# nihofm/volren

Hardware: AMD Instinct MI355X
Metric: Msamples/s (pixels x spp / s), volume path tracing (higher is better)
Workload: dtype f32; 1 GPU; BASELINE configs[1] 'c2': smoke.brick, no transfer function, 1024x1024, 1024 spp, seed 42, fov 40; parallelism=1 GPU, 1 fused launch(es)/frame (sample pool budget 64 GiB)

## Files before the change

### volren_amd/csrc/capi.cpp

```cpp
#include "../../include/volren_amd.h"

#include <algorithm>
#include <cmath>
#include <cstring>
#include <filesystem>
#include <functional>
#include <iostream>
#include <stdexcept>
#include <memory>
#include <string>
#include <vector>

#include "imageio.h"
#include "renderer.h"
#include "sharded.h"
#include "vr_device.h"
#include "vr_math_probe.h"

struct vr_renderer {
    vr::RendererHIP impl;
    int device = 0;
};

struct vr_sharded {
// ... 107 lines not shown

int vr_load_envmap(vr_renderer* r, const char* path) {
    NEED(r);
    if (!path) return fail(VR_ERR_ARG, "null path");
    return guard([&] { use_device(r); r->impl.environment = std::make_shared<vr::Environment>(std::string(path)); r->impl.sample = 0; });
}

int vr_load_transferfunc(vr_renderer* r, const char* path) {
    NEED(r);
    if (!path) return fail(VR_ERR_ARG, "null path");
    return guard([&] {
        use_device(r);
        r->impl.transferfunc = std::make_shared<vr::TransferFunction>(std::string(path));
        r->impl.show_environment = false;
        r->impl.sample = 0;
    });
}

static void install_grid(vr_renderer* r, const char* name, const std::shared_ptr<vr::Grid>& grid, int unit_cube) {
    const std::string n = name ? name : "density";
    auto& R = r->impl;
    if (n == "density") {
        R.volume = std::make_shared<vr::Volume>(grid);
        if (unit_cube) { R.density_scale = 1.f; R.scale_and_move_to_unit_cube(); }
    } else {
        if (!R.volume || R.volume->grids.empty()) throw std::runtime_error("set the density grid before '" + n + "'");
        R.volume->update_grid_frame(R.volume->grid_frame_counter, grid, n);
    }
    R.sample = 0;
}

int vr_set_volume_dense(vr_renderer* r, const char* name, const float* voxels, int nx, int ny, int nz, const float* transform, int unit_cube) {
    NEED(r);
    if (!voxels || nx <= 0 || ny <= 0 || nz <= 0) return fail(VR_ERR_ARG, "bad dense grid arguments");
    return guard([&] {
        use_device(r);
        auto g = std::make_shared<vr::DenseGrid>((uint32_t)nx, (uint32_t)ny, (uint32_t)nz, voxels);
        if (transform) memcpy(g->transform.m, transform, 64);
        install_grid(r, name, g, unit_cube);
    });
}

int vr_volume_add_grid_frame_dense(vr_renderer* r, const char* name, const float* voxels, int nx, int ny, int nz, const float* transform) {
    NEED(r);
    if (!voxels || nx <= 0 || ny <= 0 || nz <= 0) return fail(VR_ERR_ARG, "bad dense grid arguments");
    return guard([&] {
        auto g = std::make_shared<vr::DenseGrid>((uint32_t)nx, (uint32_t)ny, (uint32_t)nz, voxels);
        if (transform) memcpy(g->transform.m, transform, 64);
        if (!r->impl.volume) r->impl.volume = std::make_shared<vr::Volume>();
        r->impl.volume->add_grid_frame(g, name ? name : "density");
        r->impl.sample = 0;
    });
}
int vr_volume_update_grid_frame_dense(vr_renderer* r, int frame, const char* name, const float* voxels, int nx, int ny, int nz, const float* transform) {
    NEED(r);
    if (!voxels || nx <= 0 || ny <= 0 || nz <= 0 || frame < 0) return fail(VR_ERR_ARG, "bad dense grid arguments");
    return guard([&] {
        if (!r->impl.volume || (size_t)frame >= r->impl.volume->n_grid_frames()) throw std::out_of_range("vr_volume_update_grid_frame_dense: no such frame");
        auto g = std::make_shared<vr::DenseGrid>((uint32_t)nx, (uint32_t)ny, (uint32_t)nz, voxels);
        if (transform) memcpy(g->transform.m, transform, 64);
        r->impl.volume->update_grid_frame((size_t)frame, g, name ? name : "density");
        r->impl.sample = 0;
    });
}
int vr_volume_n_grid_frames(vr_renderer* r, int* n) {
    NEED(r);
    if (!n) return fail(VR_ERR_ARG, "null output");
    *n = r->impl.volume ? (int)r->impl.volume->n_grid_frames() : 0;
    return VR_OK;
}

int vr_set_volume_dense_f16(vr_renderer* r, const char* name, const uint16_t* voxels, int nx, int ny, int nz, const float* transform, int unit_cube) {
    NEED(r);
    if (!voxels || nx <= 0 || ny <= 0 || nz <= 0) return fail(VR_ERR_ARG, "bad dense grid arguments");
    return guard([&] {
        use_device(r);
        auto g = std::make_shared<vr::DenseGridF16>((uint32_t)nx, (uint32_t)ny, (uint32_t)nz, voxels);
        if (transform) memcpy(g->transform.m, transform, 64);
        install_grid(r, name, g, unit_cube);
    });
}

int vr_set_volume_brick(vr_renderer* r, const char* name, const float* transform, const uint32_t nb[3], const float min_maj[2],
                        const uint32_t* indirection, const uint32_t* range, const uint32_t atlas_dim[3], const uint8_t* atlas,
                        int n_mips, const uint32_t* const* mips, const uint32_t (*mip_dims)[3], int unit_cube) {
    NEED(r);
    if (!nb || !min_maj || !indirection || !range || !atlas_dim || !atlas || n_mips < 0 || n_mips > 3) return fail(VR_ERR_ARG, "bad brick grid arguments");
    return guard([&] {
        use_device(r);
        auto g = std::make_shared<vr::BrickGrid>();
        if (transform) memcpy(g->transform.m, transform, 64);
        g->n_bricks = { nb[0], nb[1], nb[2] };
        g->min_maj = { min_maj[0], min_maj[1] };
        const size_t n = (size_t)nb[0] * nb[1] * nb[2];
        g->indirection = vr::Buf3D<uint32_t>(nb[0], nb[1], nb[2]);
        g->range = vr::Buf3D<uint32_t>(nb[0], nb[1], nb[2]);
        memcpy(g->indirection.data.data(), indirection, n * 4);
        memcpy(g->range.data.data(), range, n * 4);
        if ((atlas_dim[0] % 8) || (atlas_dim[1] % 8) || (atlas_dim[2] % 8)) throw std::runtime_error("atlas dimensions must be multiples of 8");
        g->atlas = vr::Buf3D<uint8_t>(atlas_dim[0], atlas_dim[1], atlas_dim[2]);
        memcpy(g->atlas.data.data(), atlas, g->atlas.data.size());
        uint64_t cnt = 0;
        for (size_t i = 0; i < n; ++i) cnt += (vr::half2float(range[i] & 0xFFFFu) != vr::half2float(range[i] >> 16));
        g->brick_counter = cnt;
        for (int m = 0; m < n_mips; ++m) {
            vr::Buf3D<uint32_t> b(mip_dims[m][0], mip_dims[m][1], mip_dims[m][2]);
            memcpy(b.data.data(), mips[m], b.data.size() * 4);
            g->range_mipmaps.push_back(std::move(b));
        }
        install_grid(r, name, g, unit_cube);
    });
}

int vr_set_envmap(vr_renderer* r, const float* rgb, int w, int h) {
    NEED(r);
    if (!rgb || w <= 0 || h <= 0) return fail(VR_ERR_ARG, "bad envmap arguments");
    return guard([&] { use_device(r); r->impl.environment = std::make_shared<vr::Environment>(rgb, w, h); r->impl.sample = 0; });
}

int vr_set_transferfunc(vr_renderer* r, const float* rgba, int n) {
    NEED(r);
    return guard([&] {
        use_device(r);
        if (n <= 0 || !rgba) { r->impl.transferfunc.reset(); r->impl.sample = 0; return; }
        std::vector<vr::vec4> lut;
        for (int i = 0; i < n; ++i) lut.emplace_back(rgba[4 * i], rgba[4 * i + 1], rgba[4 * i + 2], rgba[4 * i + 3]);
        r->impl.transferfunc = std::make_shared<vr::TransferFunction>(lut);
        r->impl.sample = 0;
    });
}

int vr_set_int(vr_renderer* r, const char* name, int v) {
    NEED(r);
    if (!name) return fail(VR_ERR_ARG, "null name");
    return guard([&] {
        auto& R = r->impl;
        const std::string n = name;
        if (n == "sample") { R.sample = v; R.drop_tile_samples(); }
        else if (n == "sppx") R.sppx = v;
        else if (n == "seed") R.seed = v;
        else if (n == "bounces") R.bounces = v;
        else if (n == "show_environment") R.show_environment = v != 0;
        else if (n == "tonemapping") R.tonemapping = v != 0;
        else if (n == "integrator") R.integrator = v;
        else if (n == "fast_math") R.fast_math = v != 0;
        else if (n == "variance") { if (v < 0 || v > 1) throw std::runtime_error("variance: 0 (off) or 1 (keep the per-pixel second moments)"); R.variance = v; }
        else if (n == "denoise_iterations") {
            if (v < 0 || v > vr::kDenoiseMaxIterations) throw std::runtime_error("denoise_iterations must be in [0, 10]");
            R.denoise_iterations = v;
        }
        else if (n == "coalesce_trace") { R.flush_pending(); R.coalesce_trace = v != 0; }
        else if (n == "majorant_layout") { if (v < -1 || v > 1) throw std::runtime_error("majorant_layout: -1 (per grid, chosen at commit), 0 (linear), 1 (4x4x4-cell blocks)"); R.majorant_layout = v; }
        else if (n == "tf_float_atlas") R.tf_float_atlas = v != 0;
        else if (n == "wide_addressing") { if (v < 0 || v > 1) throw std::runtime_error("wide_addressing: 0 (by the tables' sizes), 1 (always the kernels with 64-bit gather addresses)"); R.tuning.wide_addressing = v; }
        else if (n == "gpu_encoder") R.gpu_encoder = v != 0;
        else if (n == "sample_pool_mb") { if (v < 16 || v > 65536) throw std::runtime_error("sample_pool_mb must be in [16, 65536] (item indices of a sub-launch are 32-bit: < 2^32 RGBA32F items)"); R.sample_pool_bytes = (size_t)v << 20; }
        else if (n == "launch_target_ms") { if (v < 0) throw std::runtime_error("launch_target_ms must be >= 0 (0 = no sizing by time)"); R.launch_target_ms = v; }
        else if (n == "order_tiles") { if (v < 0 || v > 2) throw std::runtime_error("order_tiles: 0 (never), 1 (tile subsets), 2 (always)"); R.order_tiles = v; }
        else if (n == "grid_frame_counter") {
            if (!R.volume || v < 0 || (size_t)v >= R.volume->n_grid_frames()) throw std::runtime_error("grid_frame_counter out of range");
            R.volume->grid_frame_counter = (size_t)v;
        } else throw std::runtime_error("unknown int parameter: " + n);
    });
}

int vr_get_int(vr_renderer* r, const char* name, int* v) {
    NEED(r);
    if (!name || !v) return fail(VR_ERR_ARG, "null argument");
    return guard([&] {
        auto& R = r->impl;
        const std::string n = name;
        if (n == "sample") *v = R.sample;
        else if (n == "sppx") *v = R.sppx;
        else if (n == "seed") *v = R.seed;
        else if (n == "bounces") *v = R.bounces;
        else if (n == "show_environment") *v = R.show_environment ? 1 : 0;
        else if (n == "tonemapping") *v = R.tonemapping ? 1 : 0;
        else if (n == "integrator") *v = R.integrator;
        else if (n == "fast_math") *v = R.fast_math ? 1 : 0;
        else if (n == "variance") *v = R.variance;
        else if (n == "denoise_iterations") *v = R.denoise_iterations;
        else if (n == "coalesce_trace") *v = R.coalesce_trace ? 1 : 0;
        else if (n == "majorant_layout") *v = R.majorant_layout;
        else if (n == "majorant_blocked") {
            vr::SceneParams P; R.fill_params(P); *v = P.density.maj_blocked;
        }
        else if (n == "kernel_variant" || n == "kernel_variant_reason") {
            vr::SceneParams P; R.fill_params(P);
            int why = 0; const int variant = vr::pathtrace_variant_of(P, &why);
            *v = n == "kernel_variant" ? variant : why;
        }
        else if (n == "wide_addressing") *v = R.tuning.wide_addressing;
        else if (n == "kernel_wide") {
            vr::SceneParams P; R.fill_params(P);
            *v = (vr::pathtrace_wide_of(R.tuning, P) || vr::pathtrace_variant_of(P, nullptr) >= 2) ? 1 : 0;
        }
        else if (n == "env_div_safe") *v = R.environment && R.environment->cdf_div_safe ? 1 : 0;
        else if (n == "env_compact") *v = R.environment && R.environment->envmap_rgbe ? 1 : 0;
        else if (n == "pending_samples") *v = R.pending_samples();
        else if (n == "tf_float_atlas") *v = R.tf_float_atlas ? 1 : 0;
        else if (n == "gpu_encoder") *v = R.gpu_encoder ? 1 : 0;
        else if (n == "sample_pool_mb") *v = (int)(R.sample_pool_bytes >> 20);
        else if (n == "launch_target_ms") *v = R.launch_target_ms;
        else if (n == "order_tiles") *v = R.order_tiles;
        else if (n == "grid_frame_counter") *v = R.volume ? (int)R.volume->grid_frame_counter : 0;
        else if (n == "n_grid_frames") *v = R.volume ? (int)R.volume->n_grid_frames() : 0;
        else if (n == "last_launches") *v = R.last_launches;
        else if (n == "adaptive_rounds") *v = R.adaptive_rounds;
        else if (n == "width") *v = R.resolution.x;
        else if (n == "height") *v = R.resolution.y;
        else throw std::runtime_error("unknown int parameter: " + n);
    });
}

namespace {
struct FloatField { float* ptr; int count; };
FloatField float_field(vr::RendererHIP& R, const std::string& n) {
    if (n == "tonemap_exposure") return { &R.tonemap_exposure, 1 };
    if (n == "tonemap_gamma") return { &R.tonemap_gamma, 1 };
    if (n == "albedo") return { &R.albedo.x, 3 };
    if (n == "phase") return { &R.phase, 1 };
    if (n == "density_scale") return { &R.density_scale, 1 };
    if (n == "emission_scale") return { &R.emission_scale, 1 };
    if (n == "vol_clip_min") return { &R.vol_clip_min.x, 3 };
    if (n == "vol_clip_max") return { &R.vol_clip_max.x, 3 };
    if (n == "cam_pos") return { &R.camera.pos.x, 3 };
    if (n == "cam_dir") return { &R.camera.dir.x, 3 };
    if (n == "cam_up") return { &R.camera.up.x, 3 };
    if (n == "cam_fov") return { &R.camera.fov_degree, 1 };
    if (n == "env_strength") { if (!R.environment) throw std::runtime_error("no environment"); return { &R.environment->strength, 1 }; }
    if (n == "env_transform") { if (!R.environment) throw std::runtime_error("no environment"); return { R.environment->transform.m, 9 }; }
    if (n == "tf_window_left") { if (!R.transferfunc) throw std::runtime_error("no transfer function"); return { &R.transferfunc->window_left, 1 }; }
    if (n == "tf_window_width") { if (!R.transferfunc) throw std::runtime_error("no transfer function"); return { &R.transferfunc->window_width, 1 }; }
    if (n == "volume_transform") { if (!R.volume) throw std::runtime_error("no volume"); return { R.volume->transform.m, 16 }; }
    if (n == "denoise_sigma") return { R.denoise_sigma, 5 };
    if (n == "denoise_alpha") return { &R.denoise_alpha, 1 };
    throw std::runtime_error("unknown float parameter: " + n);
}
}

int vr_set_float(vr_renderer* r, const char* name, const float* values, int count) {
    NEED(r);
    if (!name || !values) return fail(VR_ERR_ARG, "null argument");
    return guard([&] {
        auto& R = r->impl;
        const std::string n = name;
        if (n == "env_rot") {
            if (count != 1) throw std::runtime_error("env_rot takes 1 value");
            if (!R.environment) throw std::runtime_error("no environment");
            R.environment->transform = vr::rotation_axis(values[0], 1);
            return;
        }
        if (n == "albedo" && count == 1) { R.albedo = vr::vec3(values[0]); return; }
        if (n == "denoise_sigma") {
            if (count != 5) throw std::runtime_error("denoise_sigma takes 5 values (colour, normal, depth, coverage, albedo)");
            for (int i = 0; i < 5; ++i)
                if (!(values[i] >= vr::kDenoiseSigmaMin && values[i] <= vr::kDenoiseSigmaMax))
                    throw std::runtime_error("denoise_sigma: every value must be in [2^-60, 2^60]");
        }
        if (n == "denoise_alpha" && count == 1 && !(values[0] >= vr::kTemporalAlphaMin && values[0] <= vr::kTemporalAlphaMax))
            throw std::runtime_error("denoise_alpha must be in [2^-20, 1]");
        const FloatField f = float_field(R, n);
        if (count != f.count) throw std::runtime_error("wrong value count for " + n);
        memcpy(f.ptr, values, sizeof(float) * (size_t)count);
    });
}

int vr_get_float(vr_renderer* r, const char* name, float* values, int count) {
    NEED(r);
    if (!name || !values) return fail(VR_ERR_ARG, "null argument");
    return guard([&] {
        const FloatField f = float_field(r->impl, name);
        if (count != f.count) throw std::runtime_error(std::string("wrong value count for ") + name);
        memcpy(values, f.ptr, sizeof(float) * (size_t)count);
    });
}

int vr_commit(vr_renderer* r) { NEED(r); return guard([&] { use_device(r); r->impl.commit(); }); }
int vr_reset(vr_renderer* r) { NEED(r); return guard([&] { r->impl.reset(); }); }
int vr_scale_and_move_to_unit_cube(vr_renderer* r) { NEED(r); return guard([&] { r->impl.scale_and_move_to_unit_cube(); }); }

int vr_trace(vr_renderer* r) { NEED(r); return guard([&] { use_device(r); r->impl.trace(); }); }
int vr_flush(vr_renderer* r) { NEED(r); return guard([&] { use_device(r); r->impl.flush_pending(); }); }
int vr_render(vr_renderer* r, int spp) { NEED(r); return guard([&] { use_device(r); r->impl.render(spp); }); }

int vr_synchronize(vr_renderer* r) {
    NEED(r);
    return guard([&] {
        use_device(r);
        r->impl.synchronize();
        r->impl.check_watchdog();
    });
}

int vr_last_kernel_ms(vr_renderer* r, double* ms) {
    NEED(r);
    if (!ms) return fail(VR_ERR_ARG, "null argument");
    return guard([&] { use_device(r); *ms = r->impl.last_kernel_ms(); });
}

int vr_last_pathtrace_ms(vr_renderer* r, double* ms) {
    NEED(r);
    if (!ms) return fail(VR_ERR_ARG, "null output");
    return guard([&] { use_device(r); *ms = r->impl.last_pathtrace_ms(); });
}

int vr_framebuffer(vr_renderer* r, float* out) {
    NEED(r);
    if (!out) return fail(VR_ERR_ARG, "null argument");
    return guard([&] { use_device(r); r->impl.download(out); });
}
int vr_render_features(vr_renderer* r, int spp) {
    NEED(r);
    if (vr_device_count() <= 0) return fail(VR_ERR_NO_DEVICE, "no HIP device available (libvolren_amd has no CPU path)");
    return guard([&] { use_device(r); r->impl.render_features(spp); });
}
int vr_features(vr_renderer* r, float* out) {
    NEED(r);
    if (!out) return fail(VR_ERR_ARG, "null argument");
    if (vr_device_count() <= 0) return fail(VR_ERR_NO_DEVICE, "no HIP device available (libvolren_amd has no CPU path)");
    return guard([&] { use_device(r); r->impl.download_features(out); });
}
int vr_variance(vr_renderer* r, float* out) {
    NEED(r);
    if (!out) return fail(VR_ERR_ARG, "null argument");
    if (vr_device_count() <= 0) return fail(VR_ERR_NO_DEVICE, "no HIP device available (libvolren_amd has no CPU path)");
    return guard([&] { use_device(r); r->impl.download_variance(out); });
}
int vr_denoise(vr_renderer* r) {
    NEED(r);
    if (vr_device_count() <= 0) return fail(VR_ERR_NO_DEVICE, "no HIP device available (libvolren_amd has no CPU path)");
    return guard([&] { use_device(r); r->impl.denoise(); });
}
int vr_denoise_temporal(vr_renderer* r) {
    NEED(r);
    if (vr_device_count() <= 0) return fail(VR_ERR_NO_DEVICE, "no HIP device available (libvolren_amd has no CPU path)");
    return guard([&] { use_device(r); r->impl.denoise_temporal(); });
}
int vr_denoise_history_reset(vr_renderer* r) {
    NEED(r);
    if (vr_device_count() <= 0) return fail(VR_ERR_NO_DEVICE, "no HIP device available (libvolren_amd has no CPU path)");
    return guard([&] { use_device(r); r->impl.flush_pending(); r->impl.drop_history(); });
}
int vr_denoise_history(vr_renderer* r, float* rgba_out, float* var_out, float* length_out) {
    NEED(r);
    if (vr_device_count() <= 0) return fail(VR_ERR_NO_DEVICE, "no HIP device available (libvolren_amd has no CPU path)");
    return guard([&] { use_device(r); r->impl.download_history(rgba_out, var_out, length_out); });
}
int vr_denoised(vr_renderer* r, float* out) {
    NEED(r);
    if (!out) return fail(VR_ERR_ARG, "null argument");
    if (vr_device_count() <= 0) return fail(VR_ERR_NO_DEVICE, "no HIP device available (libvolren_amd has no CPU path)");
    return guard([&] { use_device(r); r->impl.download_denoised(out); });
// ... 272 lines not shown
```

### volren_amd/csrc/renderer.cpp

```cpp
#include "renderer.h"

#include <algorithm>
#include <cfloat>
#include <cmath>
#include <cstdlib>
#include <cstring>
#include <iostream>

#include "vr_adaptive.h"
#include "vr_device.h"
#include "vr_math.h"
#include "vr_probe.h"

namespace vr {

mat3 Camera::view_inverse() const {
    const vec3 f = normalize(dir);
    const vec3 s = normalize(cross(f, up));
    const vec3 u = cross(s, f);
    mat3 r(0.0f);
    r.m[0] = s.x; r.m[1] = s.y; r.m[2] = s.z;
    r.m[3] = u.x; r.m[4] = u.y; r.m[5] = u.z;
    r.m[6] = -f.x; r.m[7] = -f.y; r.m[8] = -f.z;
    return r;
// ... 192 lines not shown
}

BrickGridHIP RendererHIP::dense_grid_to_device(const std::shared_ptr<DenseGridF16>& g) {
    BrickGridHIP out;
    const uvec3 nb = g->range.stride;
    out.nb[0] = (int)nb.x; out.nb[1] = (int)nb.y; out.nb[2] = (int)nb.z;
    out.dim[0] = (int)g->dim.x; out.dim[1] = (int)g->dim.y; out.dim[2] = (int)g->dim.z;
    if (g->dim.x > 65535u || g->dim.y > 65535u || g->dim.z > 65535u) throw std::runtime_error("dense_grid_to_device: more than 65535 voxels along an axis");
    out.transform = g->transform;
    const uint32_t bx = (g->dim.x + 3u) / 4u, by = (g->dim.y + 3u) / 4u, bz = (g->dim.z + 3u) / 4u;
    if ((uint64_t)bx * by * bz > (1ull << 31)) throw std::runtime_error("dense_grid_to_device: more than 2^31 blocks");
    out.dblk[0] = (int)bx; out.dblk[1] = (int)by;
    std::vector<uint16_t> blocked((size_t)bx * by * bz * 64u, 0);
    for (uint32_t z = 0; z < g->dim.z; ++z)
        for (uint32_t y = 0; y < g->dim.y; ++y) {
            const uint16_t* row = &g->voxels[((size_t)z * g->dim.y + y) * g->dim.x];
            for (uint32_t x = 0; x < g->dim.x; ++x) blocked[dense_blocked_index(x, y, z, bx, by)] = row[x];
        }
    out.dense = make_device_buffer(blocked.size() * sizeof(uint16_t));
    out.dense->upload(blocked.data(), blocked.size() * sizeof(uint16_t));
    upload_range_words(out, nb, g->range, g->range_mipmaps);
    return out;
}

BrickGridHIP RendererHIP::brick_grid_to_device(const std::shared_ptr<BrickGrid>& g) {
    BrickGridHIP out;
    const uvec3 nb = g->n_bricks;
    const size_t n_bricks = (size_t)nb.x * nb.y * nb.z;
    if (n_bricks == 0) throw std::runtime_error("brick_grid_to_device: empty grid");
    out.nb[0] = (int)nb.x; out.nb[1] = (int)nb.y; out.nb[2] = (int)nb.z;
    out.transform = g->transform;
    const uvec3 ad = g->atlas.stride;
    const uint32_t sx = ad.x / 8, sy = ad.y / 8, sz = ad.z / 8;
    upload_range_words(out, nb, g->range, g->range_mipmaps);
    check_grid_bytes(brick_records(out) * (kBrickBlockBytes + sizeof(BrickRec) + 8), "the brick-linear atlas", out.nb);
    std::vector<BrickRec> recs(brick_records(out), BrickRec{ 0u, 0.f, 0.f, 0u });
    std::vector<uint8_t> atlas(recs.size() * (size_t)kBrickBlockBytes, 0);
    for (size_t i = 0; i < n_bricks; ++i) {
        const uint32_t ind = g->indirection.data[i], rg = g->range.data[i];
        const uint32_t px = ind >> 22, py = (ind >> 12) & 1023u, pz = (ind >> 2) & 1023u;
        const float lo = half2float(rg & 0xFFFFu), hi = half2float(rg >> 16);
        const size_t idx = i;
        BrickRec r;
        r.slot = (uint32_t)idx;
        r.rmin = lo;
        r.rdiff = hi - lo;
        r.range = rg;
        recs[idx] = r;
        uint8_t* dst = &atlas[idx * (size_t)kBrickBlockBytes];
        if (VR_BRICK_HEADERS)
            for (uint32_t l = 0; l < 5; ++l) { memcpy(dst + l * 128u, &r.rmin, 4); memcpy(dst + l * 128u + 4u, &r.rdiff, 4); }
        if (r.rdiff != 0.f && px < sx && py < sy && pz < sz) {
            ++out.n_active;
            for (uint32_t z = 0; z < 8; ++z)
                for (uint32_t y = 0; y < 8; ++y) {
                    const uint8_t* src = &g->atlas.data[g->atlas.index(px * 8, py * 8 + y, pz * 8 + z)];
                    for (uint32_t x = 0; x < 8; ++x) dst[brick_voxel_byte(z * 64 + y * 8 + x)] = src[x];
                }
        }
    }
    out.bricks = make_device_buffer(recs.size() * sizeof(BrickRec));
    out.bricks->upload(recs.data(), recs.size() * sizeof(BrickRec));
    std::vector<float> rng(recs.size() * 2);
    for (size_t i = 0; i < recs.size(); ++i) { rng[2 * i] = recs[i].rmin; rng[2 * i + 1] = recs[i].rdiff; }
    out.rng = make_device_buffer(rng.size() * sizeof(float));
    out.rng->upload(rng.data(), rng.size() * sizeof(float));
    out.atlas = make_device_buffer(atlas.size());
    out.atlas->upload(atlas.data(), atlas.size());
    return out;
}

void RendererHIP::scale_and_move_to_unit_cube() {
    vec3 bb_min(FLT_MAX), bb_max(FLT_MIN);
    for (const auto& frame : volume->grids) {
        const auto grid = frame.at("density");
        const uvec3 e = grid->index_extent();
        bb_min = vmin(bb_min, transform_point(grid->transform, vec3(0.f, 0.f, 0.f)));
        bb_max = vmax(bb_max, transform_point(grid->transform, vec3((float)e.x, (float)e.y, (float)e.z)));
    }
    const vec3 extent = bb_max - bb_min;
    const float size = std::fmax(extent.x, std::fmax(extent.y, extent.z));
    if (size != 1.f) {
        volume->transform = scale_then_translate(1.f / size, -bb_min - extent * 0.5f);
        density_scale *= size;
    }
}

static void copy3(float* dst, vec3 v) { dst[0] = v.x; dst[1] = v.y; dst[2] = v.z; }

static GridView make_view(const BrickGridHIP& g, bool paired = false, bool maj_blocked = false) {
    GridView v;
    memset(&v, 0, sizeof v);
    v.bricks = g.bricks ? g.bricks->as<BrickRec>() : nullptr;
    v.atlas = paired ? g.atlas_paired->as<uint8_t>() : (g.atlas ? g.atlas->as<uint8_t>() : nullptr);
    v.dense = g.dense ? g.dense->as<uint16_t>() : nullptr;
    for (int i = 0; i < 3; ++i) v.dim[i] = g.dim[i];
    for (int i = 0; i < 2; ++i) v.dblk[i] = g.dblk[i];
    v.majorant = g.majorant->as<float>();
    v.majorant16 = g.majorant16->as<uint16_t>();
    v.rng = g.rng ? g.rng->as<float>() : nullptr;
    v.atlas_f32 = g.atlas_f32 ? g.atlas_f32->as<float>() : nullptr;
    for (int i = 0; i < 3; ++i) v.nb[i] = g.nb[i];
    for (int i = 0; i < 3; ++i) { v.mshift[i] = g.mshift[i]; v.mlim[i] = (float)(8u << g.mshift[i]); }
    v.n_mips = g.n_mips;
    v.maj_blocked = maj_blocked ? 1 : 0;
    v.maj_outside = (int32_t)majorant_padded_cells((uint32_t)(g.mshift[0] + g.mshift[1] + g.mshift[2]));
    return v;
}

static float camera_z(float fov_degree) { return -0.5f / tan_(0.5f * kPi * fov_degree / 180.f); }

void RendererHIP::fill_params(SceneParams& P) {
    if (!volume || volume->grids.empty() || density_grids.empty())
        throw std::runtime_error("RendererHIP::trace: no volume committed");
    if (volume->grid_frame_counter >= density_grids.size())
        throw std::runtime_error("RendererHIP::trace: grid_frame_counter out of range (commit() after changing the volume)");
    memset(&P, 0, sizeof P);
    Uniforms& u = P.u;
    u.bounces = bounces;
    u.seed = seed;
    u.show_environment = show_environment ? 1 : 0;
    copy3(u.cam_pos, camera.pos);
    u.cam_fov = camera.fov_degree;
    const mat3 ct = camera.view_inverse();
    memcpy(u.cam_transform, ct.m, sizeof ct.m);
    P.cam_z = camera_z(camera.fov_degree);
    const auto [bb_min, bb_max] = volume->AABB();
    const auto [mn, maj] = volume->minorant_majorant();
    copy3(u.vol_bb_min, bb_min + vol_clip_min * (bb_max - bb_min));
    copy3(u.vol_bb_max, bb_min + vol_clip_max * (bb_max - bb_min));
    u.vol_minorant = mn * density_scale;
    u.vol_majorant = maj * density_scale;
    u.vol_inv_majorant = 1.f / (maj * density_scale);
    copy3(u.vol_albedo, albedo);
    u.vol_phase_g = phase;
    u.vol_density_scale = density_scale;
    u.vol_emission_scale = emission_scale;
    u.vol_emission_norm = majorant_emission > 0.f ? 1.f / std::fmax(majorant_emission, 1e-4f) : 1.f;
    const BrickGridHIP& density = density_grids[volume->grid_frame_counter];
    const mat4 dt = volume->transform * density.transform;
    const mat4 dti = inverse(dt);
    memcpy(u.vol_density_transform, dt.m, sizeof dt.m);
    memcpy(u.vol_density_inv_transform, dti.m, sizeof dti.m);
    P.density = make_view(density);
    if (volume->grid_frame_counter < emission_grids.size()) {
        const BrickGridHIP& emission = emission_grids[volume->grid_frame_counter];
        const mat4 et = volume->transform * emission.transform;
        const mat4 eti = inverse(et);
        memcpy(u.vol_emission_transform, et.m, sizeof et.m);
        memcpy(u.vol_emission_inv_transform, eti.m, sizeof eti.m);
        const mat4 efd = eti * dt;
        memcpy(P.emission_from_density, efd.m, sizeof efd.m);
        const bool scale_ok = u.vol_density_scale >= 1.0f / 65536.0f && u.vol_density_scale <= 16777216.0f;
        P.paired = (integrator == 0 && environment->cdf_div_safe && scale_ok && density.atlas_paired && density.atlas_paired == emission.atlas_paired) ? 1 : 0;
        if (P.paired) P.density = make_view(density, true, majorant_layout < 0 ? density.maj_blocked : majorant_layout == 1);
        P.emission = make_view(emission, P.paired != 0);
        u.has_emission = 1;
    }
    if (transferfunc) {
        u.use_tf = 1;
        u.tf_size = transferfunc->size();
        u.tf_window_left = transferfunc->window_left;
        u.tf_window_width = transferfunc->window_width;
        P.tf_lut = transferfunc->lut_ssbo->as<float>();
    }
    const mat3 eit = inverse(environment->transform);
    memcpy(u.env_transform, environment->transform.m, sizeof eit.m);
    memcpy(u.env_inv_transform, eit.m, sizeof eit.m);
    u.env_strength = environment->strength;
    u.env_imp_inv_dim[0] = u.env_imp_inv_dim[1] = 1.f / (float)environment->dimension();
    u.env_imp_base_mip = (int)std::floor(std::log2((float)environment->dimension()));
    P.envmap = environment->envmap->as<float>();
    P.env_rgbe = environment->envmap_rgbe ? environment->envmap_rgbe->as<uint32_t>() : nullptr;
    P.env_w = environment->width; P.env_h = environment->height;
    P.env_avg_w = environment->avg_importance; P.env_avg_w_set = 1;
    P.impmap = environment->impmap->as<float>();
    P.imp_dim = (int)environment->dimension();
    P.env_cdf = environment->cdf->as<float>();
    P.env_div_safe = environment->cdf_div_safe ? 1 : 0;
    u.resolution[0] = resolution.x; u.resolution[1] = resolution.y;
    u.integrator = integrator;
}

void RendererHIP::update_majorants(const LaunchInputs& in, BrickGridHIP& g) {
    const MajKey& k = in.maj;
    if (k.density_scale == maj_key_.density_scale && k.tf_version == maj_key_.tf_version &&
        k.wl == maj_key_.wl && k.ww == maj_key_.ww && k.frame == maj_key_.frame && k.blocked == maj_key_.blocked)
        return;
    launch_majorants(in.P, g.range_words->as<uint32_t>(), g.nb, g.mip_off, g.n_mips, g.mshift, g.majorant->as<float>(), g.majorant16->as<uint16_t>(), in.stream);
    VR_HIP(hipGetLastError());
    maj_key_ = k;
}

void RendererHIP::set_tiles(const std::vector<int32_t>& tile_ids) {
    flush_pending();
    tiles_host_ = tile_ids;
    tiles_dev_.reset();
    if (tile_ids.empty()) return;
    if (resolution.x > 0) {
        const int n_all = tile_count(resolution.x, resolution.y);
        for (int32_t t : tile_ids)
            if (t < 0 || t >= n_all) throw std::runtime_error("set_tiles: tile id out of range");
    }
    tiles_dev_ = make_device_buffer(tile_ids.size() * sizeof(int32_t));
    tiles_dev_->upload(tile_ids.data(), tile_ids.size() * sizeof(int32_t));
}

std::vector<int32_t> RendererHIP::costliest_first(const SceneParams& P, const std::vector<int32_t>& tile_ids, int n_tiles) const {
    const Uniforms& u = P.u;
    const int W = u.resolution[0], H = u.resolution[1], tiles_x = vr::tiles_x(W);
    std::vector<int32_t> ids(tile_ids);
    if (ids.empty()) { ids.resize((size_t)n_tiles); for (int i = 0; i < n_tiles; ++i) ids[(size_t)i] = i; }
    auto chord = [&](float px, float py) {
        float d[3] = { (px - 0.5f * (float)W) / (float)H, (py - 0.5f * (float)H) / (float)H, P.cam_z };
        float w[3];
        for (int i = 0; i < 3; ++i) w[i] = u.cam_transform[i] * d[0] + u.cam_transform[3 + i] * d[1] + u.cam_transform[6 + i] * d[2];
        const float len = std::sqrt(w[0] * w[0] + w[1] * w[1] + w[2] * w[2]);
        float t0 = 0.f, t1 = FLT_MAX;
        for (int i = 0; i < 3; ++i) {
            const float inv = 1.f / (w[i] / len);
            const float a = (u.vol_bb_min[i] - u.cam_pos[i]) * inv, b = (u.vol_bb_max[i] - u.cam_pos[i]) * inv;
            t0 = std::fmax(t0, std::fmin(a, b)); t1 = std::fmin(t1, std::fmax(a, b));
        }
        return t1 > t0 ? t1 - t0 : 0.f;
    };
    std::vector<float> cost(ids.size());
    for (size_t k = 0; k < ids.size(); ++k) {
        const float x0 = (float)((ids[k] % tiles_x) * 16), y0 = (float)((ids[k] / tiles_x) * 16);
        const float x1 = std::fmin(x0 + 16.f, (float)W), y1 = std::fmin(y0 + 16.f, (float)H);
        cost[k] = std::fmax(std::fmax(std::fmax(chord(x0, y0), chord(x1, y0)), std::fmax(chord(x0, y1), chord(x1, y1))), chord(0.5f * (x0 + x1), 0.5f * (y0 + y1)));
    }
    std::vector<int32_t> perm(ids.size());
    for (size_t k = 0; k < perm.size(); ++k) perm[k] = (int32_t)k;
    const size_t seg = (ids.size() + 7) / 8;
    for (size_t b = 0; b < ids.size(); b += seg)
        std::stable_sort(perm.begin() + (ptrdiff_t)b, perm.begin() + (ptrdiff_t)std::min(ids.size(), b + seg), [&](int32_t x, int32_t y) { return cost[(size_t)x] > cost[(size_t)y]; });
    std::vector<int32_t> ordered(ids.size());
    for (size_t k = 0; k < ids.size(); ++k) ordered[k] = ids[(size_t)perm[k]];
    return ordered;
}

const int32_t* RendererHIP::tile_order(const SceneParams& P, const std::vector<int32_t>& ids, int n_tiles) {
    const Uniforms& u = P.u;
    uint64_t key = 1469598103934665603ull;
    auto mix = [&key](const void* p, size_t nbytes) { const uint8_t* b = static_cast<const uint8_t*>(p); for (size_t i = 0; i < nbytes; ++i) { key ^= b[i]; key *= 1099511628211ull; } };
    mix(u.cam_pos, sizeof u.cam_pos); mix(u.cam_transform, sizeof u.cam_transform); mix(&P.cam_z, sizeof P.cam_z);
    mix(u.vol_bb_min, sizeof u.vol_bb_min); mix(u.vol_bb_max, sizeof u.vol_bb_max); mix(u.resolution, sizeof u.resolution); mix(&n_tiles, sizeof n_tiles);
    if (!ids.empty()) mix(ids.data(), ids.size() * sizeof(int32_t));
    key = key ? key : 1;
    if (order_dev_ && order_key_ == key && order_dev_->size_bytes() == (size_t)n_tiles * sizeof(int32_t)) return order_dev_->as<int32_t>();
    const std::vector<int32_t> ordered = costliest_first(P, ids, n_tiles);
    ensure_buffer(order_dev_, ordered.size() * sizeof(int32_t));
    order_dev_->upload(ordered.data(), ordered.size() * sizeof(int32_t), stream);
    order_key_ = key;
    return order_dev_->as<int32_t>();
}

bool RendererHIP::LaunchInputs::same_launch_as(const LaunchInputs& o) const {
    return memcmp(&P, &o.P, sizeof P) == 0 && frame == o.frame && maj.density_scale == o.maj.density_scale && maj.tf_version == o.maj.tf_version &&
           maj.wl == o.maj.wl && maj.ww == o.maj.ww && maj.blocked == o.maj.blocked && memcmp(tuning.thr, o.tuning.thr, sizeof tuning.thr) == 0 && tuning.stats == o.tuning.stats &&
           tuning.samples_per_unit == o.tuning.samples_per_unit && tuning.blocks_per_cu == o.tuning.blocks_per_cu && tuning.wide_addressing == o.tuning.wide_addressing && order_tiles == o.order_tiles &&
           launch_target_ms == o.launch_target_ms && fast_math == o.fast_math && variance == o.variance && sample_pool_bytes == o.sample_pool_bytes && stream == o.stream;
}

void RendererHIP::capture(LaunchInputs& in) {
    if (!color) throw std::runtime_error("RendererHIP::trace: no framebuffer (call resize first)");
    if (integrator == 2 && !transferfunc) throw std::runtime_error("RendererHIP::trace: integrator 2 (direct volume rendering) needs a transfer function");
    if (integrator < 0 || integrator > 3) throw std::runtime_error("RendererHIP::trace: unknown integrator");
    if (fast_math && transferfunc) throw std::runtime_error("RendererHIP::trace: fast_math is not available while a transfer function is bound (it misses the 1e-3 bound there); set fast_math 0");
    if (!volume || volume->grids.empty() || density_grids.empty()) throw std::runtime_error("RendererHIP::trace: no volume committed");
    if (volume->grid_frame_counter >= density_grids.size()) throw std::runtime_error("RendererHIP::trace: grid_frame_counter out of range (commit() after changing the volume)");
    {
        BrickGridHIP& g = density_grids[volume->grid_frame_counter];
        const bool build = transferfunc && tf_float_atlas && !g.dense && g.atlas && g.rng && !g.atlas_f32 && !g.atlas_f32_failed;
        const bool drop = (!transferfunc || !tf_float_atlas) && (g.atlas_f32 || g.atlas_f32_failed);
        if (build || drop) flush_pending();
        if (build) {
            try {
                const size_t n_blocks = g.atlas->size_bytes() / kBrickBlockBytes, want = n_blocks * 512u * sizeof(float);
                auto drop_others = [&] { for (BrickGridHIP& other : density_grids) if (&other != &g) other.atlas_f32.reset(); };
                size_t free_b = 0, total_b = 0;
                if (hipMemGetInfo(&free_b, &total_b) != hipSuccess) { (void)hipGetLastError(); free_b = ~(size_t)0; }
                if (want > free_b / 2) drop_others();
                try { g.atlas_f32 = make_device_buffer(want); }
                catch (const std::exception&) { (void)hipGetLastError(); drop_others(); g.atlas_f32 = make_device_buffer(want); }
                launch_decode_atlas(g.rng->as<float>(), g.atlas->as<uint8_t>(), g.atlas_f32->as<float>(), n_blocks, stream);
                VR_HIP(hipGetLastError());
            } catch (const std::exception& e) {
                (void)hipGetLastError();
                g.atlas_f32.reset();
                g.atlas_f32_failed = true;
                std::cerr << "volren_amd: no room for the decoded float atlas (" << (g.atlas->size_bytes() / kBrickBlockBytes * 2048u >> 20) << " MiB): transfer-function taps read the byte atlas (" << e.what() << ")" << std::endl;
            }
        }
        if (drop) { g.atlas_f32.reset(); g.atlas_f32_failed = false; }
    }
    fill_params(in.P);
    in.frame = volume->grid_frame_counter;
    in.maj = MajKey{};
    in.maj.density_scale = density_scale;
    in.maj.tf_version = transferfunc ? transferfunc->version : 0;
    in.maj.wl = transferfunc ? transferfunc->window_left : 0.f;
    in.maj.ww = transferfunc ? transferfunc->window_width : 0.f;
    in.maj.frame = in.frame;
    in.maj.blocked = in.P.density.maj_blocked;
    in.tuning = tuning;
    in.order_tiles = order_tiles; in.launch_target_ms = launch_target_ms; in.fast_math = fast_math ? 1 : 0; in.variance = variance != 0 ? 1 : 0;
    in.sample_pool_bytes = sample_pool_bytes;
    in.stream = stream;
    in.env = environment; in.tf = transferfunc;
    in.keep[0] = environment->envmap; in.keep[1] = environment->impmap; in.keep[2] = environment->cdf;
    in.keep[3] = transferfunc ? transferfunc->lut_ssbo : DeviceBufferPtr();
    in.keep[4] = environment->envmap_rgbe;
}

int RendererHIP::samples_per_launch(const LaunchInputs& in, int n_tiles) const {
    const size_t per_sample = pathtrace_pool_floats(in.tuning, n_tiles, 1) * sizeof(float);
    int per_launch = (int)std::max<size_t>(1, in.sample_pool_bytes / per_sample);
    const size_t lim = (size_t)0xFFFFFFFFu / ((size_t)n_tiles * 256u);
    per_launch = (int)std::min<size_t>((size_t)per_launch, lim > 8 ? lim - 8 : 1);
    if (per_launch > 32) per_launch -= per_launch % 32;
    return per_launch;
}

void RendererHIP::submit_tile_set(const LaunchInputs& in, int first, int n) {
    if (n <= 0) return;
    const int n_tiles = tiles_dev_ ? (int)tiles_host_.size() : tile_count(in.P.u.resolution[0], in.P.u.resolution[1]);
    const bool ordered = in.order_tiles >= 2 || (in.order_tiles == 1 && tiles_dev_);
// ... 518 lines not shown
```

### volren_amd/csrc/renderer.h

```cpp
#pragma once

#include <memory>
#include <vector>

#include "devmem.h"
#include "environment.h"
#include "grids.h"
#include "transferfunc.h"
#include "vr_device.h"
#include "vr_scene.h"

namespace vr {

struct Camera {
    vec3 pos{ 1.f, 0.f, 1.f };
    vec3 dir = normalize(-pos);
    vec3 up{ 0.f, 1.f, 0.f };
    float fov_degree = 70.f;
    mat3 view_inverse() const;
};

struct BrickGridHIP {
    DeviceBufferPtr bricks;
    DeviceBufferPtr atlas;
    DeviceBufferPtr range_words;
    DeviceBufferPtr majorant;
    DeviceBufferPtr majorant16;
    DeviceBufferPtr rng;
    DeviceBufferPtr atlas_f32;
    bool atlas_f32_failed = false;
    DeviceBufferPtr atlas_paired;
    DeviceBufferPtr dense;
    int32_t dim[3] = { 0, 0, 0 };
    int32_t dblk[2] = { 0, 0 };
    int32_t nb[3] = { 0, 0, 0 };
    int32_t mip_off[4] = { 0, 0, 0, 0 };
    int32_t n_mips = 0;
    int32_t n_cells = 0;
    int32_t mshift[3] = { 3, 3, 3 };
    size_t n_active = 0;
    bool maj_blocked = false;
    mat4 transform;
};

struct RendererHIP {
    void init();
    void resize(uint32_t w, uint32_t h);
    void commit();
    void trace();
    void draw();
    void reset();

    void render(int n = 0);
    void render_adaptive(int min_spp, int max_spp, float threshold);
    std::vector<int32_t> tile_samples();
    std::vector<float> tile_error();
    bool ragged();
    void drop_tile_samples();
    void check_watchdog();

    BrickGridHIP brick_grid_to_device(const std::shared_ptr<BrickGrid>& grid);
    BrickGridHIP dense_grid_to_device(const std::shared_ptr<DenseGridF16>& grid);
    BrickGridHIP grid_to_device(const Volume::GridPtr& grid);
    BrickGridHIP dense_to_bricks_on_device(const std::shared_ptr<DenseGrid>& grid);
    bool gpu_encoder = true;
    void grid_checksums(const BrickGridHIP& g, uint64_t out[3]) const;
    void scale_and_move_to_unit_cube();

    int sample = 0;
    int sppx = 1024;
    int seed = 42;
    int bounces = 100;
    float tonemap_exposure = 5.f;
    float tonemap_gamma = 2.2f;
    bool tonemapping = true;
    bool show_environment = true;

    vec3 albedo = vec3(0.9f);
    float phase = 0.f;
    float density_scale = 1.f;
    float emission_scale = 100.f;

    DeviceBufferPtr color;
    DeviceBufferPtr display;
    std::vector<BrickGridHIP> density_grids;
    std::vector<BrickGridHIP> emission_grids;
    float majorant_emission = 0.f;

    std::shared_ptr<Volume> volume;

    vec3 vol_clip_min = vec3(0.f);
    vec3 vol_clip_max = vec3(1.f);

    std::shared_ptr<Environment> environment;
    std::shared_ptr<TransferFunction> transferfunc;

    Camera camera;
    ivec2 resolution{ 0, 0 };
    hipStream_t stream = nullptr;
    int integrator = 0;
    bool tf_float_atlas = true;
    int order_tiles = 1;
    int majorant_layout = -1;
    int variance = 0;
    int denoise_iterations = kDenoiseDefaultIterations;
    float denoise_sigma[5] = { kDenoiseDefaultSigma[0], kDenoiseDefaultSigma[1], kDenoiseDefaultSigma[2], kDenoiseDefaultSigma[3], kDenoiseDefaultSigma[4] };
    float denoise_alpha = kTemporalDefaultAlpha;
    bool fast_math = false;
    PathtraceTuning tuning = default_tuning();
    int last_launches = 0;
    int adaptive_rounds = 0;
    int launch_target_ms = 2000;
    size_t sample_pool_bytes = (size_t)64 << 30;

    void set_tiles(const std::vector<int32_t>& tile_ids);
    void fill_params(SceneParams& P);
    void download(float* rgba);
    void render_features(int spp);
    void probe(int what, int form, const uint32_t* in, float* out, size_t n);
    void download_features(float* out);
    void download_variance(float* rgba);
    void denoise();
    void denoise_temporal();
    void drop_history();
    void download_history(float* rgba, float* var, float* length);
    void download_denoised(float* rgba);
    const DeviceBuffer* denoised() const { return denoised_.get(); }
    void draw_from(const DeviceBuffer& src);
    void download_display(float* rgba) const;
    void synchronize();
    void flush_pending();
    int pending_samples() const { return pending_n_; }
    bool coalesce_trace = true;
    double last_kernel_ms();
    double last_pathtrace_ms();
    void sched_stats(bool enable, unsigned long long out[32]);
    void wave_timeline(unsigned long long* out, size_t n_words);
    uint32_t watchdog_status();
    ~RendererHIP();

private:
    struct MajKey { float density_scale = -1.f; uint64_t tf_version = ~0ull; float wl = 0, ww = 0; size_t frame = ~(size_t)0; int blocked = -1; };
    struct LaunchInputs {
        SceneParams P;
        MajKey maj;
        size_t frame = 0;
        PathtraceTuning tuning;
        int order_tiles = 0, launch_target_ms = 0, fast_math = 0, variance = 0;
        size_t sample_pool_bytes = 0;
        hipStream_t stream = nullptr;
        std::shared_ptr<Environment> env;
        std::shared_ptr<TransferFunction> tf;
        DeviceBufferPtr keep[5];
        bool same_launch_as(const LaunchInputs& o) const;
    };
    void capture(LaunchInputs& in);
    void submit(const LaunchInputs& in, int first, int n, const int32_t* tiles, int n_tiles);
    void submit_tile_set(const LaunchInputs& in, int first, int n);
    int samples_per_launch(const LaunchInputs& in, int n_tiles) const;
    LaunchInputs pending_;
    int pending_n_ = 0, pending_first_ = 0, pending_cap_ = 0;
    void update_majorants(const LaunchInputs& in, BrickGridHIP& g);
    std::vector<int32_t> tiles_host_;
    DeviceBufferPtr tiles_dev_;
    DeviceBufferPtr order_dev_;
    uint64_t order_key_ = 0;
    std::vector<int32_t> costliest_first(const SceneParams& P, const std::vector<int32_t>& ids, int n_tiles) const;
    const int32_t* tile_order(const SceneParams& P, const std::vector<int32_t>& ids, int n_tiles);
    std::vector<int32_t> tile_n_;
    int tile_n_sample_ = -1;
    DeviceBufferPtr tile_n_dev_, adaptive_lists_, adaptive_err_;
    bool keep_timing_ = false;
    DeviceBufferPtr status_;
    DeviceBufferPtr pool_;
    DeviceBufferPtr workspace_;
    DeviceBufferPtr stats_;
    DeviceBufferPtr features_;
    DeviceBufferPtr moments_;
    int moments_n_ = -1;
    void check_moments(const char* who);
    DeviceBufferPtr dn_guide_, dn_var_[2], dn_color_[2];
    DeviceBufferPtr denoised_;
    void run_denoise(const char* who, bool temporal);
    DeviceBufferPtr hist_color_[2], hist_record_[2];
    int hist_cur_ = -1;
    TemporalCamera hist_cam_{};
    hipEvent_t ev0_ = nullptr, ev1_ = nullptr;
    std::vector<hipEvent_t> pt_events_;
    size_t pt_events_used_ = 0;
    double last_ms_ = 0.0, last_pathtrace_ms_ = 0.0;
    bool timing_pending_ = false;
    double rate_samples_per_ms_ = 0.0;
    uint64_t rate_key_ = 0, rate_pending_key_ = 0;
    double rate_pending_samples_ = 0.0;
    void harvest_rate(bool wait);
    MajKey maj_key_;
};

using Renderer = RendererHIP;

}
```

### volren_amd/csrc/vr_device.h

```cpp
#pragma once

#include <hip/hip_runtime.h>
#include <stdint.h>

#include "vr_denoise.h"
#include "vr_scene.h"
#include "vr_temporal.h"
#include "vr_tiles.h"

namespace vr {

struct PathtraceTuning {
    int32_t thr[8] = { 64, 0, 56, 0, 60, 60, 64, 0 };
    unsigned long long* stats = nullptr;
    int32_t samples_per_unit = 0;
    int32_t blocks_per_cu = 0;
    int32_t wide_addressing = 0;
};
PathtraceTuning default_tuning();
size_t pathtrace_pool_floats(const PathtraceTuning& T, int32_t n_tiles, int32_t n_samples);
size_t pathtrace_workspace_floats();
void launch_pathtrace(const PathtraceTuning& T, const SceneParams& P, float* fb, float* sample_pool, float* workspace, uint32_t* unit_counter, const int32_t* tiles, int32_t n_tiles,
                      int32_t first_sample, int32_t n_samples, uint32_t* status, hipStream_t stream, bool fast_math = false,
                      hipEvent_t ev_kernel_begin = nullptr, hipEvent_t ev_kernel_end = nullptr,
                      float* moments = nullptr);
constexpr uint32_t kFeatureLostStatus = 4u;
void launch_features(const SceneParams& P, const int32_t* tiles, int32_t n_tiles, int32_t spp, float* out, uint32_t* status, hipStream_t stream);
enum PathtraceVariantReason : int {
    VR_VARIANT_INTEGRATOR = 1,
    VR_VARIANT_ENV_DIVISION = 2,
    VR_VARIANT_DENSITY_SCALE = 4,
    VR_VARIANT_GRID_FORMS = 8
};
int pathtrace_variant_of(const SceneParams& P, int* why);
bool pathtrace_wide_of(const PathtraceTuning& T, const SceneParams& P);
void launch_denoise_prepare(const float* moments, const float* features, int32_t W, int32_t H, int32_t n, float vscale, const int32_t* counts, float* v, float* guide,
                            hipStream_t stream);
void launch_denoise_atrous(const float* cin, const float* vin, const float* guide, int32_t W, int32_t H, int32_t step, const DenoiseSigma& sg,
                           float* cout, float* vout, hipStream_t stream);
void launch_denoise_temporal(const float* color, float* v, const float* guide, const float* hist_color, const float* hist_record, bool same_cam,
                             const TemporalCamera& cur, const TemporalCamera& prev, int32_t W, int32_t H, float alpha, float* out_color, float* out_record,
                             hipStream_t stream);
void launch_adaptive_error(const float* fb, const float* moments, const int32_t* tiles, const int32_t* counts, int32_t n_tiles, int32_t W, int32_t H, float* out,
                           hipStream_t stream);

void launch_tonemap(float* fb, int32_t w, int32_t h, float exposure, float gamma, hipStream_t stream);

void launch_pack_tiles(const float* fb, int32_t w, int32_t h, const int32_t* tiles, int32_t n_tiles, float* packed, hipStream_t stream);
void launch_unpack_tiles(const float* packed, const int32_t* tiles, int32_t n_tiles, float* fb, int32_t w, int32_t h, hipStream_t stream);
void launch_build_impmap(const float* envmap_rgba, int32_t env_w, int32_t env_h, int32_t dim, float* pyramid, hipStream_t stream);

void launch_build_env_cdf(const float* pyramid, int32_t dim, float* table, uint32_t* unsafe_flag, hipStream_t stream);

void launch_majorants(const SceneParams& P, const uint32_t* range_words_all_mips, const int32_t nb[3], const int32_t mip_off[4], int32_t n_mips,
                      const int32_t mshift[3], float* out_padded, uint16_t* out16_padded, hipStream_t stream);

void launch_encode_ranges(const float* dense, const int32_t dim[3], const int32_t nb[3], uint32_t* range, uint32_t* flag, hipStream_t stream);
void launch_encode_bricks(const float* dense, const int32_t dim[3], const int32_t nb[3], const uint32_t* range, const uint32_t* flag,
                          BrickRec* recs, float* rng, uint8_t* atlas, hipStream_t stream);
void launch_range_mip(const uint32_t* src, const int32_t sdim[3], uint32_t* dst, const int32_t ddim[3], hipStream_t stream);

void launch_pair_atlas(const uint8_t* atlas_density, const uint8_t* atlas_emission, uint8_t* out, size_t n_records, hipStream_t stream);

void launch_decode_atlas(const float* rng, const uint8_t* atlas, float* out, size_t n_records, hipStream_t stream);
void launch_math_probe(int32_t fn, const float* a, const float* b, float* out, int32_t n, hipStream_t stream);
void launch_math_sweep(int32_t fn, uint32_t first, float b, float* out, int32_t n, hipStream_t stream);
void launch_fast_math_sweep(int32_t fn, uint32_t first, float* out, int32_t n, hipStream_t stream);
void launch_probe(const SceneParams& P, int32_t what, int32_t form, const uint32_t* in, float* out, uint32_t n, hipStream_t stream);

}
```

### volren_amd/csrc/vr_launch.hip

```cpp
#include <hip/hip_runtime.h>

#include <algorithm>
#include <cstdlib>
#include <map>
#include <mutex>
#include <stdexcept>
#include <string>

#include "vr_device.h"
#include "vr_pathtrace.h"

namespace vr {

template <int INTEGRATOR>
__global__ void __launch_bounds__(256)
item_kernel(const SceneParams P, float* __restrict__ sbuf, const LaunchDesc D) {
    const uint32_t per_unit = (uint32_t)(D.spu * 64);
    const uint32_t g = blockIdx.x * 256u + threadIdx.x;
    const uint32_t u = g / per_unit, item = g - u * per_unit;
    if (u >= D.n_units) return;
    const WorkUnit wu = make_unit(D, P.u.resolution[0], u, sbuf);
    if ((int32_t)item >= wu.n_items) return;
    const int32_t px = wu.px0 + (int32_t)(item & 7u), py = wu.py0 + (int32_t)((item >> 3) & 7u);
    if (px >= P.u.resolution[0] || py >= P.u.resolution[1]) return;
    float L[4];
    if (INTEGRATOR == 2) dvr_sample(P, px, py, wu.first_sample + (int32_t)(item >> 6), L);
    else raymarch_path_sample(P, px, py, wu.first_sample + (int32_t)(item >> 6), L);
    reinterpret_cast<float4*>(sbuf)[wu.base + item] = pack4(L);
}

template <bool MOMENTS>
__global__ void __launch_bounds__(256)
accumulate_kernel(const float* __restrict__ sbuf, float* __restrict__ fb, float* __restrict__ moments, const int32_t* __restrict__ tiles, int32_t n_tiles,
                  int32_t W, int32_t H, int32_t first_sample, int32_t n_samples, int32_t spu) {
    const TilePixel q = wave_tiled_pixel(tiles ? tiles[blockIdx.x] : (int32_t)blockIdx.x, threadIdx.x, W);
    if (q.px >= W || q.py >= H) return;
    float4* texel = reinterpret_cast<float4*>(fb) + (size_t)q.py * W + q.px;
    float4* mtexel = MOMENTS ? reinterpret_cast<float4*>(moments) + (size_t)q.py * W + q.px : nullptr;
    float acc[4] = { 0.0f, 0.0f, 0.0f, 0.0f }, S[4] = { 0.0f, 0.0f, 0.0f, 0.0f };
    if (first_sample > 1) {
        unpack4(*texel, acc);
        if (MOMENTS) unpack4(*mtexel, S);
    }
    const float4* sb = reinterpret_cast<const float4*>(sbuf);
    for (int32_t k = 0; k < n_samples; ++k) {
        const int32_t chunk = k / spu, sl = k - chunk * spu;
        float L[4];
        unpack4(sb[pool_slot<size_t>((size_t)chunk, n_tiles, (size_t)blockIdx.x, (uint32_t)q.sub, spu, (size_t)sl, (uint32_t)q.lane)], L);
        const float a = 1.0f / (float)(first_sample + k);
        for (int32_t c = 0; c < 4; ++c) {
            const float x = sanitize(L[c]);
            const float mu = acc[c], mu1 = mix_(mu, x, a);
            if (MOMENTS) S[c] = mix_(S[c], (x - mu) * (x - mu1), a);
            acc[c] = mu1;
        }
    }
    *texel = pack4(acc);
    if (MOMENTS) *mtexel = pack4(S);
}

template <bool TF>
__global__ void __launch_bounds__(256)
features_kernel(const SceneParams P, const int32_t* __restrict__ tiles, int32_t spp, float* __restrict__ out, uint32_t* __restrict__ status) {
    const int32_t W = P.u.resolution[0], H = P.u.resolution[1];
    const TilePixel q = wave_tiled_pixel(tiles ? tiles[blockIdx.x] : (int32_t)blockIdx.x, threadIdx.x, W);
    if (q.px >= W || q.py >= H) return;
    float f[8];
    if (!feature_pixel<TF>(P, q.px, q.py, spp, f)) atomicOr(status, kFeatureLostStatus);
    float4* o = reinterpret_cast<float4*>(out) + 2u * ((size_t)q.py * W + q.px);
    o[0] = pack4(f);
    o[1] = pack4(f + 4);
}
void launch_features(const SceneParams& P, const int32_t* tiles, int32_t n_tiles, int32_t spp, float* out, uint32_t* status, hipStream_t stream) {
    if (n_tiles <= 0 || spp <= 0) return;
    if (P.u.use_tf) hipLaunchKernelGGL(features_kernel<true>, dim3((unsigned)n_tiles), dim3(256), 0, stream, P, tiles, spp, out, status);
    else hipLaunchKernelGGL(features_kernel<false>, dim3((unsigned)n_tiles), dim3(256), 0, stream, P, tiles, spp, out, status);
}

constexpr int32_t kMaxSamplesPerUnit = 8;
static int32_t samples_per_unit(const PathtraceTuning& T, int variant) { return T.samples_per_unit > 0 ? T.samples_per_unit : ((variant == 1 || variant == 2 || variant == 4) ? 4 : kMaxSamplesPerUnit); }
constexpr int kPtVariants = 5;

PathtraceTuning default_tuning() {
    static std::once_flag once;
    static int32_t env_spu = 0, env_blocks = 0;
    std::call_once(once, [] {
        if (const char* e = getenv("VR_SPU")) env_spu = std::max(1, atoi(e));
        if (const char* e = getenv("VR_BLOCKS_PER_CU")) env_blocks = std::max(0, atoi(e));
    });
    PathtraceTuning T;
    T.samples_per_unit = env_spu;
    T.blocks_per_cu = env_blocks;
    return T;
}

size_t pathtrace_pool_floats(const PathtraceTuning& T, int32_t n_tiles, int32_t n_samples) {
    size_t padded = 0;
    for (int variant = 0; variant < kPtVariants; ++variant) {
        const int32_t spu = std::min(n_samples, samples_per_unit(T, variant));
        padded = std::max(padded, (size_t)((n_samples + spu - 1) / spu) * (size_t)spu);
    }
    return padded * (size_t)n_tiles * 4u * 64u * 4u;
}

extern "C" {
#define VR_PT_DECL(N) \
    int vr_pt_occupancy_##N(int tf, int stats); \
    void vr_pt_launch_##N(int tf, int stats, unsigned grid, hipStream_t stream, const void* P, float* sbuf, float* cold_ws, const void* D, const void* S, uint32_t* status, unsigned long long* stats_buf);
VR_PT_DECL(0) VR_PT_DECL(1) VR_PT_DECL(2) VR_PT_DECL(3) VR_PT_DECL(4) VR_PT_DECL(0_fast) VR_PT_DECL(1_fast) VR_PT_DECL(2_fast) VR_PT_DECL(3_fast) VR_PT_DECL(4_fast)
VR_PT_DECL(0w) VR_PT_DECL(1w) VR_PT_DECL(0w_fast) VR_PT_DECL(1w_fast)
#undef VR_PT_DECL
}
typedef int (*PtOccupancy)(int, int);
typedef void (*PtLaunch)(int, int, unsigned, hipStream_t, const void*, float*, float*, const void*, const void*, uint32_t*, unsigned long long*);
static const PtOccupancy kPtOccupancy[2][2][kPtVariants] = { { { vr_pt_occupancy_0, vr_pt_occupancy_1, vr_pt_occupancy_2, vr_pt_occupancy_3, vr_pt_occupancy_4 },
                                                               { vr_pt_occupancy_0w, vr_pt_occupancy_1w, vr_pt_occupancy_2, vr_pt_occupancy_3, vr_pt_occupancy_4 } },
                                                             { { vr_pt_occupancy_0_fast, vr_pt_occupancy_1_fast, vr_pt_occupancy_2_fast, vr_pt_occupancy_3_fast, vr_pt_occupancy_4_fast },
                                                               { vr_pt_occupancy_0w_fast, vr_pt_occupancy_1w_fast, vr_pt_occupancy_2_fast, vr_pt_occupancy_3_fast, vr_pt_occupancy_4_fast } } };
static const PtLaunch kPtLaunch[2][2][kPtVariants] = { { { vr_pt_launch_0, vr_pt_launch_1, vr_pt_launch_2, vr_pt_launch_3, vr_pt_launch_4 },
                                                         { vr_pt_launch_0w, vr_pt_launch_1w, vr_pt_launch_2, vr_pt_launch_3, vr_pt_launch_4 } },
                                                       { { vr_pt_launch_0_fast, vr_pt_launch_1_fast, vr_pt_launch_2_fast, vr_pt_launch_3_fast, vr_pt_launch_4_fast },
                                                         { vr_pt_launch_0w_fast, vr_pt_launch_1w_fast, vr_pt_launch_2_fast, vr_pt_launch_3_fast, vr_pt_launch_4_fast } } };

int pathtrace_variant_of(const SceneParams& P, int* why) {
    const bool scale_ok = P.u.vol_density_scale >= 1.0f / 65536.0f && P.u.vol_density_scale <= 16777216.0f;
    int reason = 0;
    if (P.u.integrator != 0) reason |= VR_VARIANT_INTEGRATOR;
    if (!P.env_div_safe) reason |= VR_VARIANT_ENV_DIVISION;
    if (!scale_ok) reason |= VR_VARIANT_DENSITY_SCALE;
    int variant;
    if (reason) variant = 3;
    else if (P.u.has_emission) {
        const bool mixed = P.density.dense || P.emission.dense || (VR_PAIRED_ATLAS && !P.paired);
        if (mixed) reason |= VR_VARIANT_GRID_FORMS;
        variant = mixed ? 3 : (P.density.maj_blocked ? 4 : 2);
    } else variant = P.density.dense ? 1 : 0;
    if (why) *why = reason;
    return variant;
}
bool pathtrace_wide_of(const PathtraceTuning& T, const SceneParams& P) {
    if (T.wide_addressing) return true;
    uint64_t m = grid_largest_table_bytes(P.density, P.paired != 0, P.u.use_tf != 0);
    if (P.u.has_emission) m = std::max(m, grid_largest_table_bytes(P.emission, P.paired != 0, false));
    return m >= (1ull << 32);
}
static int pathtrace_variant(const SceneParams& P) {
    int why = 0;
    const int variant = pathtrace_variant_of(P, &why);
    if (why & (VR_VARIANT_ENV_DIVISION | VR_VARIANT_DENSITY_SCALE)) {
        static std::once_flag once;
        std::call_once(once, [&] {
            fprintf(stderr, "volren_amd: note: this scene is rendered by the run-time kernel variant (slower; results unchanged):%s%s\n",
                    (why & VR_VARIANT_ENV_DIVISION) ? " the environment's warp table has thresholds below 2^-76 (vr_get_int env_div_safe = 0);" : "",
                    (why & VR_VARIANT_DENSITY_SCALE) ? " the density scale lies outside [2^-16, 2^24];" : "");
        });
    }
    return variant;
}

static int resident_blocks(const PathtraceTuning& T, int mode, int wide, int variant, bool tf, bool stats) {
    int dev = 0, cus = 0;
    if (hipGetDevice(&dev) != hipSuccess) return 1024;
    static std::mutex mu;
    static std::map<uint32_t, std::pair<int, int>> cache;
    const uint32_t key = ((uint32_t)dev << 8) | ((uint32_t)wide << 6) | ((uint32_t)mode << 5) | ((uint32_t)variant << 2) | (tf ? 2u : 0u) | (stats ? 1u : 0u);
    std::pair<int, int> v;
    {
        std::lock_guard<std::mutex> lock(mu);
        auto it = cache.find(key);
        if (it == cache.end()) {
            if (hipDeviceGetAttribute(&cus, hipDeviceAttributeMultiprocessorCount, dev) != hipSuccess || cus <= 0) cus = 256;
            it = cache.emplace(key, std::make_pair(cus, kPtOccupancy[mode][wide][variant](tf, stats))).first;
        }
        v = it->second;
    }
    const int per_cu = T.blocks_per_cu > 0 ? T.blocks_per_cu : v.second;
    return std::min(v.first * per_cu, kMaxWorkgroups * 4 / kWgWaves);
}

size_t pathtrace_workspace_floats() { return kColdMainFloats + (size_t)kMaxWorkgroups * 4u * (size_t)kColdSideWaveFloats; }

void launch_pathtrace(const PathtraceTuning& T, const SceneParams& P, float* fb, float* sample_pool, float* workspace, uint32_t* unit_counter, const int32_t* tiles, int32_t n_tiles,
                      int32_t first_sample, int32_t n_samples, uint32_t* status, hipStream_t stream, bool fast_math, hipEvent_t ev_kernel_begin, hipEvent_t ev_kernel_end,
                      float* moments) {
    if (n_tiles <= 0 || n_samples <= 0) return;
    SchedParams S;
    for (int i = 0; i < ST_COUNT; ++i) S.thr[i] = T.thr[i];
    LaunchDesc D;
    D.tiles = tiles; D.n_tiles = n_tiles; D.first_sample = first_sample; D.n_samples = n_samples;
    const int variant = pathtrace_variant(P);
    D.spu = std::min(n_samples, samples_per_unit(T, variant));
    const int32_t chunks = (n_samples + D.spu - 1) / D.spu;
    if ((uint64_t)chunks * (uint64_t)n_tiles * 4u * (uint64_t)(D.spu * 64) > 0xFFFFFFFFull)
        throw std::runtime_error("launch_pathtrace: " + std::to_string(n_tiles) + " tiles x " + std::to_string(n_samples) + " samples do not fit the 32-bit item index of one launch");
    D.n_units = (uint32_t)chunks * (uint32_t)n_tiles * 4u;
    D.chunks = (uint32_t)chunks;
    D.seg_len = (D.n_units + kQueueSegments - 1u) / kQueueSegments;
    D.unit_counter = unit_counter;
    S.max_iters = kMaxIdleIters;
    if (S.thr[ST_COLLIDE] <= 0) S.thr[ST_COLLIDE] = (P.u.use_tf || P.u.has_emission) ? 32 : 24;
    const bool tf = P.u.use_tf != 0, stats = T.stats != nullptr;
    const int mode = fast_math ? 1 : 0, wide = pathtrace_wide_of(T, P) ? 1 : 0;
    const int blocks = resident_blocks(T, mode, wide, variant, tf, stats);
    const uint32_t groups_needed = (D.n_units + (uint32_t)kWgWaves - 1u) / (uint32_t)kWgWaves;
    const dim3 grid((unsigned)std::min<uint32_t>((uint32_t)blocks, groups_needed > 0 ? groups_needed : 1u)), block(256);
    if (P.u.integrator == 3 || (P.u.integrator == 2 && P.u.use_tf)) {
        const uint64_t items = (uint64_t)D.n_units * (uint64_t)(D.spu * 64);
        const auto integrate = P.u.integrator == 2 ? item_kernel<2> : item_kernel<3>;
        hipLaunchKernelGGL(integrate, dim3((unsigned)((items + 255) / 256)), block, 0, stream, P, sample_pool, D);
    } else {
        (void)hipMemsetAsync(unit_counter, 0, kQueueSegments * sizeof(uint32_t), stream);
        if (ev_kernel_begin) (void)hipEventRecord(ev_kernel_begin, stream);
        kPtLaunch[mode][wide][variant](tf, stats, grid.x, stream, &P, sample_pool, workspace, &D, &S, status, T.stats);
        if (ev_kernel_end) (void)hipEventRecord(ev_kernel_end, stream);
    }
    const auto accumulate = moments ? accumulate_kernel<true> : accumulate_kernel<false>;
    hipLaunchKernelGGL(accumulate, dim3((unsigned)n_tiles), block, 0, stream, sample_pool, fb, moments, tiles, n_tiles, P.u.resolution[0], P.u.resolution[1],
                       first_sample, n_samples, D.spu);
}

}
```

### volren_amd/csrc/vr_pathtrace.h

```cpp
#pragma once

#include <hip/hip_runtime.h>

#include <type_traits>

#include "vr_tiles.h"
#include "vr_trace.h"

namespace vr {

struct SchedParams {
    int32_t thr[ST_COUNT];
    uint32_t max_iters;
};

constexpr uint32_t kQueueSegments = 8u;
constexpr uint32_t kMaxIdleIters = 1u << 26;
constexpr uint64_t kMaxIdleTicks = 7200000000ull;
struct LaunchDesc {
    const int32_t* tiles;
    int32_t n_tiles, first_sample, n_samples, spu;
    uint32_t n_units, chunks, seg_len;
    uint32_t* unit_counter;
};

__device__ __forceinline__ WorkUnit make_unit(const LaunchDesc& D, int32_t W, uint32_t j, float* sbuf) {
    const uint32_t rem = j / D.chunks, chunk = j - rem * D.chunks;
    const uint32_t slot = rem >> 2, sub = rem & 3u;
    const TilePixel q = wave_tiled_pixel(D.tiles ? D.tiles[slot] : (int32_t)slot, sub * 64u, W);
    WorkUnit wu;
    wu.px0 = q.px;
    wu.py0 = q.py;
    wu.first_sample = D.first_sample + (int32_t)chunk * D.spu;
    wu.n_items = min(D.spu, D.n_samples - (int32_t)chunk * D.spu) * 64;
    wu.base = pool_slot<uint32_t>(chunk, D.n_tiles, slot, sub, D.spu, 0u, 0u);
    wu.out = sbuf;
    return wu;
}

#ifndef VR_WAVES_PER_SIMD
#define VR_WAVES_PER_SIMD 4
#endif
#ifndef VR_MARCH_SPECULATIVE
#define VR_MARCH_SPECULATIVE 1
#endif
#ifndef VR_MARCH_LOADS_PINNED
#define VR_MARCH_LOADS_PINNED (VR_MARCH_STEPS == 2)
#endif
#ifndef VR_DIAG_PAD_VALU
#define VR_DIAG_PAD_VALU 0
#endif
#ifndef VR_DIAG_PAD_SLEEP
#define VR_DIAG_PAD_SLEEP 0
#endif
#ifndef VR_BATCH_REGS
#define VR_BATCH_REGS 1
#endif
#ifndef VR_PRIO_HOT
#define VR_PRIO_HOT 1
#endif
#ifndef VR_PRIO_EVENTS
#define VR_PRIO_EVENTS 0
#endif
#ifndef VR_EMISSION_BY_POINTER
#define VR_EMISSION_BY_POINTER 1
#endif

#ifndef VR_HOT_RI
#define VR_HOT_RI 0
#endif
#ifndef VR_HOT_STRIDE
#define VR_HOT_STRIDE (VR_HOT_RI ? 15 : 12)
#endif
#ifndef VR_WG_WAVES
#define VR_WG_WAVES 4
#endif
#ifndef VR_MAJ_LDS
#define VR_MAJ_LDS 0
#endif
constexpr int32_t kWgWaves = VR_WG_WAVES;
constexpr int32_t kLdsPerWorkgroup = 163840 / 16 * kWgWaves;
constexpr int32_t kLutLdsEntries = 256;
template <class K> constexpr int32_t maj_lds_cells() { return !VR_MAJ_LDS ? 0 : (K::tf ? 2560 : ((K::dense == 0 && K::emission == 0) ? 10240 : 5120)); }
#ifndef VR_COLD_REGS
#define VR_COLD_REGS 0
#endif
template <class K> constexpr bool cold_in_regs() { return VR_COLD_REGS != 0 && !K::tf && K::dense == 1 && K::emission == 0; }
template <class K> constexpr int32_t waves_per_simd() { return cold_in_regs<K>() ? 3 : VR_WAVES_PER_SIMD; }

enum PoolStack : int32_t { Q_READY = 0, Q_NEE = 1, Q_POST = 2, Q_ESC = 3, Q_FREE = 4, Q_COUNT = 5 };

#ifndef VR_LAZY_EMISSION
#define VR_LAZY_EMISSION 1
#endif
template <class K> constexpr bool lazy_emission() { return VR_LAZY_EMISSION != 0 && !VR_HOT_RI && K::emission == 1; }
template <class K> constexpr int32_t hot_stride() { return lazy_emission<K>() ? 15 : VR_HOT_STRIDE; }
constexpr int32_t HOT_EL = 12;
template <class K> constexpr int32_t pool_slots() {
#ifdef VR_NSLOT
    return cold_in_regs<K>() ? 192 : VR_NSLOT;
#else
    if (cold_in_regs<K>()) return 192;
    const int32_t shared = maj_lds_cells<K>() * (K::tf ? 4 : 2) + (K::tf ? kLutLdsEntries * 16 + 16 : kWgWaves * 256);
    const int32_t n = (kLdsPerWorkgroup - shared) / kWgWaves / (hot_stride<K>() * 4 + Q_COUNT);
    return n > 192 ? 192 : n;
#endif
}
constexpr int32_t NSLOT = 192;
constexpr int32_t HOT_COL = VR_HOT_RI ? 12 : 4;
template <int32_t HOT_STRIDE, bool WORLD = false>
struct HotStoreT {
    static constexpr int32_t kStride = HOT_STRIDE;
    uint32_t* base;
    __device__ __forceinline__ void save_first_radiance(v3 eL, int32_t slot) const { uint32_t* p = base + slot * HOT_STRIDE + HOT_EL; p[0] = f2u(eL.x); p[1] = f2u(eL.y); p[2] = f2u(eL.z); }
    __device__ __forceinline__ v3 load_first_radiance(int32_t slot) const { const uint32_t* p = base + slot * HOT_STRIDE + HOT_EL; return v3{ u2f(p[0]), u2f(p[1]), u2f(p[2]) }; }
    float cam_ipos[3];
    __device__ __forceinline__ static uint32_t flags(const Hot& h) { return (uint32_t)h.state | ((uint32_t)h.shadow << 8) | ((uint32_t)h.first << 12) | ((uint32_t)h.mipq << 16); }
    __device__ __forceinline__ void save_new(const Hot& h, int32_t slot) const {
        uint32_t* p = base + slot * HOT_STRIDE;
        p[0] = h.seed;
        const v3 a = WORLD ? h.wpos : h.ipos, d = WORLD ? h.wdir : h.idir;
        p[1] = f2u(a.x); p[2] = f2u(a.y); p[3] = f2u(a.z);
        p[4] = f2u(d.x); p[5] = f2u(d.y); p[6] = f2u(d.z);
        p[7] = f2u(h.t); p[8] = f2u(h.far); p[9] = f2u(h.tau);
        p[10] = f2u(h.Tr);
        p[11] = flags(h);
        if (VR_HOT_RI) { p[12] = f2u(h.ri.x); p[13] = f2u(h.ri.y); p[14] = f2u(h.ri.z); }
    }
    __device__ __forceinline__ void save(const Hot& h, int32_t slot) const {
        uint32_t* p = base + slot * HOT_STRIDE;
        p[0] = h.seed;
        if (WORLD) {
            p[1] = f2u(h.wpos.x); p[2] = f2u(h.wpos.y); p[3] = f2u(h.wpos.z);
            p[4] = f2u(h.wdir.x); p[5] = f2u(h.wdir.y); p[6] = f2u(h.wdir.z);
            if (!h.first) p[10] = f2u(h.Tr);
        } else {
        if (!h.first) { p[1] = f2u(h.ipos.x); p[2] = f2u(h.ipos.y); p[3] = f2u(h.ipos.z); p[10] = f2u(h.Tr); }
        p[4] = f2u(h.idir.x); p[5] = f2u(h.idir.y); p[6] = f2u(h.idir.z);
        }
        p[7] = f2u(h.t); p[8] = f2u(h.far); p[9] = f2u(h.tau);
        p[11] = flags(h);
        if (VR_HOT_RI) { p[12] = f2u(h.ri.x); p[13] = f2u(h.ri.y); p[14] = f2u(h.ri.z); }
    }
    __device__ __forceinline__ void save_marched(const Hot& h, int32_t slot) const {
        uint32_t* p = base + slot * HOT_STRIDE;
        p[0] = h.seed;
        p[7] = f2u(h.t); p[9] = f2u(h.tau);
        if (!h.first) p[10] = f2u(h.Tr);
        p[11] = flags(h);
    }
    __device__ __forceinline__ void load(Hot& h, int32_t slot) const {
        const uint32_t* p = base + slot * HOT_STRIDE;
        h.seed = p[0];
        h.ipos = v3{ u2f(p[1]), u2f(p[2]), u2f(p[3]) };
        h.idir = v3{ u2f(p[4]), u2f(p[5]), u2f(p[6]) };
        if (WORLD) { h.wpos = h.ipos; h.wdir = h.idir; }
        h.ri = VR_HOT_RI ? v3{ u2f(p[12 % HOT_STRIDE]), u2f(p[13 % HOT_STRIDE]), u2f(p[14 % HOT_STRIDE]) } : v3{ 0.0f, 0.0f, 0.0f };
        h.t = u2f(p[7]); h.far = u2f(p[8]); h.tau = u2f(p[9]);
        h.Tr = u2f(p[10]);
        const uint32_t f = p[11];
        h.state = (int32_t)(f & 0xFFu); h.shadow = (int32_t)((f >> 8) & 0xFu); h.first = (int32_t)((f >> 12) & 0xFu);
        h.mipq = (int32_t)(f >> 16);
        h.majorant = 0.0f;
    }
    __device__ __forceinline__ void load_resume(Hot& h, int32_t slot, const float* inv_transform = nullptr) const {
        load(h, slot);
        const bool first = h.first != 0;
        if (WORLD) {
            h.ipos = mat4_point(inv_transform, h.wpos);
            h.idir = mat4_dir(inv_transform, h.wdir);
        } else
        h.ipos = v3{ first ? cam_ipos[0] : h.ipos.x, first ? cam_ipos[1] : h.ipos.y, first ? cam_ipos[2] : h.ipos.z };
        h.Tr = first ? 1.0f : h.Tr;
        if (!VR_HOT_RI) h.ri = rcp3_exact(h.idir);
    }
};
constexpr uint32_t kStatsWaveBase = 32u;
constexpr int32_t kMaxWorkgroups = 2048;
#ifndef VR_COLD_NT_STORES
#define VR_COLD_NT_STORES 0
#endif
template <bool SWAP = false>
struct ColdGlobalT {
    static __device__ __forceinline__ constexpr int32_t phys(int32_t f) {
        return !SWAP ? f : ((f >= C_THR && f < C_THR + 3) ? f + (C_DIR - C_THR) : ((f >= C_DIR && f < C_DIR + 3) ? f - (C_DIR - C_THR) : (f == C_SHPDF ? C_FPL : (f == C_FPL ? C_SHPDF : f))));
    }
    float* base;
    float* side;
    float* col;
    __device__ __forceinline__ float ld(int32_t f) const {
        return f >= C_COL ? col[f - C_COL]
             : f < C_SIDE ? static_cast<const float*>(__builtin_assume_aligned(base, C_STRIDE * 4))[phys(f)]
                          : static_cast<const float*>(__builtin_assume_aligned(side, C_SIDE_STRIDE * 4))[f - C_SIDE];
    }
    __device__ __forceinline__ void st(int32_t f, float v) {
        if (f >= C_COL) col[f - C_COL] = v;
#if VR_COLD_NT_STORES
        else if (f < C_SIDE) __builtin_nontemporal_store(v, static_cast<float*>(__builtin_assume_aligned(base, C_STRIDE * 4)) + phys(f));
#else
        else if (f < C_SIDE) static_cast<float*>(__builtin_assume_aligned(base, C_STRIDE * 4))[phys(f)] = v;
#endif
        else static_cast<float*>(__builtin_assume_aligned(side, C_SIDE_STRIDE * 4))[f - C_SIDE] = v;
    }
};
typedef ColdGlobalT<false> ColdGlobal;
template <bool SWAP>
__device__ __forceinline__ Quad ld4(const ColdGlobalT<SWAP>& c, int32_t f3, int32_t f1) {
    const int32_t p3 = ColdGlobalT<SWAP>::phys(f3), p1 = ColdGlobalT<SWAP>::phys(f1);
    if (f3 + 2 < C_SIDE && f1 < C_SIDE && (p3 & 3) == 0 && p1 == p3 + 3 && ColdGlobalT<SWAP>::phys(f3 + 2) == p3 + 2) {
        const float4 v = *reinterpret_cast<const float4*>(static_cast<const float*>(__builtin_assume_aligned(c.base, C_STRIDE * 4)) + p3);
        return Quad{ v3{ v.x, v.y, v.z }, v.w };
    }
    return Quad{ ld3(c, f3), c.ld(f1) };
}
constexpr int32_t kColdWaveFloats = C_STRIDE * NSLOT, kColdSideWaveFloats = C_SIDE_STRIDE * NSLOT;
constexpr size_t kColdMainFloats = (size_t)kMaxWorkgroups * 4u * (size_t)kColdWaveFloats;

__device__ __forceinline__ uint64_t wave_ballot(bool cond) { return __builtin_amdgcn_ballot_w64(cond); }
__device__ __forceinline__ int32_t popc(uint64_t mask) { return (int32_t)__popcll(mask); }
__device__ __forceinline__ int32_t popc_s(uint64_t mask) { int32_t r; asm("s_bcnt1_i32_b64 %0, %1" : "=s"(r) : "s"(mask) : "scc"); return r; }
__device__ __forceinline__ uint32_t lane_rank(uint64_t mask) {
    return __builtin_amdgcn_mbcnt_hi((uint32_t)(mask >> 32), __builtin_amdgcn_mbcnt_lo((uint32_t)mask, 0u));
}

struct ShleBanks { v3 b[3]; uint32_t item[3]; };
__device__ __forceinline__ uint32_t lane_pull_u(uint32_t src_lane, uint32_t v) { return (uint32_t)__builtin_amdgcn_ds_bpermute((int)(src_lane << 2), (int)v); }
__device__ __forceinline__ float lane_pull(uint32_t src_lane, float v) { return u2f(lane_pull_u(src_lane, f2u(v))); }
template <bool ITEMS>
__device__ __forceinline__ void shle_park(ShleBanks& B, uint32_t* stage, int32_t lane, bool valid, int32_t bs, v3 val, bool with_item, uint32_t item) {
    stage[lane] = 0u;
    __builtin_amdgcn_fence(__ATOMIC_SEQ_CST, "wavefront");
    if (valid) reinterpret_cast<uint8_t*>(stage)[((bs & 63) << 2) + (bs >> 6)] = (uint8_t)((lane + 1) | (ITEMS && with_item ? 0x80 : 0));
    __builtin_amdgcn_fence(__ATOMIC_SEQ_CST, "wavefront");
    const uint32_t w = stage[lane];
#pragma unroll
    for (int k = 0; k < 3; ++k) {
        const uint32_t byte = (w >> (8 * k)) & 0xFFu, src = byte & 0x7Fu;
        const uint32_t from = src ? src - 1u : (uint32_t)lane;
        const float x = lane_pull(from, val.x), y = lane_pull(from, val.y), z = lane_pull(from, val.z);
        B.b[k] = v3{ src ? x : B.b[k].x, src ? y : B.b[k].y, src ? z : B.b[k].z };
        if (ITEMS) { const uint32_t it = lane_pull_u(from, item); B.item[k] = (byte & 0x80u) ? it : B.item[k]; }
    }
}
__device__ __forceinline__ uint32_t bank_home(int32_t lane, int32_t bs) { return bs >= 0 ? (uint32_t)(bs & 63) : (uint32_t)lane; }
__device__ __forceinline__ v3 shle_fetch(const ShleBanks& B, int32_t lane, int32_t bs) {
    const uint32_t home = bank_home(lane, bs);
    const int32_t k = bs >> 6;
    v3 r[3];
#pragma unroll
    for (int j = 0; j < 3; ++j) r[j] = v3{ lane_pull(home, B.b[j].x), lane_pull(home, B.b[j].y), lane_pull(home, B.b[j].z) };
    return v3{ k == 0 ? r[0].x : (k == 1 ? r[1].x : r[2].x), k == 0 ? r[0].y : (k == 1 ? r[1].y : r[2].y), k == 0 ? r[0].z : (k == 1 ? r[1].z : r[2].z) };
}
__device__ __forceinline__ uint32_t item_fetch(const ShleBanks& B, int32_t lane, int32_t bs) {
    const uint32_t home = bank_home(lane, bs);
    const int32_t k = bs >> 6;
    const uint32_t r0 = lane_pull_u(home, B.item[0]), r1 = lane_pull_u(home, B.item[1]), r2 = lane_pull_u(home, B.item[2]);
    return k == 0 ? r0 : (k == 1 ? r1 : r2);
}

constexpr int32_t kBankFields = 20;
static_assert(C_SIDE == 16 && C_SHLE == 16 && C_ITEM == 19 && C_COL == kBankFields, "ColdLocal maps field f to v[f]");
struct ColdBanks { float v[3][kBankFields]; };
struct ColdLocal {
    float v[kBankFields];
    float* col;
    __device__ __forceinline__ float ld(int32_t f) const { return f >= C_COL ? col[f - C_COL] : v[f]; }
    __device__ __forceinline__ void st(int32_t f, float x) { if (f >= C_COL) col[f - C_COL] = x; else v[f] = x; }
};
constexpr uint32_t cold_bits(int32_t first, int32_t n) { return ((1u << n) - 1u) << first; }
constexpr uint32_t kColdNeeR = cold_bits(C_POS, 3) | cold_bits(C_THR, 3) | cold_bits(C_DIR, 3);
constexpr uint32_t kColdNeeW = cold_bits(C_POS, 8) | cold_bits(C_SHLE, 3);
constexpr uint32_t kColdNeeWFirst = cold_bits(C_L, 8) | cold_bits(C_ITEM, 1);
constexpr uint32_t kColdPostR = cold_bits(C_POS, 15) | cold_bits(C_SHLE, 4);
constexpr uint32_t kColdPostW = cold_bits(C_THR, 3) | cold_bits(C_L, 8);
constexpr uint32_t kColdEscR = cold_bits(C_THR, 3) | cold_bits(C_L, 8) | cold_bits(C_ITEM, 1);
__device__ __forceinline__ void cold_clear(ColdLocal& c) {
#pragma unroll
    for (int f = 0; f < kBankFields; ++f) c.v[f] = 0.0f;
    c.col = nullptr;
}
template <uint32_t MASK>
__device__ __forceinline__ void cold_fetch(ColdLocal& c, const ColdBanks& B, int32_t lane, int32_t bs) {
    const uint32_t home = bank_home(lane, bs);
    const int32_t k = bs >> 6;
#pragma unroll
    for (int f = 0; f < kBankFields; ++f)
        if ((MASK >> f) & 1u) {
            const float r0 = lane_pull(home, B.v[0][f]), r1 = lane_pull(home, B.v[1][f]), r2 = lane_pull(home, B.v[2][f]);
            c.v[f] = k == 0 ? r0 : (k == 1 ? r1 : r2);
        }
}
__device__ __forceinline__ uint32_t cold_stage(uint32_t* stage, int32_t lane, int32_t bs, bool flag) {
    stage[lane] = 0u;
    __builtin_amdgcn_fence(__ATOMIC_SEQ_CST, "wavefront");
    if (bs >= 0) reinterpret_cast<uint8_t*>(stage)[((bs & 63) << 2) + (bs >> 6)] = (uint8_t)((lane + 1) | (flag ? 0x80 : 0));
    __builtin_amdgcn_fence(__ATOMIC_SEQ_CST, "wavefront");
    return stage[lane];
}
template <uint32_t MASK, bool FLAGGED>
__device__ __forceinline__ void cold_store(ColdBanks& B, uint32_t w, int32_t lane, const ColdLocal& c) {
#pragma unroll
    for (int k = 0; k < 3; ++k) {
        const uint32_t byte = (w >> (8 * k)) & 0xFFu, src = byte & 0x7Fu;
        const uint32_t from = src ? src - 1u : (uint32_t)lane;
        const bool take = FLAGGED ? byte > 0x80u : src != 0u;
#pragma unroll
        for (int f = 0; f < kBankFields; ++f)
            if ((MASK >> f) & 1u) {
                const float x = lane_pull(from, c.v[f]);
                B.v[k][f] = take ? x : B.v[k][f];
            }
    }
}

struct KernelArgs {
    SceneParams P;
    LaunchDesc D;
    SchedParams S;
    float* sbuf;
    float* cold_ws;
    uint32_t* status;
    unsigned long long* stats;
};
typedef const __attribute__((address_space(4))) KernelArgs* KernargPtr;
__device__ __forceinline__ const KernelArgs& event_args() {
    KernargPtr p = (KernargPtr)__builtin_amdgcn_kernarg_segment_ptr();
    asm volatile("" : "+s"(p));
    return *(const KernelArgs*)p;
}

template <class K, bool STATS>
__global__ void __launch_bounds__(64 * kWgWaves, waves_per_simd<K>())
pathtrace_kernel(const KernelArgs A) {
#ifndef VR_PIN_TAP_POINTERS
#define VR_PIN_TAP_POINTERS 0
#endif
#if VR_PIN_TAP_POINTERS
    SceneParams Ppin = A.P;
    asm volatile("" : "+s"(Ppin.density.atlas), "+s"(Ppin.density.dense));
    const SceneParams& P = Ppin;
#else
    const SceneParams& P = A.P;
#endif
    const int32_t wave = __builtin_amdgcn_readfirstlane(threadIdx.x >> 6), lane = threadIdx.x & 63;
    constexpr int32_t NS = pool_slots<K>() - (STATS ? 3 : 0);

    static_assert(!cold_in_regs<K>() || kWgWaves == 4, "the cold-state-in-registers experiment runs 3 workgroups of 4 wavefronts per CU");
    __shared__ uint8_t lds_q[kWgWaves * Q_COUNT * NS];
    uint8_t* const q = lds_q + wave * (Q_COUNT * NS);
    const uint32_t wave_index = blockIdx.x * (uint32_t)kWgWaves + (uint32_t)wave;
    float* const cold_base = A.cold_ws + (size_t)wave_index * (size_t)kColdWaveFloats;
    float* const side_base = A.cold_ws + kColdMainFloats + (size_t)wave_index * (size_t)kColdSideWaveFloats;
    typedef ColdGlobalT<world_slot<K>()> ColdT;
#define VR_COLD(SLOT) ColdT{ cold_base + (SLOT) * C_STRIDE, side_base + (SLOT) * C_SIDE_STRIDE, reinterpret_cast<float*>(hs.base + (SLOT) * HS + HOT_COL) }
    constexpr bool kColdRegs = cold_in_regs<K>();
    constexpr bool kShleInRegs = !K::tf && !kColdRegs;
    constexpr bool kItemInRegs = kShleInRegs && K::dense == 1;
    static_assert(!kItemInRegs || K::emission == 0, "with an emission grid do_new writes the sample-buffer slot to the side array (no stash to park it from)");
    static_assert(NS <= 192, "ShleBanks holds 3 x 64 slots");
    static_assert(!kColdRegs || (K::emission == 0 && !K::tf), "ColdBanks: no marching-path access to the cold state (EmissionCache), C_COL not wired");
    __shared__ uint32_t lds_stage[kShleInRegs || kColdRegs ? kWgWaves * 64 : 4];
    uint32_t* const stage = lds_stage + (kShleInRegs || kColdRegs ? wave * 64 : 0);
    ShleBanks banks;
    banks.b[0] = banks.b[1] = banks.b[2] = v3{ 0, 0, 0 };
    banks.item[0] = banks.item[1] = banks.item[2] = 0u;
    ColdBanks cb;
    if (kColdRegs) {
#pragma unroll
        for (int k = 0; k < 3; ++k)
#pragma unroll
            for (int f = 0; f < kBankFields; ++f) cb.v[k][f] = 0.0f;
    }
    constexpr int32_t HS = hot_stride<K>();
    constexpr bool kLazyEm = lazy_emission<K>();
    static_assert(VR_BATCH_REGS || !kLazyEm, "the VR_BATCH_REGS=0 swap path moves a marching path's radiance through its cold line: a `first` path of a lazy-emission kernel has none");
    __shared__ uint32_t lds_hot[kWgWaves * HS * NS];
    constexpr bool kWorld = world_slot<K>();
    HotStoreT<HS, kWorld> hs;
    hs.base = lds_hot + wave * (HS * NS);
    {
        const v3 ci = mat4_point(P.u.vol_density_inv_transform, v3{ P.u.cam_pos[0], P.u.cam_pos[1], P.u.cam_pos[2] });
        hs.cam_ipos[0] = u2f(__builtin_amdgcn_readfirstlane(f2u(ci.x)));
        hs.cam_ipos[1] = u2f(__builtin_amdgcn_readfirstlane(f2u(ci.y)));
        hs.cam_ipos[2] = u2f(__builtin_amdgcn_readfirstlane(f2u(ci.z)));
    }
    __shared__ float lds_lut[K::tf ? 4 * kLutLdsEntries : 4];
    const bool lut_in_lds = K::tf && P.u.tf_size <= (uint32_t)kLutLdsEntries;
    const bool emission_on = K::emission == 2 ? P.u.has_emission != 0 : K::emission == 1;
    constexpr int32_t kMajCells = maj_lds_cells<K>();
    typedef typename std::conditional<K::tf, float, uint16_t>::type MajT;
    __shared__ MajT lds_maj[kMajCells > 0 ? kMajCells : 1];
    int32_t maj_first = 0x7FFFFFFF;
    if (kMajCells > 0) {
        const uint32_t k = (uint32_t)(P.density.mshift[0] + P.density.mshift[1] + P.density.mshift[2]);
        const int32_t maj_end = (int32_t)majorant_table_cells(k);
        maj_first = maj_end;
#pragma unroll
        for (int mip = 3; mip >= 0; --mip) {
            const int32_t off = (int32_t)majorant_level_offset(k, (uint32_t)mip);
            if (maj_end - off <= kMajCells) maj_first = off;
        }
        maj_first = __builtin_amdgcn_readfirstlane(maj_first);
        for (int32_t i = (int32_t)threadIdx.x; i < maj_end - maj_first; i += 64 * kWgWaves)
            lds_maj[i] = K::tf ? (MajT)P.density.majorant[maj_first + i] : (MajT)P.density.majorant16[maj_first + i];
    }
    if (K::tf && lut_in_lds)
        for (uint32_t i = threadIdx.x; i < 4u * P.u.tf_size; i += 64u * (uint32_t)kWgWaves) lds_lut[i] = P.tf_lut[i];
    if (K::tf || kMajCells > 0) __syncthreads();

    const int32_t pool = (A.S.thr[ST_BEGIN] > 0 && A.S.thr[ST_BEGIN] < NS) ? A.S.thr[ST_BEGIN] : NS;
    const uint32_t thr_a = (uint32_t)(A.S.thr[ST_NEW] & 255) | ((uint32_t)(A.S.thr[ST_NEE] & 255) << 8) | ((uint32_t)(A.S.thr[ST_POSTNEE] & 255) << 16) | ((uint32_t)(A.S.thr[ST_ESCAPE] & 255) << 24);
    const uint32_t thr_b = (uint32_t)(A.S.thr[ST_MARCH] & 255) | ((uint32_t)pool << 8) | ((uint32_t)(A.S.thr[ST_COLLIDE] & 255) << 16);
#define VR_THR_NEW ((int32_t)(thr_a & 255u))
#define VR_THR_NEE ((int32_t)((thr_a >> 8) & 255u))
#define VR_THR_POST ((int32_t)((thr_a >> 16) & 255u))
#define VR_THR_ESC ((int32_t)(thr_a >> 24))
#define VR_THR_HUNGRY ((int32_t)(thr_b & 255u))
#define VR_POOL ((int32_t)((thr_b >> 8) & 255u))
#define VR_THR_COLLIDE ((int32_t)(thr_b >> 16))
    int32_t cnt_ready = 0, cnt_nee = 0, cnt_post = 0, cnt_esc = 0, cnt_free = pool;
#if VR_READY_FIFO
    int32_t rdy_head = 0;
#endif
    for (int32_t i = lane; i < pool; i += 64) q[Q_FREE * NS + i] = (uint8_t)i;
    __builtin_amdgcn_wave_barrier();

    WorkUnit wu;
    wu.px0 = wu.py0 = 0; wu.first_sample = 1; wu.n_items = 0; wu.base = 0u; wu.out = nullptr;
    uint32_t cursor = 0u;
    bool exhausted = false;
    uint32_t seg_tries = 0u;

    Hot l;
    hot_init(l);
    int32_t slot = -1;

#ifndef VR_STATS_LEVEL
#define VR_STATS_LEVEL 2
#endif
    constexpr bool STATS_T = STATS && VR_STATS_LEVEL >= 2;
    const unsigned long long t_begin_rt = STATS_T ? __builtin_amdgcn_s_memrealtime() : 0ull;
    uint32_t iters = 0u, idle_iters = 0u;
    if (VR_PRIO_EVENTS != VR_PRIO_HOT) __builtin_amdgcn_s_setprio(VR_PRIO_HOT);
    uint32_t t_last = (uint32_t)__builtin_readcyclecounter(), t_elapsed = 0u;
    __shared__ uint32_t lds_stat[STATS ? kWgWaves * 32 : 1];
    if (STATS) { if (lane < 32) lds_stat[wave * 32 + lane] = 0u; __builtin_amdgcn_wave_barrier(); }
    auto stat_add = [&](int i, uint32_t n) __attribute__((always_inline)) { if (lane == 0) lds_stat[wave * 32 + i] += n; };
    uint32_t t_blk = 0u;
    const unsigned long long t_start = STATS_T ? __builtin_readcyclecounter() : 0ull;
#ifndef VR_STAT_SCHED
#define VR_STAT_SCHED 0
#endif
#if VR_STAT_SCHED
    uint32_t t_tail = 0u;
    bool have_tail = false;
#endif
    unsigned long long t_exhausted = 0ull;
#define VR_STAT(ST, N) do { if (STATS) { stat_add(2 * (ST), 1u); stat_add(2 * (ST) + 1, (uint32_t)(N)); if (STATS_T) t_blk = (uint32_t)__builtin_readcyclecounter(); } } while (0)
#define VR_STAT_END(ST) do { if (STATS_T) { stat_add(18 + (ST), (uint32_t)__builtin_readcyclecounter() - t_blk); } } while (0)
#define VR_PUSH(QI, CNT, COND, SLOTV) do { \
        const uint64_t m_ = wave_ballot(COND); \
        if (m_) { if (COND) q[(QI) * NS + (CNT) + (int32_t)lane_rank(m_)] = (uint8_t)(SLOTV); (CNT) += popc(m_); } \
    } while (0)

#ifndef VR_READY_FIFO
#define VR_READY_FIFO 0
#endif
#if VR_READY_FIFO
#define VR_PUSH_READY(COND, SLOTV) do { \
        const uint64_t m_ = wave_ballot(COND); \
        if (m_) { if (COND) { int32_t p_ = rdy_head + cnt_ready + (int32_t)lane_rank(m_); p_ = p_ >= NS ? p_ - NS : p_; q[Q_READY * NS + p_] = (uint8_t)(SLOTV); } cnt_ready += popc(m_); } \
    } while (0)
#else
#define VR_PUSH_READY(COND, SLOTV) VR_PUSH(Q_READY, cnt_ready, COND, SLOTV)
#endif
#define VR_ROUTE_ST(BS, STV) do { \
         \
        const int32_t s_ = (BS) >= 0 ? (STV) : -1; \
        VR_PUSH_READY((uint32_t)(s_ - ST_MARCH) < 2u, BS);                         \
        VR_PUSH(Q_NEE, cnt_nee, s_ == ST_NEE, BS); \
        VR_PUSH(Q_POST, cnt_post, s_ == ST_POSTNEE, BS); \
        VR_PUSH(Q_ESC, cnt_esc, s_ == ST_ESCAPE, BS); \
        const bool lost_ = s_ == ST_BEGIN || s_ > ST_ESCAPE || s_ < -1; \
        if (wave_ballot(lost_)) { if (lost_) atomicOr(event_args().status, 2u); } \
        const int32_t free0_ = cnt_free; \
        VR_PUSH(Q_FREE, cnt_free, s_ == ST_NEW || lost_, BS); \
        if (cnt_free != free0_) { idle_iters = 0u; t_elapsed = 0u; }           \
    } while (0)
#define VR_ROUTE(BS) VR_ROUTE_ST(BS, l.state)
#define VR_ROUTE_B(BS) VR_ROUTE_ST(BS, b.state)

    for (;;) {
        ++iters;
        bool give_up = ++idle_iters > kMaxIdleIters;
        if ((iters & 1023u) == 0u) {
            const uint32_t now = (uint32_t)__builtin_readcyclecounter(), d = now - t_last;
            t_last = now;
            if (d < (1u << 31)) t_elapsed += d >> 10;
            give_up = give_up || t_elapsed > (uint32_t)(kMaxIdleTicks >> 10);
        }
        if (give_up) {
            if (lane == 0) atomicOr(event_args().status, 1u);
            break;
        }
#if VR_STAT_SCHED
        uint32_t t_sec = STATS_T ? (uint32_t)__builtin_readcyclecounter() : 0u;
        if (STATS_T && have_tail) stat_add(26 + 4, t_sec - t_tail);
#define VR_SECTION(K) do { if (STATS_T) { const uint32_t n_ = (uint32_t)__builtin_readcyclecounter(); stat_add(26 + (K), n_ - t_sec); t_sec = n_; } } while (0)
#else
#define VR_SECTION(K) do { } while (0)
#endif
        {
            const uint64_t idle = wave_ballot(slot < 0);
            const int32_t take = min(popc(idle), cnt_ready);
            if (take > 0) {
                if (STATS) stat_add(14, 1u);
                if (slot < 0) {
                    const int32_t r = (int32_t)lane_rank(idle);
                    if (r < take) {
#if VR_READY_FIFO
                        int32_t p_ = rdy_head + r; p_ = p_ >= NS ? p_ - NS : p_;
                        slot = q[Q_READY * NS + p_]; hs.load_resume(l, slot, kWorld ? event_args().P.u.vol_density_inv_transform : nullptr);
#else
                        slot = q[Q_READY * NS + cnt_ready - 1 - r]; hs.load_resume(l, slot, kWorld ? event_args().P.u.vol_density_inv_transform : nullptr);
#endif
                        if (emission_on && !l.shadow) {
                            if (kLazyEm && l.first) { l.ethr = v3{ 1.0f, 1.0f, 1.0f }; l.eL = hs.load_first_radiance(slot); }
                            else { const ColdT c = VR_COLD(slot); l.ethr = ld3(c, C_THR); l.eL = ld3(c, C_L); }
                        }
                    }
                }
                cnt_ready -= take;
#if VR_READY_FIFO
                rdy_head += take; rdy_head = rdy_head >= NS ? rdy_head - NS : rdy_head;
#endif
            }
        }
        VR_SECTION(0);
#if !VR_STAT_SCHED
        if (STATS_T) { stat_add(26, (uint32_t)popc(wave_ballot(slot >= 0))); stat_add(27, (uint32_t)cnt_ready); stat_add(28, (uint32_t)cnt_nee); stat_add(29, (uint32_t)cnt_post); stat_add(30, (uint32_t)cnt_esc); stat_add(31, (uint32_t)cnt_free); }
#endif
#ifndef VR_HOT_PAIRS
#define VR_HOT_PAIRS 4
#endif
#ifndef VR_HOT_PAIRS_TF_EMISSION
#define VR_HOT_PAIRS_TF_EMISSION 4
#endif
        constexpr int kHotPairs = (K::tf && K::emission == 1) ? (VR_HOT_PAIRS_TF_EMISSION < VR_HOT_PAIRS ? VR_HOT_PAIRS_TF_EMISSION : VR_HOT_PAIRS) : VR_HOT_PAIRS;

#ifndef VR_HOT_PAIR_MIN
#define VR_HOT_PAIR_MIN 44
#endif
#ifndef VR_DRAIN
#define VR_DRAIN 0
#endif
#ifndef VR_BALLOT_VALID
#define VR_BALLOT_VALID 1
#endif
        const uint64_t holds_path = wave_ballot(slot >= 0);
#ifndef VR_CLEAN_FORMS
#define VR_CLEAN_FORMS VR_CLEAN_FLAG
#endif
#ifndef VR_CLEAN_FORMS_TF_EMISSION
#define VR_CLEAN_FORMS_TF_EMISSION 1
#endif
        constexpr bool kCleanForms = VR_CLEAN_FORMS && ((K::tf && K::emission == 1) ? VR_CLEAN_FORMS_TF_EMISSION != 0 : true);
        const bool all_clean = kCleanForms && (holds_path & wave_ballot((int32_t)f2u(l.far) < 0)) == 0ull;
#ifndef VR_EARLY_MARCH
#define VR_EARLY_MARCH 0
#endif
        constexpr bool kEarlyMarch = VR_EARLY_MARCH != 0 && VR_MARCH_SPECULATIVE && VR_MARCH_STEPS == 2 && K::global == 0 && !K::tf && K::emission == 0 && !K::maj_reuse && maj_lds_cells<K>() == 0;
        MarchIO pre;
        march_idle(pre); pre.maj1 = pre.maj2 = 0u;
        auto hot_pair = [&](auto clean_tag, const int hot_rep_, const int n_copies_) __attribute__((always_inline)) -> bool {
            constexpr bool CLEAN = decltype(clean_tag)::value;
#if VR_BALLOT_VALID
            if (hot_rep_ > 0 && popc_s(holds_path & wave_ballot((uint32_t)(l.state - ST_MARCH) < 2u)) < (VR_DRAIN && exhausted ? 1 : VR_HOT_PAIR_MIN)) return false;
#else
            if (hot_rep_ > 0 && popc(wave_ballot(slot >= 0 && (uint32_t)(l.state - ST_MARCH) < 2u)) < VR_HOT_PAIR_MIN) return false;
#endif
            if (STATS_T) t_blk = (uint32_t)__builtin_readcyclecounter();
            const bool is_m = slot >= 0 && l.state == ST_MARCH;
#if VR_MARCH_SPECULATIVE
            MarchIO mio;
            if (kEarlyMarch && hot_rep_ > 0) mio = pre;
            else {
            march_idle(mio);
            if (is_m) march_prep<K::dense, K::majb, CLEAN>(l, P, mio);
            if constexpr (kMajCells > 0) march_load_lds<K::tf, MajT, K::a32>(P, mio, lds_maj, maj_first);
            else if constexpr (K::maj_reuse) march_load_reuse<K::tf, K::a32>(P, mio, l);
            else march_load<K::tf, K::a32>(P, mio);
#if VR_MARCH_LOADS_PINNED
            asm volatile("" : "+v"(mio.maj1), "+v"(mio.maj2));
#endif
            }
            if (is_m) march_finish<K::tf, K::maj_reuse, CLEAN>(l, P, mio);
#else
            for (int32_t k = 0; k < 2; ++k)
                if (slot >= 0 && l.state == ST_MARCH) do_march<K::tf, K::dense, K::majb>(l, P);
#endif
            if (STATS) { const int32_t nm = popc(wave_ballot(is_m)); if (nm) { stat_add(2 * ST_MARCH, 1u); stat_add(2 * ST_MARCH + 1, (uint32_t)nm); } }
            if (STATS_T) { const uint32_t t_now = (uint32_t)__builtin_readcyclecounter(); stat_add(18 + ST_MARCH, t_now - t_blk); t_blk = t_now; }
#if VR_DIAG_PAD_VALU > 0
            {
                float pad_ = l.t;
#pragma unroll
                for (int k_ = 0; k_ < VR_DIAG_PAD_VALU; ++k_) asm volatile("v_add_f32 %0, 1.0, %0" : "+v"(pad_));
                asm volatile("" :: "v"(pad_));
            }
#endif
#if VR_DIAG_PAD_SLEEP > 0
            __builtin_amdgcn_s_sleep(VR_DIAG_PAD_SLEEP);
#endif
            const bool is_c = slot >= 0 && l.state == ST_COLLIDE;
#if VR_BALLOT_VALID
            const int32_t n_c = popc(holds_path & wave_ballot(l.state == ST_COLLIDE));
            const int32_t n_m = popc(holds_path & wave_ballot(l.state == ST_MARCH));
#else
            const int32_t n_c = popc(wave_ballot(is_c));
            const int32_t n_m = popc(wave_ballot(slot >= 0 && l.state == ST_MARCH));
#endif
            const bool run_c = n_c > 0 && n_c >= min(VR_THR_COLLIDE, (n_c + n_m + 1) >> 1);
            if (kEarlyMarch) {
                CollideIO<K> cio;
                collide_idle<K>(cio);
                if (run_c) {
                    if (is_c) collide_prep<K, CLEAN>(l, P, P, cio);
                    collide_load<K>(P, P, cio);
                }
                const bool early = hot_rep_ + 1 < n_copies_;
                if (early) {
                    const bool spec = run_c && is_c;
                    Hot ls = l;
                    ls.mipq = spec ? (l.mipq > 8 ? l.mipq - 8 : 0) : l.mipq;
                    march_idle(pre);
                    if (slot >= 0 && (l.state == ST_MARCH || spec)) march_prep<K::dense, K::majb, CLEAN>(ls, P, pre);
                    march_load<K::tf, K::a32>(P, pre);
                    if (VR_EARLY_MARCH == 1) asm volatile("" : "+v"(cio.d.raw), "+v"(cio.d.rmin), "+v"(cio.d.rdiff));
                }
                if (run_c) {
                    if (is_c) { ColdT c = VR_COLD(slot); collide_finish<K, ColdT, true>(l, c, P, P, cio, P.tf_lut); }
                    if (STATS) { stat_add(2 * ST_COLLIDE, 1u); stat_add(2 * ST_COLLIDE + 1, (uint32_t)n_c); }
                }
                if (early) asm volatile("" : "+v"(pre.maj1), "+v"(pre.maj2));
            } else
            if (run_c) {
                CollideIO<K> cio;
                collide_idle<K>(cio);
                const SceneParams& PE = VR_EMISSION_BY_POINTER && K::emission != 0 ? event_args().P : P;
#ifndef VR_COLLIDE_BY_POINTER
#define VR_COLLIDE_BY_POINTER 1
#endif
                const SceneParams& PF = (VR_COLLIDE_BY_POINTER && K::tf && (K::global == 2 || K::emission == 1)) ? event_args().P : P;
                if (is_c) collide_prep<K, CLEAN>(l, PF, PE, cio);
                collide_load<K>(PF, PE, cio);
                if (is_c) {
                    ColdT c = VR_COLD(slot);
                    if (lut_in_lds) collide_finish<K, ColdT, true>(l, c, PF, PE, cio, lds_lut);
                    else collide_finish<K, ColdT, true>(l, c, PF, PE, cio, PF.tf_lut);
                }
                if (STATS) { stat_add(2 * ST_COLLIDE, 1u); stat_add(2 * ST_COLLIDE + 1, (uint32_t)n_c); }
            }
            __builtin_amdgcn_s_waitcnt(0x0F70);
            if (STATS_T) stat_add(18 + ST_COLLIDE, (uint32_t)__builtin_readcyclecounter() - t_blk);
            return true;
        };
        if constexpr (kCleanForms) {
            if (all_clean) {
#pragma unroll
                for (int hot_rep_ = 0; hot_rep_ < kHotPairs; ++hot_rep_) if (!hot_pair(std::true_type{}, hot_rep_, kHotPairs)) break;
            } else hot_pair(std::false_type{}, 0, 1);
        } else {
#pragma unroll
            for (int hot_rep_ = 0; hot_rep_ < kHotPairs; ++hot_rep_) if (!hot_pair(std::false_type{}, hot_rep_, kHotPairs)) break;
        }
        VR_SECTION(1);
        {
            const int32_t ps = (slot >= 0 && l.state != ST_MARCH && l.state != ST_COLLIDE) ? l.state : -1;
            if (wave_ballot(ps >= 0)) {
                if (STATS) stat_add(15, 1u);
                if (ps >= 0) {
                    hs.save_marched(l, slot);
                    if (emission_on && !l.shadow) {
                        if (kLazyEm && l.first) hs.save_first_radiance(l.eL, slot);
                        else { ColdT c = VR_COLD(slot); st3(c, C_L, l.eL); }
                    }
                }
                VR_PUSH(Q_NEE, cnt_nee, ps == ST_NEE, slot);
                VR_PUSH(Q_POST, cnt_post, ps == ST_POSTNEE, slot);
                VR_PUSH(Q_ESC, cnt_esc, ps == ST_ESCAPE, slot);
                if (ps >= 0) slot = -1;
            }
        }
        VR_SECTION(2);
        int32_t n;
        const int32_t n_live = popc(wave_ballot(slot >= 0)) + cnt_ready;
        const bool hungry = n_live < VR_THR_HUNGRY;
        const int32_t c_new = exhausted ? 0 : cnt_free;
        int32_t big = c_new;
        if (cnt_nee > big) big = cnt_nee;
        if (cnt_post > big) big = cnt_post;
        if (cnt_esc > big) big = cnt_esc;
        const bool drain_all = VR_DRAIN && exhausted;
        const bool want_new = c_new > 0 && (c_new >= VR_THR_NEW || (hungry && c_new == big));
        const bool want_nee = cnt_nee > 0 && (cnt_nee >= VR_THR_NEE || (hungry && (cnt_nee == big || drain_all)));
        const bool want_post = cnt_post > 0 && (cnt_post >= VR_THR_POST || (hungry && (cnt_post == big || drain_all)));
        const bool want_esc = cnt_esc > 0 && (cnt_esc >= VR_THR_ESC || (hungry && (cnt_esc == big || drain_all)));
        if (want_new || want_nee || want_post || want_esc) {
#if VR_BATCH_REGS
            Hot b;
#else
            const int32_t my_slot = slot;
            const float my_majorant = l.majorant;
            if (my_slot >= 0) { hs.save(l, my_slot); if (emission_on && !l.shadow) { ColdT c = VR_COLD(my_slot); st3(c, C_L, l.eL); } }
            __builtin_amdgcn_wave_barrier();
            Hot& b = l;
#endif
            if (VR_PRIO_EVENTS != VR_PRIO_HOT) __builtin_amdgcn_s_setprio(VR_PRIO_EVENTS);
            if (want_esc) {
                n = min(64, cnt_esc);
                VR_STAT(ST_ESCAPE, n);
                int32_t bs = -1;
                if (lane < n) { bs = q[Q_ESC * NS + cnt_esc - 1 - lane]; hs.load(b, bs); if (kLazyEm && b.first) b.eL = hs.load_first_radiance(bs); }
                if (kItemInRegs) b.item = item_fetch(banks, lane, bs);
                if constexpr (kColdRegs) {
                    ColdLocal c;
                    cold_clear(c);
                    cold_fetch<kColdEscR>(c, cb, lane, bs);
                    if (lane < n) {
                        const KernelArgs& E = event_args();
                        WorkUnit w; w.out = E.sbuf;
                        do_escape<ColdLocal, false>(b, c, E.P, w);
                    }
                } else
                if (lane < n) {
                    const ColdT c = VR_COLD(b.first ? 0 : bs);
                    const KernelArgs& E = event_args();
                    WorkUnit w; w.out = E.sbuf;
                    do_escape<ColdT, kItemInRegs, kLazyEm, kWorld>(b, c, E.P, w);
                }
                cnt_esc -= n;
                VR_ROUTE_B(bs);
                VR_STAT_END(ST_ESCAPE);
            }
            if (want_post) {
                n = min(64, cnt_post);
                VR_STAT(ST_POSTNEE, n);
                int32_t bs = -1;
                if (lane < n) { bs = q[Q_POST * NS + cnt_post - 1 - lane]; hs.load(b, bs); }
                if (kShleInRegs) b.shle = shle_fetch(banks, lane, bs);
                if (kItemInRegs) b.item = item_fetch(banks, lane, bs);
                if constexpr (kColdRegs) {
                    ColdLocal c;
                    cold_clear(c);
                    cold_fetch<kColdPostR>(c, cb, lane, bs);
                    if (lane < n) {
                        const KernelArgs& E = event_args();
                        WorkUnit w; w.out = E.sbuf;
                        do_postnee<K, ColdLocal, false, false>(b, c, E.P, w);
                        hs.save(b, bs);
                    }
                    cold_store<kColdPostW, false>(cb, cold_stage(stage, lane, bs, false), lane, c);
                } else
                if (lane < n) {
                    ColdT c = VR_COLD(bs);
                    const KernelArgs& E = event_args();
                    WorkUnit w; w.out = E.sbuf;
                    do_postnee<K, ColdT, kShleInRegs, kItemInRegs>(b, c, E.P, w);
                    hs.save(b, bs);
                }
                cnt_post -= n;
                VR_ROUTE_B(bs);
                VR_STAT_END(ST_POSTNEE);
            }
            if (want_new) {
                if (cursor == (uint32_t)wu.n_items) {
                    const KernelArgs& E = event_args();
                    uint32_t j = 0xFFFFFFFFu;
                    while (seg_tries < kQueueSegments) {
                        const uint32_t k = ((blockIdx.x & (kQueueSegments - 1u)) + seg_tries) & (kQueueSegments - 1u);
                        const uint32_t lo = k * E.D.seg_len, hi = min(lo + E.D.seg_len, E.D.n_units);
                        uint32_t v = 0xFFFFFFFFu;
                        if (lo < hi) { if (lane == 0) v = atomicAdd(E.D.unit_counter + k, 1u); v = __builtin_amdgcn_readfirstlane(v); }
                        if (lo < hi && v < hi - lo) { j = lo + v; break; }
                        ++seg_tries;
                    }
                    if (j == 0xFFFFFFFFu) { exhausted = true; if (STATS_T) t_exhausted = __builtin_amdgcn_s_memrealtime(); }
                    else { wu = make_unit(E.D, E.P.u.resolution[0], j, nullptr); cursor = 0u; idle_iters = 0u; t_elapsed = 0u; }
                }
                n = min(min(64, cnt_free), (int32_t)((uint32_t)wu.n_items - cursor));
                if (n > 0) {
                    VR_STAT(ST_NEW, n);
                    int32_t bs = -1;
                    if (lane < n) {
                        bs = q[Q_FREE * NS + cnt_free - 1 - lane];
                        hot_init(b);
                        ColdT c = VR_COLD(bs);
                        do_new<K, ColdT, kLazyEm>(b, c, event_args().P, wu, cursor + (uint32_t)lane);
                        hs.save_new(b, bs);
                        if (kLazyEm) hs.save_first_radiance(v3{ 0.0f, 0.0f, 0.0f }, bs);
                    }
                    cnt_free -= n;
                    cursor += (uint32_t)n;
                    VR_ROUTE_B(bs);
                    VR_STAT_END(ST_NEW);
                }
            }
            if (want_nee) {
                n = min(64, cnt_nee);
                VR_STAT(ST_NEE, n);
                int32_t bs = -1;
                bool was_first = false;
                uint32_t first_item = 0u;
                if (lane < n) { bs = q[Q_NEE * NS + cnt_nee - 1 - lane]; hs.load(b, bs); }
                if constexpr (kColdRegs) {
                    ColdLocal c;
                    cold_clear(c);
                    cold_fetch<kColdNeeR>(c, cb, lane, bs);
                    if (lane < n) {
                        was_first = b.first != 0;
                        do_nee<K, ColdLocal, false, false>(b, c, c, event_args().P);
                        hs.save(b, bs);
                    }
                    const uint32_t w = cold_stage(stage, lane, bs, was_first);
                    cold_store<kColdNeeW, false>(cb, w, lane, c);
                    if (wave_ballot(was_first)) cold_store<kColdNeeWFirst, true>(cb, w, lane, c);
                } else
                if (lane < n) {
                    was_first = b.first != 0; first_item = f2u(b.Tr);
                    if (kLazyEm && b.first) b.eL = hs.load_first_radiance(bs);
                    ColdT c = VR_COLD(bs);
                    const ColdT crd = VR_COLD(b.first ? 0 : bs);
                    do_nee<K, ColdT, kShleInRegs, kItemInRegs, kLazyEm>(b, c, crd, event_args().P);
                    hs.save(b, bs);
                }
                if (kShleInRegs) shle_park<kItemInRegs>(banks, stage, lane, bs >= 0, bs, b.shle, was_first, first_item);
                cnt_nee -= n;
                VR_ROUTE_B(bs);
                VR_STAT_END(ST_NEE);
            }
#if !VR_BATCH_REGS
            __builtin_amdgcn_wave_barrier();
            if (my_slot >= 0) { hs.load_resume(l, my_slot); l.majorant = my_majorant; if (emission_on && !l.shadow) { const ColdT c = VR_COLD(my_slot); l.ethr = ld3(c, C_THR); l.eL = ld3(c, C_L); } }
#endif
        }
        if (VR_PRIO_EVENTS != VR_PRIO_HOT) __builtin_amdgcn_s_setprio(VR_PRIO_HOT);
        VR_SECTION(3);
#if VR_STAT_SCHED
        t_tail = t_sec; have_tail = true;
#endif
        if (exhausted && cnt_free == VR_POOL) break;
    }
    unsigned long long* const stats = A.stats;
    if (STATS && stats) {
        stat_add(16, iters);
        stat_add(17, 1u);
        __builtin_amdgcn_wave_barrier();
        if (lane < 32 && lane != 25) atomicAdd(&stats[lane], (unsigned long long)lds_stat[wave * 32 + lane]);
        if (STATS_T && lane == 0) {
            atomicAdd(&stats[25], __builtin_readcyclecounter() - t_start);
            stats[kStatsWaveBase + 3u * wave_index] = t_begin_rt;
            stats[kStatsWaveBase + 3u * wave_index + 1u] = t_exhausted;
            stats[kStatsWaveBase + 3u * wave_index + 2u] = __builtin_amdgcn_s_memrealtime();
        }
    }
#undef VR_STAT
#undef VR_COLD
#undef VR_THR_NEW
#undef VR_THR_NEE
#undef VR_THR_POST
#undef VR_THR_ESC
#undef VR_THR_HUNGRY
#undef VR_POOL
#undef VR_THR_COLLIDE
#undef VR_STAT_END
#undef VR_SECTION
#undef VR_PUSH
#undef VR_PUSH_READY
#undef VR_ROUTE
#undef VR_ROUTE_B
#undef VR_ROUTE_ST
}

}
```

### volren_amd/csrc/vr_probe.h

```cpp
#pragma once

#include "vr_trace.h"

namespace vr {

enum ProbeWhat { PROBE_VOXEL = 0, PROBE_TRILINEAR, PROBE_MAJORANT, PROBE_IMPORTANCE, PROBE_TEXEL, PROBE_SKY, PROBE_LIGHT, PROBE_TF, PROBE_COUNT };
constexpr int32_t kProbeInWords = 4;
VR_HD int32_t probe_out_words(int32_t what) {
    return what == PROBE_LIGHT ? 7 : (what == PROBE_TF ? 4 : ((what == PROBE_TEXEL || what == PROBE_SKY) ? 3 : 1));
}

struct ProbeForm { int32_t dense, pair, majb, f32; bool tf, clean; };
inline ProbeForm probe_decode_form(int32_t what, int32_t form) {
    ProbeForm f{ 0, 0, 0, 0, false, false };
    if (what == PROBE_VOXEL) { f.dense = form % 3; f.pair = form / 3; }
    else if (what == PROBE_TRILINEAR) { f.dense = form % 3; f.pair = (form / 3) % 2; f.f32 = form / 6; }
    else if (what == PROBE_MAJORANT) { f.tf = (form & 1) != 0; f.dense = (form >> 1) % 3; f.majb = (form / 6) % 3; f.clean = form / 18 != 0; }
    return f;
}

inline const char* probe_form_error(const SceneParams& P, int32_t what, int32_t form) {
    if (what < 0 || what >= PROBE_COUNT) return "unknown probe";
    if (form < 0) return "negative form";
    const ProbeForm f = probe_decode_form(what, form);
    const bool dense_grid = P.density.dense != nullptr;
    switch (what) {
    case PROBE_VOXEL:
    case PROBE_TRILINEAR:
        if (what == PROBE_VOXEL ? form >= 9 : form >= 12) return "form out of range";
        if (f.pair != 0 && f.dense != 0) return "no kernel reads a paired atlas in a DENSE form other than 0";
        if (f.pair != 0 && !P.paired) return "PAIR form on a scene without a paired atlas";
        if (f.dense == 0 && dense_grid) return "DENSE = 0 form on a dense density grid";
        if (f.dense == 1 && !dense_grid) return "DENSE = 1 form on a brick density grid";
        if (f.f32 && (dense_grid || !P.density.atlas_f32)) return "no decoded float atlas (needs a brick grid, a LUT and tf_float_atlas)";
        return nullptr;
    case PROBE_MAJORANT:
        if (form >= 36) return "form out of range";
        if (!((f.dense == 0 && f.majb == 0) || (f.dense == 1 && f.majb == 0) || (f.dense == 0 && f.majb == 1) || (f.dense == 2 && f.majb == 2)))
            return "no kernel is compiled for this (DENSE, MAJB)";
        if (f.clean && f.dense == 2) return "the run-time variant has no CLEAN form";
        if (f.tf != (P.u.use_tf != 0)) return "TF form does not match the scene (a kernel's TF instance is chosen by use_tf)";
        if (f.dense == 0 && dense_grid) return "DENSE = 0 form on a dense density grid";
        if (f.dense == 1 && !dense_grid) return "DENSE = 1 form on a brick density grid";
        if (f.majb != 2 && (f.majb == 1) != (P.density.maj_blocked != 0)) return "MAJB form does not match the layout the table is built in";
        return nullptr;
    case PROBE_IMPORTANCE: return form > 2 ? "form out of range" : nullptr;
    case PROBE_TEXEL:
        if (form > 1) return "form out of range";
        return (form == 1 && !P.env_rgbe) ? "the environment map has no compact form" : nullptr;
    case PROBE_SKY: return form != 0 ? "form out of range" : nullptr;
    case PROBE_LIGHT:
        if (form > 1) return "form out of range";
        return (form == 0 && !P.env_div_safe) ? "the div_core sampler on a warp table that failed the division check (env_div_safe = 0)" : nullptr;
    case PROBE_TF:
        if (form != 0) return "form out of range";
        return P.u.use_tf ? nullptr : "no transfer function bound";
    }
    return "unknown probe";
}

inline const char* probe_items_error(const SceneParams& P, int32_t what, int32_t form, const uint32_t* in, size_t n) {
    const ProbeForm f = probe_decode_form(what, form);
    for (size_t i = 0; i < n; ++i) {
        const uint32_t* w = in + kProbeInWords * i;
        if (what == PROBE_VOXEL || what == PROBE_TRILINEAR) {
            if (w[0] > 1u) return "grid must be 0 (density) or 1 (emission)";
            if (w[0] == 1u && !P.u.has_emission) return "no emission grid";
            if (f.pair != 0 && w[0] != (what == PROBE_VOXEL ? (uint32_t)f.pair - 1u : 0u)) return "PAIR 1 reads the density grid, PAIR 2 the emission grid";
            if (w[0] == 1u && (f.f32 || f.dense == 1)) return "only the density grid has a decoded float atlas or a compiled-in dense form";
            if (w[0] == 1u && f.dense == 0 && P.emission.dense) return "DENSE = 0 form on a dense emission grid";
        } else if (what == PROBE_MAJORANT) {
            if (w[3] > 3u) return "mip must be 0..3 (the table has four levels)";
            if (f.clean)
                for (int k = 0; k < 3; ++k) { const float x = u2f(w[k]); if (!(abs_(x) < kCleanBound)) return "CLEAN form: positions must be finite and below 2^20"; }
        } else if (what == PROBE_IMPORTANCE && form == 0) {
            if ((int32_t)w[2] < 0 || (int32_t)w[2] > P.u.env_imp_base_mip) return "mip outside the pyramid";
        }
    }
    return nullptr;
}

template <int DENSE, int PAIR>
VR_HD float probe_voxel(const GridView& g, int32_t x, int32_t y, int32_t z) {
    const TapAddr a = tap_addr<DENSE>(g, x, y, z);
    return tap_value<DENSE>(g, tap_load<DENSE, PAIR>(g, a), a.in);
}
template <int DENSE, int PAIR>
VR_HD float probe_trilinear(const SceneParams& P, const GridView& g, v3 ipos) {
    TriIO io;
    trilinear_prep<DENSE>(g, ipos, io);
    trilinear_load<DENSE, PAIR>(g, io);
    return P.u.vol_density_scale * trilinear_value<DENSE>(g, io);
}
template <bool TF, int DENSE, int MAJB, bool CLEAN>
VR_HD float probe_majorant(const SceneParams& P, v3 ipos, int32_t mip) {
    if (!CLEAN) return majorant_at<TF, DENSE, MAJB>(P, ipos, mip);
    const int32_t idx = majorant_index<DENSE, MAJB, CLEAN>(P.density, ipos, mip);
    return majorant_of<TF>(P, idx, majorant_fetch<TF>(P.density, idx));
}

VR_HD void probe_item(const SceneParams& P, int32_t what, int32_t form, const uint32_t* w, float* out) {
    const float fx = u2f(w[0]), fy = u2f(w[1]), fz = u2f(w[2]);
    switch (what) {
    case PROBE_VOXEL: {
        const GridView& g = w[0] ? P.emission : P.density;
        const int32_t x = (int32_t)w[1], y = (int32_t)w[2], z = (int32_t)w[3];
        switch (form) {
        case 0: out[0] = probe_voxel<0, 0>(g, x, y, z); break;
        case 1: out[0] = probe_voxel<1, 0>(g, x, y, z); break;
        case 2: out[0] = probe_voxel<2, 0>(g, x, y, z); break;
        case 3: out[0] = probe_voxel<0, 1>(g, x, y, z); break;
        case 6: out[0] = probe_voxel<0, 2>(g, x, y, z); break;
        default: out[0] = nan_(); break;
        }
        break;
    }
    case PROBE_TRILINEAR: {
        GridView g = w[0] ? P.emission : P.density;
        if (form < 6) g.atlas_f32 = nullptr;
        const v3 p{ u2f(w[1]), u2f(w[2]), u2f(w[3]) };
        switch (form % 6) {
        case 0: out[0] = probe_trilinear<0, 0>(P, g, p); break;
        case 1: out[0] = probe_trilinear<1, 0>(P, g, p); break;
        case 2: out[0] = probe_trilinear<2, 0>(P, g, p); break;
        case 3: out[0] = probe_trilinear<0, 1>(P, g, p); break;
        default: out[0] = nan_(); break;
        }
        break;
    }
    case PROBE_MAJORANT: {
        const v3 p{ fx, fy, fz };
        const int32_t mip = (int32_t)w[3];
#define VR_PROBE_MAJ(TF, DENSE, MAJB, CLEAN) case ((TF ? 1 : 0) + 2 * DENSE + 6 * MAJB + (CLEAN ? 18 : 0)): out[0] = probe_majorant<TF, DENSE, MAJB, CLEAN>(P, p, mip); break;
        switch (form) {
        VR_PROBE_MAJ(false, 0, 0, false) VR_PROBE_MAJ(true, 0, 0, false) VR_PROBE_MAJ(false, 0, 0, true) VR_PROBE_MAJ(true, 0, 0, true)
        VR_PROBE_MAJ(false, 1, 0, false) VR_PROBE_MAJ(true, 1, 0, false) VR_PROBE_MAJ(false, 1, 0, true) VR_PROBE_MAJ(true, 1, 0, true)
        VR_PROBE_MAJ(false, 0, 1, false) VR_PROBE_MAJ(true, 0, 1, false) VR_PROBE_MAJ(false, 0, 1, true) VR_PROBE_MAJ(true, 0, 1, true)
        VR_PROBE_MAJ(false, 2, 2, false) VR_PROBE_MAJ(true, 2, 2, false)
        default: out[0] = nan_(); break;
        }
#undef VR_PROBE_MAJ
        break;
    }
    case PROBE_IMPORTANCE:
        if (form == 0) out[0] = imp_fetch(P, (int32_t)w[0], (int32_t)w[1], (int32_t)w[2]);
        else if (form == 1) out[0] = env_average_importance(P);
        else { SceneParams Q; Q.u.env_imp_base_mip = P.u.env_imp_base_mip; Q.impmap = P.impmap; Q.imp_dim = P.imp_dim; Q.env_avg_w_set = 0; Q.env_avg_w = 0.0f; out[0] = env_average_importance(Q); }
        break;
    case PROBE_TEXEL: {
        SceneParams Q;
        Q.envmap = P.envmap; Q.env_rgbe = form == 1 ? P.env_rgbe : nullptr; Q.env_w = P.env_w; Q.env_h = P.env_h;
        const v3 c = env_texture(Q, fx, fy);
        out[0] = c.x; out[1] = c.y; out[2] = c.z;
        break;
    }
    case PROBE_SKY: {
        const v3 c = lookup_environment(P, v3{ fx, fy, fz });
        out[0] = c.x; out[1] = c.y; out[2] = c.z;
        break;
    }
    case PROBE_LIGHT: {
        v3 wi, Le; float pdf;
        if (form == 0) sample_environment<true, true>(P, fx, fy, wi, Le, pdf);
        else sample_environment<false, false>(P, fx, fy, wi, Le, pdf);
        out[0] = wi.x; out[1] = wi.y; out[2] = wi.z; out[3] = Le.x; out[4] = Le.y; out[5] = Le.z; out[6] = pdf;
        break;
    }
    case PROBE_TF: tf_lookup(P, fx, out); break;
    default: break;
    }
}

}
```

### volren_amd/csrc/vr_trace.h

```cpp
#pragma once

#include "vr_math.h"
#include "vr_scene.h"

#if defined(VR_HOST_TRACE) && !defined(__HIP_DEVICE_COMPILE__)
namespace vr {
enum TraceClass : int32_t { TR_MAJORANT = 0, TR_TAP = 1, TR_ENV_WARP = 2, TR_ENV_TEXEL = 3 };
void host_trace(int32_t cls, const void* table, size_t a, size_t b);
}
#define VR_TRACE(CLS, TABLE, A, B) ::vr::host_trace((CLS), (TABLE), (size_t)(A), (size_t)(B))
#else
#define VR_TRACE(CLS, TABLE, A, B) do { } while (0)
#endif

namespace vr {

enum LaneState : int32_t {
    ST_NEW = 0,
    ST_BEGIN = 1,
    ST_MARCH = 2,
    ST_COLLIDE = 3,
    ST_NEE = 4,
    ST_POSTNEE = 5,
    ST_ESCAPE = 6,
// ... 471 lines not shown
#if VR_TAP_CHAIN
        uint32_t st_ = sh8;
#if defined(__HIP_DEVICE_COMPILE__)
#define VR_TAP_KEEP(X) asm("" : "+v"(X))
#else
#define VR_TAP_KEEP(X) do { } while (0)
#endif
#define VR_TAP(J, V, W, S, N) do { \
            st_ = st_ * 1664525u + (1013904223u << 8); \
            VR_TAP_KEEP(st_); \
            const float x_ = fma_((float)st_, S, -(W));      \
            J = x_ < -kTapBand ? V : J; \
            amin = __builtin_fminf(amin, __builtin_fabsf(x_)); \
        } while (0)
#else
#define VR_TAP(J, V, W, S, N) do { \
            constexpr LcgJump g_ = lcg_jump(N); \
            const float x_ = fma_((float)(sh8 * g_.A + (g_.C << 8)), S, -(W));      \
            J = x_ < -kTapBand ? V : J; \
            amin = __builtin_fminf(amin, __builtin_fabsf(x_)); \
        } while (0)
#endif
#else
        const uint32_t lo24 = seed & 0x00FFFFFFu;
        bool unsure = false;
#define VR_TAP(J, V, W, S, N) do { \
            constexpr LcgJump g_ = lcg_jump(N); \
            bool yes_, no_; \
            tricubic_fast_test((float)((mul24(lo24, g_.A & 0x00FFFFFFu) + g_.C) & 0x00FFFFFFu), W, S, yes_, no_); \
            J = yes_ ? V : J; \
            unsure = unsure | !(yes_ | no_); \
        } while (0)
#endif
        VR_TAP(jx, 1, fx.w2, fx.s2, 1); VR_TAP(jy, 1, fy.w2, fy.s2, 2); VR_TAP(jz, 1, fz.w2, fz.s2, 3);
        VR_TAP(jx, 2, fx.w3, fx.s3, 4); VR_TAP(jy, 2, fy.w3, fy.s3, 5); VR_TAP(jz, 2, fz.w3, fz.s3, 6);
        VR_TAP(jx, 3, fx.w4, 6.0f, 7); VR_TAP(jy, 3, fy.w4, 6.0f, 8); VR_TAP(jz, 3, fz.w4, 6.0f, 9);
#undef VR_TAP
#if VR_TAP_ABS_BAND && VR_TAP_PRESHIFT
        const bool unsure = !(amin > kTapBand);
#endif
        rng_skip9(seed);
        exact = unsure;
        if (unsure) { seed = seed0; jx = jy = jz = 0; }
    } else {
        flx = floor_(ipos.x - 0.5f); fly = floor_(ipos.y - 0.5f); flz = floor_(ipos.z - 0.5f);
    }
    if (exact) {
        const AxisWeights ax = tricubic_axis_weights(ipos.x - 0.5f);
        const AxisWeights ay = tricubic_axis_weights(ipos.y - 0.5f);
        const AxisWeights az = tricubic_axis_weights(ipos.z - 0.5f);
        float r;
        r = rng(seed); if (r < ax.w2 / ax.s2) jx = 1;
        r = rng(seed); if (r < ay.w2 / ay.s2) jy = 1;
        r = rng(seed); if (r < az.w2 / az.s2) jz = 1;
        r = rng(seed); if (r < ax.w3 / ax.s3) jx = 2;
        r = rng(seed); if (r < ay.w3 / ay.s3) jy = 2;
        r = rng(seed); if (r < az.w3 / az.s3) jz = 2;
        r = rng(seed); if (r < ax.w4 / ax.s4) jx = 3;
        r = rng(seed); if (r < ay.w4 / ay.s4) jy = 3;
        r = rng(seed); if (r < az.w4 / az.s4) jz = 3;
    }
#endif
    tx = voxel_index(flx, jx - 1); ty = voxel_index(fly, jy - 1); tz = voxel_index(flz, jz - 1);
    if (GUARD) tx = nan_guard(tx, flx, fly, flz);
}
template <bool GUARD = true>
VR_HD void tricubic_tap(v3 ipos, uint32_t& seed, int32_t& tx, int32_t& ty, int32_t& tz) { tricubic_tap_t<VR_TAP_FAST != 0, GUARD>(ipos, seed, tx, ty, tz); }

VR_HD void tf_lookup_at(const Uniforms& u, const float* lut, float d, float rgba[4]) {
    const float tc = clamp_((d - u.tf_window_left) / u.tf_window_width, 0.0f, 1.0f - 1e-6f);
    const float tcs = tc * (float)u.tf_size;
    int32_t idx = floor2i(tcs);
    const float f = tcs - floor_(tcs);
    const int32_t n = (int32_t)u.tf_size;
    if (idx == kIntMin) idx = 0;
    idx = idx < 0 ? 0 : (idx > n - 1 ? n - 1 : idx);
    const int32_t idx1 = idx + 1 < n - 1 ? idx + 1 : n - 1;
    const float* a = lut + 4 * idx;
    const float* b = lut + 4 * idx1;
#pragma unroll
    for (int k = 0; k < 4; ++k) rgba[k] = mix_(a[k], b[k], f);
}
VR_HD void tf_lookup(const SceneParams& P, float d, float rgba[4]) { tf_lookup_at(P.u, P.tf_lut, d, rgba); }

VR_HD int32_t wrap_repeat(int32_t i, int32_t n) {
    if ((uint32_t)(i + n) < 3u * (uint32_t)n) return i < 0 ? i + n : (i >= n ? i - n : i);
    const int32_t m = i % n;
    return m < 0 ? m + n : m;
}
VR_HD int32_t clampi(int32_t i, int32_t lo, int32_t hi) { return i < lo ? lo : (i > hi ? hi : i); }

VR_HD void ld_pair(const uint32_t* p, uint32_t& a, uint32_t& b) {
#if defined(__HIP_DEVICE_COMPILE__)
    typedef uint32_t Pair __attribute__((ext_vector_type(2), aligned(4)));
    const Pair v = *reinterpret_cast<const Pair*>(p);
    a = v.x; b = v.y;
#else
    a = p[0]; b = p[1];
#endif
}
VR_HD void ld_quad(const float* p, float out[4]) {
#if defined(__HIP_DEVICE_COMPILE__)
    typedef float Quad4 __attribute__((ext_vector_type(4), aligned(4)));
    const Quad4 v = *reinterpret_cast<const Quad4*>(p);
    out[0] = v.x; out[1] = v.y; out[2] = v.z; out[3] = v.w;
#else
    out[0] = p[0]; out[1] = p[1]; out[2] = p[2]; out[3] = p[3];
#endif
}
VR_HD float rgbe_scale(uint32_t q) { const uint32_t e = q >> 24; return e ? u2f((e - 9u) << 23) : 0.0f; }
VR_HD v3 env_texture(const SceneParams& P, float u, float v) {
    const int32_t w = P.env_w, h = P.env_h;
    const float x = u * (float)w - 0.5f, y = v * (float)h - 0.5f;
    float fx = x - floor_(x), fy = y - floor_(y);
    int32_t ix = floor2i(x), iy = floor2i(y);
    if (ix == kIntMin || iy == kIntMin || ix > (1 << 28) || ix < -(1 << 28)) { ix = 0; iy = 0; fx = 0.0f; fy = 0.0f; }
    const int32_t x0 = wrap_repeat(ix, w), x1 = wrap_repeat(ix + 1, w);
    const int32_t y0 = clampi(iy, 0, h - 1), y1 = clampi(iy + 1, 0, h - 1);
    if (P.env_rgbe) {
        uint32_t q00, q10, q01, q11;
        if (x1 == x0 + 1) {
            ld_pair(P.env_rgbe + ((size_t)y0 * w + x0), q00, q10);
            ld_pair(P.env_rgbe + ((size_t)y1 * w + x0), q01, q11);
        } else {
            q00 = P.env_rgbe[(size_t)y0 * w + x0]; q10 = P.env_rgbe[(size_t)y0 * w + x1]; q01 = P.env_rgbe[(size_t)y1 * w + x0]; q11 = P.env_rgbe[(size_t)y1 * w + x1];
        }
        VR_TRACE(3, P.env_rgbe, ((size_t)y0 * w + x0) * 4, 4); VR_TRACE(3, P.env_rgbe, ((size_t)y0 * w + x1) * 4, 4);
        VR_TRACE(3, P.env_rgbe, ((size_t)y1 * w + x0) * 4, 4); VR_TRACE(3, P.env_rgbe, ((size_t)y1 * w + x1) * 4, 4);
        const float s00 = rgbe_scale(q00), s10 = rgbe_scale(q10), s01 = rgbe_scale(q01), s11 = rgbe_scale(q11);
        v3 r;
        r.x = mix_(mix_((float)(q00 & 255u) * s00, (float)(q10 & 255u) * s10, fx), mix_((float)(q01 & 255u) * s01, (float)(q11 & 255u) * s11, fx), fy);
        r.y = mix_(mix_((float)((q00 >> 8) & 255u) * s00, (float)((q10 >> 8) & 255u) * s10, fx), mix_((float)((q01 >> 8) & 255u) * s01, (float)((q11 >> 8) & 255u) * s11, fx), fy);
        r.z = mix_(mix_((float)((q00 >> 16) & 255u) * s00, (float)((q10 >> 16) & 255u) * s10, fx), mix_((float)((q01 >> 16) & 255u) * s01, (float)((q11 >> 16) & 255u) * s11, fx), fy);
        return r;
    }
    const float* t00 = P.envmap + kEnvTexelFloats * ((size_t)y0 * w + x0);
    const float* t10 = P.envmap + kEnvTexelFloats * ((size_t)y0 * w + x1);
    const float* t01 = P.envmap + kEnvTexelFloats * ((size_t)y1 * w + x0);
    const float* t11 = P.envmap + kEnvTexelFloats * ((size_t)y1 * w + x1);
    VR_TRACE(3, P.envmap, (t00 - P.envmap) * 4, 16); VR_TRACE(3, P.envmap, (t10 - P.envmap) * 4, 16);
    VR_TRACE(3, P.envmap, (t01 - P.envmap) * 4, 16); VR_TRACE(3, P.envmap, (t11 - P.envmap) * 4, 16);
    v3 r;
    r.x = mix_(mix_(t00[0], t10[0], fx), mix_(t01[0], t11[0], fx), fy);
    r.y = mix_(mix_(t00[1], t10[1], fx), mix_(t01[1], t11[1], fx), fy);
    r.z = mix_(mix_(t00[2], t10[2], fx), mix_(t01[2], t11[2], fx), fy);
    return r;
}
VR_HD int32_t imp_level_offset(int32_t dim, int32_t mip) { const int32_t d = dim >> mip; return (4 * dim * dim - 4 * d * d) / 3; }
VR_HD float imp_fetch(const SceneParams& P, int32_t x, int32_t y, int32_t mip) {
    const int32_t d = P.imp_dim >> mip;
    if (x < 0 || y < 0 || x >= d || y >= d) return 0.0f;
    return P.impmap[imp_level_offset(P.imp_dim, mip) + y * d + x];
}
VR_HD float env_average_importance(const SceneParams& P) { return P.env_avg_w_set ? P.env_avg_w : imp_fetch(P, 0, 0, P.u.env_imp_base_mip); }
VR_HD v3 lookup_environment(const SceneParams& P, v3 dir) {
    const v3 idir = mat3_mul(P.u.env_inv_transform, dir);
    const float u = atan2_(idir.z, idir.x) / (2.0f * kPi) + 0.5f;
    const float v = 1.0f - acos_(idir.y) / kPi;
    const v3 c = env_texture(P, u, v);
    return v3{ P.u.env_strength * c.x, P.u.env_strength * c.y, P.u.env_strength * c.z };
}
template <bool SAFE = false>
VR_HD int32_t env_warp_level(const float* rec, float& px, float& py, int32_t& posx, int32_t& posy) {
    const float d = rec[0], e0 = rec[1], e1 = rec[2];
    const bool right = !(px < d);
    const float e = right ? e1 : e0;
    const float nx = right ? px - d : px, dx = right ? 1.0f - d : d;
    px = SAFE ? div_core(nx, dx) : nx / dx;
    const bool up = !(py < e);
    const float ny = up ? py - e : py, dy = up ? 1.0f - e : e;
    py = SAFE ? div_core(ny, dy) : ny / dy;
    posx = 2 * posx + (right ? 1 : 0);
    posy = 2 * posy + (up ? 1 : 0);
    return (up ? 2 : 0) + (right ? 1 : 0);
}
#if defined(__HIP_DEVICE_COMPILE__)
template <bool ENVDC>
__device__ __forceinline__ void env_warp_block(float4 q0, float4 q1, float4 q2, float4 q3, float& px, float& py, int32_t& posx, int32_t& posy) {
    const float parent[3] = { q0.x, q0.y, q0.z };
    const int32_t c = env_warp_level<ENVDC>(parent, px, py, posx, posy);
    const bool c_right = (c & 1) != 0, c_up = (c & 2) != 0;
    const float lo_d = c_right ? q1.z : q0.w, lo_e0 = c_right ? q1.w : q1.x, lo_e1 = c_right ? q2.x : q1.y;
    const float hi_d = c_right ? q3.x : q2.y, hi_e0 = c_right ? q3.y : q2.z, hi_e1 = c_right ? q3.z : q2.w;
    const float child[3] = { c_up ? hi_d : lo_d, c_up ? hi_e0 : lo_e0, c_up ? hi_e1 : lo_e1 };
    env_warp_level<ENVDC>(child, px, py, posx, posy);
}
#endif
#ifndef VR_ENV_BLOCK_LOADS
#define VR_ENV_BLOCK_LOADS 1
#endif
#ifndef VR_ENV_SCALAR_TOP
#define VR_ENV_SCALAR_TOP 0
#endif
#ifndef VR_ENV_BLOCK_BELOW
#define VR_ENV_BLOCK_BELOW 64
#endif
template <bool BLOCK = true, bool ENVDC = false>
VR_HD void sample_environment(const SceneParams& P, float r0, float r1, v3& w_i, v3& Le, float& pdf_out) {
    int32_t posx = 0, posy = 0;
    float px = r0, py = r1;
    const int32_t top = P.u.env_imp_base_mip - 1;
    const float* blk = P.env_cdf;
    float w_texel = 0.0f;
    int32_t k = 0;
    if ((top & 1) == 0) {
        VR_TRACE(2, P.env_cdf, 0, 12);
        const int32_t c = env_warp_level<ENVDC>(blk, px, py, posx, posy);
        if (top == 0) w_texel = blk[3 + c];
        blk += kEnvCdfBlockFloats; k = 1;
    }
#if VR_ENV_BLOCK_LOADS && VR_ENV_SCALAR_TOP && defined(__HIP_DEVICE_COMPILE__)
    if (BLOCK && k == 0 && 1 < top) {
        typedef const float4 __attribute__((address_space(4))) * ConstQ;
        uint64_t addr = reinterpret_cast<uint64_t>(blk);
        asm("" : "+s"(addr));
        ConstQ cb = (ConstQ)(addr);
        env_warp_block<ENVDC>(cb[0], cb[1], cb[2], cb[3], px, py, posx, posy);
        blk += kEnvCdfBlockFloats; k = 2;
    }
#endif
    for (; k + 1 < top; k += 2) {
        const float* b = blk + kEnvCdfBlockFloats * (size_t)((posy << k) + posx);
        VR_TRACE(2, P.env_cdf, (b - P.env_cdf) * 4, 64);
#if VR_ENV_BLOCK_LOADS && defined(__HIP_DEVICE_COMPILE__)
        if (BLOCK && k < VR_ENV_BLOCK_BELOW) {
        const float4 q0 = reinterpret_cast<const float4*>(b)[0], q1 = reinterpret_cast<const float4*>(b)[1], q2 = reinterpret_cast<const float4*>(b)[2], q3 = reinterpret_cast<const float4*>(b)[3];
        env_warp_block<ENVDC>(q0, q1, q2, q3, px, py, posx, posy);
        } else
#endif
        {
        const int32_t c = env_warp_level<ENVDC>(b, px, py, posx, posy);
        env_warp_level<ENVDC>(b + 3 + 3 * c, px, py, posx, posy);
        }
        blk += (size_t)kEnvCdfBlockFloats << (2 * k);
    }
    if (k < top) {
        const int32_t s = (top & 1) ? 0 : 1;
        const float* b = P.env_cdf + env_cdf_last_pair_floats(s, (top + 1 - s) / 2) + kEnvCdfLastBlockFloats * (size_t)((posy << k) + posx);
        VR_TRACE(2, P.env_cdf, (b - P.env_cdf) * 4, 128);
        const int32_t c = env_warp_level<ENVDC>(b, px, py, posx, posy);
        const float* child = b + kEnvCdfLastChild0 + kEnvCdfLastChildFloats * c;
        float w4[4];
        ld_quad(child + 3, w4);
        const int32_t c2 = env_warp_level<ENVDC>(child, px, py, posx, posy);
        w_texel = c2 == 0 ? w4[0] : (c2 == 1 ? w4[1] : (c2 == 2 ? w4[2] : w4[3]));
    }
    const float u = ((float)posx + px) * P.u.env_imp_inv_dim[0];
    const float v = ((float)posy + py) * P.u.env_imp_inv_dim[1];
    const float theta = saturate(1.0f - v) * kPi;
    const float phi = (saturate(u) * 2.0f - 1.0f) * kPi;
    float sin_t, cos_t, sin_p, cos_p;
    sincos_(theta, sin_t, cos_t);
    sincos_(phi, sin_p, cos_p);
    w_i = mat3_mul(P.u.env_transform, v3{ sin_t * cos_p, cos_t, sin_t * sin_p });
    const v3 c = env_texture(P, u, v);
    Le = v3{ P.u.env_strength * c.x, P.u.env_strength * c.y, P.u.env_strength * c.z };
    const float avg_w = env_average_importance(P);
    pdf_out = (w_texel / avg_w) * kInv4Pi;
}

VR_HD float phase_hg(float cos_t, float g) {
    const float denom = 1.0f + sqr(g) + 2.0f * g * cos_t;
    return kInv4Pi * (1.0f - sqr(g)) / (denom * sqrt_(denom));
}
VR_HD v3 align(v3 N, v3 v) {
    const bool xa = abs_(N.x) > abs_(N.y);
    const float a = xa ? N.x : N.y;
    const v3 T = (xa ? v3{ -N.z, 0.0f, N.x } : v3{ 0.0f, N.z, -N.y }) / sqrt_(a * a + N.z * N.z);
    const v3 B = cross(N, T);
    return normalize(v3{ v.x * T.x + v.y * B.x + v.z * N.x,
                         v.x * T.y + v.y * B.y + v.z * N.y,
                         v.x * T.z + v.y * B.z + v.z * N.z });
}
VR_HD v3 sample_phase_hg(v3 dir, float g, float r0, float r1) {
    const float cos_t = abs_(g) < 1e-4f ? 1.0f - 2.0f * r0 :
        (1.0f + sqr(g) - sqr((1.0f - sqr(g)) / (1.0f - g + 2.0f * g * r0))) / (2.0f * g);
    const float sin_t = sqrt_(max_(0.0f, 1.0f - sqr(cos_t)));
    const float phi = 2.0f * kPi * r1;
    float sp, cp;
    sincos_(phi, sp, cp);
    return align(dir, v3{ sin_t * cp, sin_t * sp, cos_t });
}
VR_HD float power_heuristic(float a, float b) { return sqr(a) / (sqr(a) + sqr(b)); }

VR_HD v3 rcp3_exact(v3 v) {
#if defined(__HIP_DEVICE_COMPILE__) && !VR_FAST_DEVICE
    v3 r = v3{ rcp_newton(v.x), rcp_newton(v.y), rcp_newton(v.z) };
    if (!((int)rcp_in_fast_range(v.x) & (int)rcp_in_fast_range(v.y) & (int)rcp_in_fast_range(v.z))) r = v3{ 1.0f / v.x, 1.0f / v.y, 1.0f / v.z };
    return r;
#else
    return v3{ 1.0f / v.x, 1.0f / v.y, 1.0f / v.z };
#endif
}

VR_HD bool intersect_box(v3 pos, v3 dir, const float* bmin, const float* bmax, float& tnear, float& tfar) {
    const v3 inv = rcp3_exact(dir);
    const v3 lo = (v3{ bmin[0], bmin[1], bmin[2] } - pos) * inv;
    const v3 hi = (v3{ bmax[0], bmax[1], bmax[2] } - pos) * inv;
    const v3 tmin = v3{ min_(lo.x, hi.x), min_(lo.y, hi.y), min_(lo.z, hi.z) };
    const v3 tmax = v3{ max_(lo.x, hi.x), max_(lo.y, hi.y), max_(lo.z, hi.z) };
    tnear = max_(0.0f, max_(tmin.x, max_(tmin.y, tmin.z)));
    tfar = min_(tmax.x, min_(tmax.y, tmax.z));
    return tnear <= tfar;
}

#ifndef VR_DDA_INT_DIM
#define VR_DDA_INT_DIM 1
#endif
template <bool CLEAN = false>
VR_HD float step_dda(v3 p, v3 ri, int32_t mip) {
#if VR_DDA_INT_DIM
    const float dim = u2f((uint32_t)(130 + mip) << 23);
#else
    const float dim = (float)(8 << mip);
#endif
    const float idim = u2f((uint32_t)(124 - mip) << 23);
    const float ox = ri.x >= 0.0f ? dim + 0.5f : -0.5f;
    const float oy = ri.y >= 0.0f ? dim + 0.5f : -0.5f;
    const float oz = ri.z >= 0.0f ? dim + 0.5f : -0.5f;
    const float tx = (floor_(p.x * idim) * dim + ox - p.x) * ri.x;
    const float ty = (floor_(p.y * idim) * dim + oy - p.y) * ri.y;
    const float tz = (floor_(p.z * idim) * dim + oz - p.z) * ri.z;
    if (CLEAN) return __builtin_fminf(tx, __builtin_fminf(ty, tz));
    return min_(tx, min_(ty, tz));
}


VR_HD void hot_init(Hot& h) {
    h.seed = 0u; h.item = 0u;
    h.ipos = h.idir = h.ri = h.ethr = h.eL = h.shle = h.wpos = h.wdir = v3{ 0, 0, 0 };
    h.t = h.far = h.tau = h.majorant = h.Tr = 0.0f;
    h.mipq = 0;
    h.shadow = 0;
    h.state = ST_NEW;
    h.first = 0;
    h.maj_idx = -2; h.maj_raw = 0u;
}

#ifndef VR_SAMPLE_NT
#define VR_SAMPLE_NT 1
#endif
VR_HD void write_sample(const WorkUnit& wu, uint32_t item, v3 L, uint32_t n_paths) {
    float* o = wu.out + 4u * (size_t)item;
#if defined(__HIP_DEVICE_COMPILE__) && VR_SAMPLE_NT
    typedef float vr_f4 __attribute__((ext_vector_type(4)));
    __builtin_nontemporal_store(vr_f4{ L.x, L.y, L.z, n_paths > 0u ? 1.0f : 0.0f }, reinterpret_cast<vr_f4*>(o));
#elif defined(__HIP_DEVICE_COMPILE__)
    *reinterpret_cast<float4*>(o) = make_float4(L.x, L.y, L.z, n_paths > 0u ? 1.0f : 0.0f);
#else
    o[0] = L.x; o[1] = L.y; o[2] = L.z; o[3] = n_paths > 0u ? 1.0f : 0.0f;
#endif
}

VR_HD void accumulate_sample(float acc[4], const float L[4], int32_t current_sample) {
    const float a = 1.0f / (float)current_sample;
    acc[0] = mix_(acc[0], sanitize(L[0]), a);
    acc[1] = mix_(acc[1], sanitize(L[1]), a);
    acc[2] = mix_(acc[2], sanitize(L[2]), a);
    acc[3] = mix_(acc[3], sanitize(L[3]), a);
}

template <class K>
VR_HD bool begin_segment(Hot& h, const SceneParams& P, v3 pos, v3 d, int32_t shadow) {
    h.wpos = pos; h.wdir = d;
    h.shadow = shadow;
    h.Tr = 1.0f;
    h.mipq = 12;
    float tnear, tfar;
    if (!intersect_box(pos, d, P.u.vol_bb_min, P.u.vol_bb_max, tnear, tfar)) {
        h.state = segment_end_state(shadow);
        return false;
    }
    h.ipos = mat4_point(P.u.vol_density_inv_transform, pos);
    h.idir = mat4_dir(P.u.vol_density_inv_transform, d);
    h.far = tfar;
    if (K::global == 2 ? P.u.integrator != 0 : K::global == 1) {
        h.ri = v3{ 0, 0, 0 };
        h.tau = 0.0f;
        if (VR_CLEAN_FLAG) h.far = -tfar;
        h.t = tnear + neg_log_1m(rng(h.seed)) * P.u.vol_inv_majorant;
        if (h.t < tfar) { h.majorant = P.u.vol_majorant; h.state = ST_COLLIDE; }
        else h.state = segment_end_state(shadow);
        return true;
    }
    h.ri = rcp3_exact(h.idir);
    h.t = tnear + 1e-6f;
    h.tau = neg_log_1m(rng(h.seed));
    h.state = ST_MARCH;
#if VR_CLEAN_FLAG
    {
        const float ax = abs_(h.idir.x), ay = abs_(h.idir.y), az = abs_(h.idir.z), amax = __builtin_fmaxf(ax, __builtin_fmaxf(ay, az));
        const bool clean = (int)(abs_(h.ipos.x) < kCleanBound) & (int)(abs_(h.ipos.y) < kCleanBound) & (int)(abs_(h.ipos.z) < kCleanBound) &
                           (int)(ax * tfar < kCleanBound) & (int)(ay * tfar < kCleanBound) & (int)(az * tfar < kCleanBound) &
                           (int)(amax < kCleanBound) & (int)(amax >= 1.0f / kCleanBound);
        h.far = clean ? tfar : -tfar;
    }
#endif
    return true;
}

template <class K, class Cold, bool LAZY_EM = false>
VR_HD void do_new(Hot& h, Cold& c, const SceneParams& P, const WorkUnit& wu, uint32_t item) {
    const int32_t W = P.u.resolution[0], H = P.u.resolution[1];
    const int32_t px = wu.px0 + (int32_t)(item & 7u), py = wu.py0 + (int32_t)((item >> 3) & 7u);
    const int32_t smp = wu.first_sample + (int32_t)(item >> 6);
    if (px >= W || py >= H) return;
    h.seed = tea32((uint32_t)P.u.seed * (uint32_t)(py * W + px), (uint32_t)smp);
    const float jx = rng(h.seed), jy = rng(h.seed);
    const float fx = (((float)px + jx) - (float)W * 0.5f) / (float)H;
    const float fy = (((float)py + jy) - (float)H * 0.5f) / (float)H;
// ... 146 lines not shown
    if (t >= seg_far(h)) { h.state = segment_end_state(h.shadow); return; }
    h.majorant = maj;
    h.state = ST_COLLIDE;
}
#endif
template <bool TF, int DENSE = 2, int MAJB = 2>
VR_HD void do_march(Hot& h, const SceneParams& P) {
    if (!(h.t < seg_far(h))) { h.state = segment_end_state(h.shadow); return; }
    const v3 curr = axpy(h.ipos, h.t, h.idir);
    const int32_t m = round_mip_q(h.mipq);
    const float majorant = majorant_at<TF, DENSE, MAJB>(P, curr, m);
    const float dt = step_dda(curr, h.ri, m);
    h.t += dt;
    h.tau -= majorant * dt;
    h.mipq = h.mipq < 12 ? h.mipq + 1 : 12;
    if (h.tau > 0.0f) return;
    h.t += h.tau / majorant;
    if (h.t >= seg_far(h)) { h.state = segment_end_state(h.shadow); return; }
    h.majorant = majorant;
    h.state = ST_COLLIDE;
}

template <class K> struct CollideIO {
    TapAddr a; TapData d;
    TriIO tri;
    TapAddr ea; TapData ed;
};
template <class K, bool CLEAN = false>
VR_HD void collide_prep(Hot& h, const SceneParams& P, const SceneParams& PE, CollideIO<K>& io) {
    const v3 ip = axpy(h.ipos, h.t, h.idir);
    if (K::tf) {
        trilinear_prep<K::dense, !CLEAN>(P.density, ip, io.tri);
    } else {
        int32_t tx, ty, tz;
        tricubic_tap<!CLEAN>(ip, h.seed, tx, ty, tz);
        io.a = tap_addr<K::dense>(P.density, tx, ty, tz);
    }
    io.ea.cell = io.ea.off = 0u; io.ea.in = false;
    if (!h.shadow) {
        if (K::emission == 2 ? P.u.has_emission != 0 : K::emission == 1) {
            const v3 ie = mat4_point(PE.emission_from_density, ip);
            int32_t ex, ey, ez;
            tricubic_tap(ie, h.seed, ex, ey, ez);
            io.ea = tap_addr<K::edense>(PE.emission, ex, ey, ez);
        } else {
            rng_skip9(h.seed);
        }
    }
}
template <class K>
VR_HD void collide_idle(CollideIO<K>& io) {
    io.a.cell = io.a.off = 0u; io.a.in = false;
    io.ea.cell = io.ea.off = 0u; io.ea.in = false;
    if (K::tf) trilinear_idle(io.tri);
}
template <class K, bool CLEAN = false>
VR_HD void collide_prep(Hot& h, const SceneParams& P, CollideIO<K>& io) { collide_prep<K, CLEAN>(h, P, P, io); }
template <class K>
VR_HD void collide_load(const SceneParams& P, const SceneParams& PE, CollideIO<K>& io) {
    if (K::tf) trilinear_load<K::dense, K::pair_d, K::a32>(P.density, io.tri);
    else io.d = tap_load<K::dense, K::pair_d, K::a32>(P.density, io.a);
    if (K::emission == 2 ? P.u.has_emission != 0 : K::emission == 1) io.ed = tap_load<K::edense, K::pair_e, K::a32>(PE.emission, io.ea);
}
template <class K>
VR_HD void collide_load(const SceneParams& P, CollideIO<K>& io) { collide_load<K>(P, P, io); }
#ifndef VR_SHADOW_BLOCKED_SHORTCUT
#define VR_SHADOW_BLOCKED_SHORTCUT (!VR_FAST_DEVICE)
#endif
template <class K, class Cold, bool CACHED = false>
VR_HD void collide_finish(Hot& h, Cold& c, const SceneParams& P, const SceneParams& PE, const CollideIO<K>& io, const float* tf_lut) {
    constexpr bool USE_TF = K::tf;
    const Uniforms& u = P.u;
    const bool global = K::global == 2 ? u.integrator != 0 : K::global == 1;
    float d;
    float rgba[4] = { 0, 0, 0, 0 };
    if (USE_TF) {
        tf_lookup_at(u, tf_lut, (u.vol_density_scale * trilinear_value<K::dense>(P.density, io.tri)) * u.vol_inv_majorant, rgba);
        d = u.vol_majorant * rgba[3];
    } else {
        d = u.vol_density_scale * tap_value<K::dense>(P.density, io.d, io.a.in);
    }
    if (!h.shadow) {
        const float P_real = d * u.vol_inv_majorant;
        if (K::emission == 2 ? u.has_emission != 0 : K::emission == 1) {
            const float tt = tap_value<K::edense>(PE.emission, io.ed, io.ea.in) * u.vol_emission_norm;
            const v3 e3 = v3{ tt, sqr(tt), sqr(sqr(tt)) };
            const v3 em = v3{ u.vol_emission_scale * sqr(e3.x), u.vol_emission_scale * sqr(e3.y), u.vol_emission_scale * sqr(e3.z) };
            const v3 oma = v3{ 1.0f - u.vol_albedo[0], 1.0f - u.vol_albedo[1], 1.0f - u.vol_albedo[2] };
            const v3 thr = CACHED ? h.ethr : ld3(c, C_THR);
            const v3 L0 = CACHED ? h.eL : ld3(c, C_L);
            const v3 L1 = global ? L0 + ((thr * oma) * em) * P_real : L0 + (((thr * oma) * em) * d) * u.vol_inv_majorant;
            if (CACHED) h.eL = L1; else st3(c, C_L, L1);
        }
        if (global ? rng(h.seed) < P_real : rng(h.seed) * h.majorant < d) {
            if (USE_TF) st3(c, C_COL, v3{ rgba[0], rgba[1], rgba[2] });
            h.state = ST_NEE;
            return;
        }
    } else if (global) {
        h.Tr *= 1.0f - d * u.vol_inv_majorant;
        if (h.Tr < 0.1f) {
            const float prob = 1.0f - h.Tr;
            if (rng(h.seed) < prob) { h.Tr = 0.0f; h.state = ST_POSTNEE; return; }
            h.Tr /= 1.0f - prob;
        }
    } else {
        if (rng(h.seed) * h.majorant < d) {
#if VR_SHADOW_BLOCKED_SHORTCUT
            if ((h.majorant > 0.0f) & (h.majorant <= u.vol_majorant) & (abs_(h.Tr) < inf_())) {
                (void)rng(h.seed);
                h.Tr = 0.0f;
                h.state = ST_POSTNEE;
                return;
            }
#endif
            const float ratio = (K::global == 0 && !K::tf) ? div_core(u.vol_majorant, h.majorant) : u.vol_majorant / h.majorant;
            h.Tr *= max_(0.0f, 1.0f - ratio);
            if (h.Tr < 0.1f) {
                const float prob = 1.0f - h.Tr;
                if (rng(h.seed) < prob) { h.Tr = 0.0f; h.state = ST_POSTNEE; return; }
                h.Tr /= 1.0f - prob;
            }
        }
    }
    if (global) {
        h.t = h.t + neg_log_1m(rng(h.seed)) * u.vol_inv_majorant;
        if (!(h.t < seg_far(h))) h.state = segment_end_state(h.shadow);
        return;
    }
    h.tau = neg_log_1m(rng(h.seed));
    h.mipq = h.mipq > 8 ? h.mipq - 8 : 0;
    h.state = ST_MARCH;
}
template <class K, class Cold, bool CACHED = false>
VR_HD void collide_finish(Hot& h, Cold& c, const SceneParams& P, const CollideIO<K>& io, const float* tf_lut) { collide_finish<K, Cold, CACHED>(h, c, P, P, io, tf_lut); }
template <class K, class Cold, bool CLEAN = false>
VR_HD void do_collide(Hot& h, Cold& c, const SceneParams& P) {
    CollideIO<K> io;
    collide_prep<K, CLEAN>(h, P, io);
    collide_load<K>(P, io);
    collide_finish<K>(h, c, P, io, P.tf_lut);
}

template <class K, class Cold, bool SHLE_IN_HOT = false, bool ITEM_IN_HOT = false, bool FIRST_L_IN_HOT = false>
VR_HD void do_nee(Hot& h, Cold& c, const Cold& crd, const SceneParams& P) {
    const bool first = h.first != 0;
    constexpr bool WS = world_slot<K>();
    if (!WS) {
        v3 dir = ld3(crd, C_DIR), pos0 = ld3(crd, C_POS), thr = ld3(crd, C_THR);
        h.first = 0;
        const float r0 = rng(h.seed), r1 = rng(h.seed);
        float pdf;
        v3 w_i, Le;
        sample_environment<K::global != 2, K::global != 2>(P, r0, r1, w_i, Le, pdf);
        dir = v3{ first ? h.ipos.x : dir.x, first ? h.ipos.y : dir.y, first ? h.ipos.z : dir.z };
        pos0 = v3{ first ? P.u.cam_pos[0] : pos0.x, first ? P.u.cam_pos[1] : pos0.y, first ? P.u.cam_pos[2] : pos0.z };
        thr = v3{ first ? 1.0f : thr.x, first ? 1.0f : thr.y, first ? 1.0f : thr.z };
        const v3 pos = axpy(pos0, h.t, dir);
        const v3 alb = v3{ P.u.vol_albedo[0], P.u.vol_albedo[1], P.u.vol_albedo[2] };
        if (K::global == 2 ? P.u.integrator != 0 : K::global == 1) thr = K::tf ? thr * (ld3(c, C_COL) * alb) : thr * alb;
        else { thr = thr * alb; if (K::tf) thr = thr * ld3(c, C_COL); }
        if (first) {
            st3(c, C_L, FIRST_L_IN_HOT ? h.eL : v3{ 0, 0, 0 }); stu(c, C_NPATHS, 0u);
            st3(c, C_DIR, dir);
            c.st(C_FP, 0.0f);
            if (!ITEM_IN_HOT) stu(c, C_ITEM, f2u(h.Tr));
        }
        const bool lit = pdf > 0.0f;
        const float f_p = phase_hg(dot(-dir, w_i), P.u.vol_phase_g);
        st3(c, C_POS, pos); c.st(C_SHPDF, lit ? pdf : 0.0f);
        st3(c, C_THR, thr); c.st(C_FPL, lit ? f_p : 0.0f);
        if (lit) {
            if (SHLE_IN_HOT) h.shle = Le; else st3(c, C_SHLE, Le);
            begin_segment<K>(h, P, pos, w_i, 1);
        } else {
            h.shadow = 0;
            h.state = ST_POSTNEE;
        }
        return;
    }
    v3 dir, pos0, thr;
    if (WS) {
        dir = h.wdir; pos0 = h.wpos; thr = v3{ 1.0f, 1.0f, 1.0f };
    } else {
        dir = ld3(crd, C_DIR); pos0 = ld3(crd, C_POS); thr = ld3(crd, C_THR);
        dir = v3{ first ? h.ipos.x : dir.x, first ? h.ipos.y : dir.y, first ? h.ipos.z : dir.z };
        pos0 = v3{ first ? P.u.cam_pos[0] : pos0.x, first ? P.u.cam_pos[1] : pos0.y, first ? P.u.cam_pos[2] : pos0.z };
        thr = v3{ first ? 1.0f : thr.x, first ? 1.0f : thr.y, first ? 1.0f : thr.z };
    }
    const v3 pos = axpy(pos0, h.t, dir);
    if (WS) {
        if (first) st3(c, C_THR, thr);
    } else
    {
        const v3 alb = v3{ P.u.vol_albedo[0], P.u.vol_albedo[1], P.u.vol_albedo[2] };
        if (K::global == 2 ? P.u.integrator != 0 : K::global == 1) thr = K::tf ? thr * (ld3(c, C_COL) * alb) : thr * alb;
        else { thr = thr * alb; if (K::tf) thr = thr * ld3(c, C_COL); }
    }
    if (first) {
        st3(c, C_L, FIRST_L_IN_HOT ? h.eL : v3{ 0, 0, 0 }); stu(c, C_NPATHS, 0u);
        if (!WS) st3(c, C_DIR, dir);
        c.st(C_FP, 0.0f);
        if (!ITEM_IN_HOT) stu(c, C_ITEM, f2u(h.Tr));
    }
    h.first = 0;
    const float r0 = rng(h.seed), r1 = rng(h.seed);
    float pdf;
    v3 w_i, Le;
    sample_environment<K::global != 2, K::global != 2>(P, r0, r1, w_i, Le, pdf);
    if (WS) {
        const bool lit = pdf > 0.0f;
        st3(c, C_DIR, dir); c.st(C_SHPDF, lit ? pdf : 0.0f);
        if (lit) {
            if (SHLE_IN_HOT) h.shle = Le; else st3(c, C_SHLE, Le);
            begin_segment<K>(h, P, pos, w_i, 1);
        } else {
            h.wpos = pos;
            h.shadow = 0;
            h.state = ST_POSTNEE;
        }
        return;
    }
    const bool lit = pdf > 0.0f;
    const float f_p = phase_hg(dot(-dir, w_i), P.u.vol_phase_g);
    st3(c, C_POS, pos); c.st(C_SHPDF, lit ? pdf : 0.0f);
    st3(c, C_THR, thr); c.st(C_FPL, lit ? f_p : 0.0f);
    if (lit) {
        if (SHLE_IN_HOT) h.shle = Le; else st3(c, C_SHLE, Le);
        begin_segment<K>(h, P, pos, w_i, 1);
    } else {
        h.shadow = 0;
        h.state = ST_POSTNEE;
    }
}

template <class K, class Cold, bool SHLE_IN_HOT = false, bool ITEM_IN_HOT = false>
VR_HD void do_postnee(Hot& h, Cold& c, const SceneParams& P, const WorkUnit& wu) {
    constexpr bool WS = world_slot<K>();
    const Quad q_l = ld4(c, C_L, C_NPATHS), q_p = WS ? Quad{ h.wpos, 0.0f } : ld4(c, C_POS, C_SHPDF);
    const Quad q_t = ld4(c, C_THR, WS ? C_FP : C_FPL), q_d = ld4(c, C_DIR, WS ? C_SHPDF : C_FP);
    v3 L = q_l.a;
    const float sh_pdf = WS ? q_d.b : q_p.b;
    v3 thr = q_t.a;
    if (WS) thr = thr * v3{ P.u.vol_albedo[0], P.u.vol_albedo[1], P.u.vol_albedo[2] };
    const float fpl_kept = WS ? 0.0f : q_t.b;
    if (sh_pdf > 0.0f) {
        const float f_p = WS ? phase_hg(dot(-q_d.a, h.wdir), P.u.vol_phase_g) : fpl_kept;
        const float mis = P.u.show_environment > 0 ? power_heuristic(sh_pdf, f_p) : 1.0f;
        L = L + ((((thr * mis) * f_p) * h.Tr) * (SHLE_IN_HOT ? h.shle : ld3(c, C_SHLE))) / sh_pdf;
    }
    const uint32_t n_paths = f2u(q_l.b) + 1u;
    if (n_paths >= (uint32_t)P.u.bounces) { write_sample(wu, ITEM_IN_HOT ? h.item : ldu(c, C_ITEM), L, n_paths); h.state = ST_NEW; return; }
    const float rr = luma(thr);
    if (rr < 0.1f) {
        const float prob = 1.0f - rr;
        if (rng(h.seed) < prob) { write_sample(wu, ITEM_IN_HOT ? h.item : ldu(c, C_ITEM), L, n_paths); h.state = ST_NEW; return; }
        thr = thr / (1.0f - prob);
        if (!WS) { st3(c, C_THR, thr); c.st(C_FPL, fpl_kept); }
    }
    const v3 dir = q_d.a;
    const float s0 = rng(h.seed), s1 = rng(h.seed);
    const v3 sd = sample_phase_hg(dir, P.u.vol_phase_g, s0, s1);
    const float f_p_next = phase_hg(dot(-dir, sd), P.u.vol_phase_g);
    if (WS) {
        st3(c, C_L, L); stu(c, C_NPATHS, n_paths);
        st3(c, C_THR, thr); c.st(C_FP, f_p_next);
    } else {
        st3(c, C_L, L); stu(c, C_NPATHS, n_paths);
        st3(c, C_DIR, sd); c.st(C_FP, f_p_next);
    }
    begin_segment<K>(h, P, q_p.a, sd, 0);
}

template <class Cold, bool ITEM_IN_HOT = false, bool FIRST_L_IN_HOT = false, bool WS = false>
VR_HD void do_escape(Hot& h, const Cold& c, const SceneParams& P, const WorkUnit& wu) {
    const bool first = h.first != 0;
    v3 L = ld3(c, C_L), thr = ld3(c, C_THR), dir = ld3(c, C_DIR);
    uint32_t n_paths = ldu(c, C_NPATHS), item = ITEM_IN_HOT ? h.item : ldu(c, C_ITEM);
    const float f_p = c.ld(C_FP);
    v3 Le_early = v3{ 0.0f, 0.0f, 0.0f };
    if (WS && P.u.show_environment > 0) Le_early = lookup_environment(P, h.wdir);
    const v3 L_first = FIRST_L_IN_HOT ? h.eL : v3{ 0.0f, 0.0f, 0.0f };
    L = v3{ first ? L_first.x : L.x, first ? L_first.y : L.y, first ? L_first.z : L.z };
    thr = v3{ first ? 1.0f : thr.x, first ? 1.0f : thr.y, first ? 1.0f : thr.z };
    if (WS) dir = h.wdir;
    else dir = v3{ first ? h.ipos.x : dir.x, first ? h.ipos.y : dir.y, first ? h.ipos.z : dir.z };
    n_paths = first ? 0u : n_paths;
    item = first ? f2u(h.Tr) : item;
    h.first = 0;
    if (P.u.show_environment > 0) {
        const v3 Le = WS ? Le_early : lookup_environment(P, dir);
        float mis = 1.0f;
        if (n_paths > 0u) {
            const float avg_w = env_average_importance(P);
            const float pdf_env = (luma(Le) / avg_w) * kInv4Pi;
            mis = power_heuristic(f_p, pdf_env);
        }
        L = L + (thr * mis) * Le;
    }
    write_sample(wu, item, L, n_paths);
    h.state = ST_NEW;
}

VR_HD void dvr_sample(const SceneParams& P, int32_t px, int32_t py, int32_t smp, float out[4]) {
    const Uniforms& u = P.u;
    const int32_t W = u.resolution[0], H = u.resolution[1];
    uint32_t seed = tea32((uint32_t)u.seed * (uint32_t)(py * W + px), (uint32_t)smp);
    const float jx = rng(seed), jy = rng(seed);
    const float fx = (((float)px + jx) - (float)W * 0.5f) / (float)H;
    const float fy = (((float)py + jy) - (float)H * 0.5f) / (float)H;
    const v3 dir = normalize(mat3_mul(u.cam_transform, normalize(v3{ fx, fy, P.cam_z })));
    const v3 pos = v3{ u.cam_pos[0], u.cam_pos[1], u.cam_pos[2] };
    v3 L = v3{ 0, 0, 0 };
    float tnear, tfar;
    if (!intersect_box(pos, dir, u.vol_bb_min, u.vol_bb_max, tnear, tfar)) {
        const v3 e = lookup_environment(P, dir);
        out[0] = e.x; out[1] = e.y; out[2] = e.z; out[3] = 0.0f;
        return;
    }
    const v3 ipos = mat4_point(u.vol_density_inv_transform, pos);
    const v3 idir = mat4_dir(u.vol_density_inv_transform, dir);
    const float dt = (tfar - tnear) / 64.0f;
    tnear += rng(seed) * dt;
    float Tr = 1.0f;
    for (int32_t i = 0; i < 64; ++i) {
        float rgba[4];
        const v3 ip = axpy(ipos, min_(tnear + (float)i * dt, tfar), idir);
        tf_lookup(P, (u.vol_density_scale * density_trilinear_raw(P.density, ip)) * u.vol_inv_majorant, rgba);
        const float dtau = rgba[3] * u.vol_majorant * dt;
        L = L + (v3{ rgba[0], rgba[1], rgba[2] } * dtau) * Tr;
        Tr *= exp_(-dtau);
        if (Tr <= 1e-6f) { out[0] = L.x; out[1] = L.y; out[2] = L.z; out[3] = 1.0f - Tr; return; }
    }
    const v3 e = lookup_environment(P, dir);
    L = L + e * Tr;
    out[0] = L.x; out[1] = L.y; out[2] = L.z; out[3] = 1.0f - Tr;
}

enum FeatureResult : int32_t { FEAT_MISS = 0, FEAT_HIT = 1, FEAT_LOST = 2 };
constexpr uint32_t kFeatureMaxSteps = 1u << 20;
struct FeatureCold {
    float v[C_COUNT];
    VR_HD float ld(int32_t f) const { return v[f]; }
    VR_HD void st(int32_t f, float x) { v[f] = x; }
};
template <bool TF>
VR_HD int32_t feature_sample(const SceneParams& P, int32_t px, int32_t py, int32_t smp, float& t, v3& albedo, v3& normal) {
    using K = TraceCfg<TF, 0, 2, 2, 2, false>;
    const Uniforms& u = P.u;
    const int32_t W = u.resolution[0], H = u.resolution[1];
    Hot h;
    hot_init(h);
    h.seed = tea32((uint32_t)u.seed * (uint32_t)(py * W + px), (uint32_t)smp);
    const float jx = rng(h.seed), jy = rng(h.seed);
    const float fx = (((float)px + jx) - (float)W * 0.5f) / (float)H;
    const float fy = (((float)py + jy) - (float)H * 0.5f) / (float)H;
    const v3 dir = normalize(mat3_mul(u.cam_transform, normalize(v3{ fx, fy, P.cam_z })));
    const v3 pos = v3{ u.cam_pos[0], u.cam_pos[1], u.cam_pos[2] };
    if (!begin_segment<K>(h, P, pos, dir, 0)) return FEAT_MISS;
    FeatureCold c;
    for (int32_t i = 0; i < C_COUNT; ++i) c.v[i] = 0.0f;
    for (uint32_t steps = 0u; h.state == ST_MARCH || h.state == ST_COLLIDE; ++steps) {
        if (steps >= kFeatureMaxSteps) return FEAT_LOST;
        if (h.state == ST_MARCH) {
            const float t0 = h.t, tau0 = h.tau;
            const int32_t mip0 = h.mipq;
            do_march<TF, 2, 2>(h, P);
            if (h.state == ST_MARCH && h.t == t0 && h.tau == tau0 && h.mipq == mip0) return FEAT_MISS;
        } else {
            do_collide<K, FeatureCold, false>(h, c, P);
        }
    }
    if (h.state != ST_NEE) return FEAT_MISS;
    t = h.t;
    albedo = v3{ u.vol_albedo[0], u.vol_albedo[1], u.vol_albedo[2] };
    if (TF) albedo = albedo * ld3(c, C_COL);
    const v3 ip = axpy(h.ipos, h.t, h.idir);
    const v3 g = v3{ density_trilinear_raw(P.density, v3{ ip.x + 1.0f, ip.y, ip.z }) - density_trilinear_raw(P.density, v3{ ip.x - 1.0f, ip.y, ip.z }),
                     density_trilinear_raw(P.density, v3{ ip.x, ip.y + 1.0f, ip.z }) - density_trilinear_raw(P.density, v3{ ip.x, ip.y - 1.0f, ip.z }),
                     density_trilinear_raw(P.density, v3{ ip.x, ip.y, ip.z + 1.0f }) - density_trilinear_raw(P.density, v3{ ip.x, ip.y, ip.z - 1.0f }) };
    const float* m = u.vol_density_inv_transform;
    const v3 n = v3{ (m[0] * g.x + m[1] * g.y) + m[2] * g.z, (m[4] * g.x + m[5] * g.y) + m[6] * g.z, (m[8] * g.x + m[9] * g.y) + m[10] * g.z };
    normal = (n.x == 0.0f && n.y == 0.0f && n.z == 0.0f) ? v3{ 0, 0, 0 } : -normalize(n);
    return FEAT_HIT;
}
template <bool TF>
VR_HD bool feature_pixel(const SceneParams& P, int32_t px, int32_t py, int32_t spp, float out[8]) {
    int32_t hits = 0;
    v3 sa = v3{ 0, 0, 0 }, sn = v3{ 0, 0, 0 };
    float sd = 0.0f;
    bool ok = true;
    for (int32_t s = 1; s <= spp; ++s) {
        float t = 0.0f;
        v3 a, n;
        const int32_t r = feature_sample<TF>(P, px, py, s, t, a, n);
        if (r == FEAT_LOST) { ok = false; break; }
        if (r != FEAT_HIT) continue;
        ++hits;
        sa = sa + a; sn = sn + n; sd += t;
    }
    for (int32_t i = 0; i < 8; ++i) out[i] = 0.0f;
    if (hits == 0) return ok;
    const float fh = (float)hits;
    out[0] = sa.x / fh; out[1] = sa.y / fh; out[2] = sa.z / fh; out[3] = fh / (float)spp;
    out[4] = sn.x / fh; out[5] = sn.y / fh; out[6] = sn.z / fh; out[7] = sd / fh;
    return ok;
}

VR_HD float raymarch_density(const SceneParams& P, v3 ip, uint32_t& seed) {
    int32_t tx, ty, tz;
    tricubic_tap(ip, seed, tx, ty, tz);
    return P.u.vol_density_scale * brick_value<2>(P.density, tx, ty, tz);
}
VR_HD float transmittance_raymarch(const SceneParams& P, v3 wpos, v3 wdir, uint32_t& seed) {
    const Uniforms& u = P.u;
    float tnear, tfar;
    if (!intersect_box(wpos, wdir, u.vol_bb_min, u.vol_bb_max, tnear, tfar)) return 1.0f;
    const v3 ipos = mat4_point(u.vol_density_inv_transform, wpos);
    const v3 idir = mat4_dir(u.vol_density_inv_transform, wdir);
    const float dt = (tfar - tnear) / 64.0f;
    tnear += rng(seed) * dt;
    float tau = 0.0f;
    for (int32_t i = 0; i < 64; ++i) {
        const float d = raymarch_density(P, axpy(ipos, min_(tnear + (float)i * dt, tfar), idir), seed);
        if (u.use_tf) {
            float rgba[4];
            tf_lookup(P, d * u.vol_inv_majorant, rgba);
            tau += rgba[3] * u.vol_majorant * dt;
        } else {
            tau += d * dt;
        }
    }
    return exp_(-tau);
}
VR_HD bool sample_volume_raymarch(const SceneParams& P, v3 wpos, v3 wdir, float& t, v3& throughput, uint32_t& seed) {
    const Uniforms& u = P.u;
    float tnear, tfar;
    if (!intersect_box(wpos, wdir, u.vol_bb_min, u.vol_bb_max, tnear, tfar)) return false;
    const v3 ipos = mat4_point(u.vol_density_inv_transform, wpos);
    const v3 idir = mat4_dir(u.vol_density_inv_transform, wdir);
    const float tau_target = neg_log_1m(rng(seed));
    const float dt = (tfar - tnear) / 64.0f;
    tnear += rng(seed) * dt;
    float tau = 0.0f;
    for (int32_t i = 0; i < 64; ++i) {
        t = min_(tnear + (float)i * dt, tfar);
        const float d = raymarch_density(P, axpy(ipos, t, idir), seed);
        float rgba[4] = { 0, 0, 0, 0 };
        if (u.use_tf) {
            tf_lookup(P, d * u.vol_inv_majorant, rgba);
            tau += rgba[3] * u.vol_majorant * dt;
        } else {
            tau += d * dt;
        }
        if (tau >= tau_target) {
            const v3 alb = u.use_tf ? v3{ rgba[0] * u.vol_albedo[0], rgba[1] * u.vol_albedo[1], rgba[2] * u.vol_albedo[2] }
                                    : v3{ u.vol_albedo[0], u.vol_albedo[1], u.vol_albedo[2] };
            throughput = throughput * alb;
            return true;
        }
    }
    return false;
}
VR_HD void raymarch_path_sample(const SceneParams& P, int32_t px, int32_t py, int32_t smp, float out[4]) {
    const Uniforms& u = P.u;
    const int32_t W = u.resolution[0], H = u.resolution[1];
    uint32_t seed = tea32((uint32_t)u.seed * (uint32_t)(py * W + px), (uint32_t)smp);
    const float jx = rng(seed), jy = rng(seed);
    const float fx = (((float)px + jx) - (float)W * 0.5f) / (float)H;
    const float fy = (((float)py + jy) - (float)H * 0.5f) / (float)H;
    v3 dir = normalize(mat3_mul(u.cam_transform, normalize(v3{ fx, fy, P.cam_z })));
    v3 pos = v3{ u.cam_pos[0], u.cam_pos[1], u.cam_pos[2] };
    v3 L = v3{ 0, 0, 0 }, thr = v3{ 1, 1, 1 };
    bool free_path = true;
    uint32_t n_paths = 0u;
    float t = 0.0f, f_p = 0.0f;
    while (sample_volume_raymarch(P, pos, dir, t, thr, seed)) {
        pos = axpy(pos, t, dir);
        const float r0 = rng(seed), r1 = rng(seed);
        float pdf;
        v3 w_i, Le;
        sample_environment(P, r0, r1, w_i, Le, pdf);
        if (pdf > 0.0f) {
            f_p = phase_hg(dot(-dir, w_i), u.vol_phase_g);
            const float mis = u.show_environment > 0 ? power_heuristic(pdf, f_p) : 1.0f;
            const float Tr = transmittance_raymarch(P, pos, w_i, seed);
            L = L + ((((thr * mis) * f_p) * Tr) * Le) / pdf;
        }
        if (++n_paths >= (uint32_t)u.bounces) { free_path = false; break; }
        const float rr = luma(thr);
        if (rr < 0.1f) {
            const float prob = 1.0f - rr;
            if (rng(seed) < prob) { free_path = false; break; }
            thr = thr / (1.0f - prob);
        }
        const float s0 = rng(seed), s1 = rng(seed);
        const v3 sd = sample_phase_hg(dir, u.vol_phase_g, s0, s1);
        f_p = phase_hg(dot(-dir, sd), u.vol_phase_g);
        dir = sd;
    }
    if (free_path && u.show_environment > 0) {
        const v3 Le = lookup_environment(P, dir);
        float mis = 1.0f;
        if (n_paths > 0u) {
            const float avg_w = env_average_importance(P);
            mis = power_heuristic(f_p, (luma(Le) / avg_w) * kInv4Pi);
        }
        L = L + (thr * mis) * Le;
    }
    out[0] = L.x; out[1] = L.y; out[2] = L.z; out[3] = n_paths > 0u ? 1.0f : 0.0f;
}

template <class K, class Cold>
VR_HD void lane_step(Hot& h, Cold& c, const SceneParams& P, const WorkUnit& wu, uint32_t& next_item, FirstStash& stash) {
    if (h.first && (h.state == ST_NEE || h.state == ST_ESCAPE)) { h.ipos = stash.dir; h.Tr = u2f(stash.item); }
    switch (h.state) {
    case ST_NEW:
        if (next_item >= (uint32_t)wu.n_items) { h.state = ST_DONE; break; }
        do_new<K>(h, c, P, wu, next_item++);
        if (h.first) { stash.dir = h.ipos; stash.item = f2u(h.Tr); first_resume(h, P); }
        break;
    case ST_MARCH: { MarchIO io; if (seg_clean(h)) march_prep<K::dense, K::majb, true>(h, P, io); else march_prep<K::dense, K::majb, false>(h, P, io); march_load<K::tf, K::a32>(P, io); if (seg_clean(h)) march_finish<K::tf, false, true>(h, P, io); else march_finish<K::tf, false, false>(h, P, io); break; }
    case ST_COLLIDE: if (seg_clean(h)) do_collide<K, Cold, true>(h, c, P); else do_collide<K, Cold, false>(h, c, P); break;
    case ST_NEE: do_nee<K>(h, c, c, P); break;
    case ST_POSTNEE: do_postnee<K>(h, c, P, wu); break;
    case ST_ESCAPE: do_escape<Cold, false, false, world_slot<K>()>(h, c, P, wu); break;
    default: break;
    }
}

}
```

### volren_amd/renderer.py

```python
import ctypes as C

import numpy as np

from . import _lib

_INT_FIELDS = ("sample", "sppx", "seed", "bounces", "show_environment", "tonemapping", "integrator", "grid_frame_counter",
               "sample_pool_mb", "gpu_encoder", "fast_math", "tf_float_atlas", "launch_target_ms", "order_tiles", "coalesce_trace", "majorant_layout",
               "variance", "denoise_iterations", "wide_addressing")
_FLOAT_FIELDS = {"tonemap_exposure": 1, "tonemap_gamma": 1, "albedo": 3, "phase": 1, "density_scale": 1,
                 "emission_scale": 1, "vol_clip_min": 3, "vol_clip_max": 3, "env_strength": 1, "env_transform": 9,
                 "tf_window_left": 1, "tf_window_width": 1, "cam_pos": 3, "cam_dir": 3, "cam_up": 3, "cam_fov": 1,
                 "volume_transform": 16, "denoise_sigma": 5, "denoise_alpha": 1}


def _f32(a):
    return np.ascontiguousarray(a, dtype=np.float32)


class Renderer:

    def __init__(self, width, height, device=0, _borrowed=None):
        object.__setattr__(self, "_h", None)
        L = _lib.load()
        object.__setattr__(self, "_owned", _borrowed is None)
        if _borrowed is None:
            h = C.c_void_p()
            _lib.check(L.vr_create(C.byref(h), int(device), int(width), int(height)))
        else:
            h = C.c_void_p(_borrowed)
        object.__setattr__(self, "_h", h)
        object.__setattr__(self, "_L", L)
        object.__setattr__(self, "width", int(width))
        object.__setattr__(self, "height", int(height))

    def close(self):
        if self._h is not None:
            if self._owned:
                self._L.vr_destroy(self._h)
            object.__setattr__(self, "_h", None)

    def __del__(self):
        try:
            self.close()
        except Exception:
            pass

    def get_int(self, name):
        v = C.c_int()
        _lib.check(self._L.vr_get_int(self._h, name.encode(), C.byref(v)))
        return v.value

    def __getattr__(self, name):
        if name in _INT_FIELDS or name in ("n_grid_frames", "last_launches", "pending_samples", "majorant_blocked", "env_div_safe", "env_compact", "kernel_variant", "kernel_variant_reason", "kernel_wide",
                                              "adaptive_rounds"):
            v = C.c_int()
            _lib.check(self._L.vr_get_int(self._h, name.encode(), C.byref(v)))
            return bool(v.value) if name in ("show_environment", "tonemapping") else v.value
        if name in _FLOAT_FIELDS:
            n = _FLOAT_FIELDS[name]
            buf = (C.c_float * n)()
            _lib.check(self._L.vr_get_float(self._h, name.encode(), buf, n))
            return buf[0] if n == 1 else np.array(buf[:], np.float32)
        raise AttributeError(name)

    def __setattr__(self, name, value):
        if name in _INT_FIELDS:
            _lib.check(self._L.vr_set_int(self._h, name.encode(), int(value)))
        elif name in _FLOAT_FIELDS or name == "env_rot":
            v = _f32(np.atleast_1d(value)).reshape(-1)
            _lib.check(self._L.vr_set_float(self._h, name.encode(), v.ctypes.data_as(C.POINTER(C.c_float)), v.size))
        else:
            object.__setattr__(self, name, value)

    def has_fast_math(self):
        return True

    def load_volume(self, path):
        _lib.check(self._L.vr_load_volume(self._h, str(path).encode()))

    def set_volume_path(self, path):
        _lib.check(self._L.vr_set_volume_path(self._h, str(path).encode()))

    def volume_aabb(self, name="density"):
        out = (C.c_float * 6)()
        _lib.check(self._L.vr_volume_aabb(self._h, name.encode(), out))
        return np.array(out[:3], np.float32), np.array(out[3:], np.float32)

    def volume_minorant_majorant(self, name="density"):
        out = (C.c_float * 2)()
        _lib.check(self._L.vr_volume_minorant_majorant(self._h, name.encode(), out))
        return float(out[0]), float(out[1])

    def load_envmap(self, path):
        _lib.check(self._L.vr_load_envmap(self._h, str(path).encode()))

    def load_transferfunc(self, path):
        _lib.check(self._L.vr_load_transferfunc(self._h, str(path).encode()))

    def set_volume_dense(self, voxels_zyx, transform=None, name="density", unit_cube=True, commit=True):
        v = _f32(voxels_zyx)
        nz, ny, nx = v.shape
        t = _f32(transform).reshape(16) if transform is not None else None
        _lib.check(self._L.vr_set_volume_dense(self._h, name.encode(), v.ctypes.data, nx, ny, nz,
                                               t.ctypes.data if t is not None else None, 1 if unit_cube else 0))
        if commit:
            self.commit()

    def volume_add_grid_frame(self, voxels_zyx, name="density", transform=None):
        v = _f32(voxels_zyx)
        nz, ny, nx = v.shape
        t = _f32(transform).reshape(16) if transform is not None else None
        _lib.check(self._L.vr_volume_add_grid_frame_dense(self._h, name.encode(), v.ctypes.data, nx, ny, nz, t.ctypes.data if t is not None else None))

    def volume_update_grid_frame(self, frame, voxels_zyx, name="density", transform=None):
        v = _f32(voxels_zyx)
        nz, ny, nx = v.shape
        t = _f32(transform).reshape(16) if transform is not None else None
        _lib.check(self._L.vr_volume_update_grid_frame_dense(self._h, int(frame), name.encode(), v.ctypes.data, nx, ny, nz, t.ctypes.data if t is not None else None))

    def volume_n_grid_frames(self):
        n = C.c_int()
        _lib.check(self._L.vr_volume_n_grid_frames(self._h, C.byref(n)))
        return n.value

    def set_volume_dense_f16(self, voxels_zyx, transform=None, name="density", unit_cube=True, commit=True):
        v = np.ascontiguousarray(voxels_zyx, dtype=np.float16)
        nz, ny, nx = v.shape
        t = _f32(transform).reshape(16) if transform is not None else None
        _lib.check(self._L.vr_set_volume_dense_f16(self._h, name.encode(), v.ctypes.data, nx, ny, nz,
                                                   t.ctypes.data if t is not None else None, 1 if unit_cube else 0))
        if commit:
            self.commit()

    def set_volume_brick(self, transform, n_bricks, min_maj, indirection, rng, atlas_dim, atlas, mips=(), name="density",
                         unit_cube=True, commit=True):
        t = _f32(transform).reshape(16)
        nb = np.asarray(n_bricks, np.uint32)
        mm = _f32(min_maj)
        ind = np.ascontiguousarray(indirection, np.uint32)
        rg = np.ascontiguousarray(rng, np.uint32)
        ad = np.asarray(atlas_dim, np.uint32)
        at = np.ascontiguousarray(atlas, np.uint8)
        mip_arrays = [np.ascontiguousarray(a, np.uint32) for _, a in mips]
        mip_ptrs = (C.c_void_p * max(1, len(mips)))(*[a.ctypes.data for a in mip_arrays])
        mip_dims = np.asarray([d for d, _ in mips], np.uint32).reshape(-1, 3) if mips else np.zeros((1, 3), np.uint32)
        _lib.check(self._L.vr_set_volume_brick(self._h, name.encode(), t.ctypes.data, nb.ctypes.data, mm.ctypes.data,
                                               ind.ctypes.data, rg.ctypes.data, ad.ctypes.data, at.ctypes.data,
                                               len(mips), C.cast(mip_ptrs, C.c_void_p), mip_dims.ctypes.data, 1 if unit_cube else 0))
        if commit:
            self.commit()

    def set_envmap(self, rgb_top_first):
        a = _f32(rgb_top_first)
        _lib.check(self._L.vr_set_envmap(self._h, a.ctypes.data, a.shape[1], a.shape[0]))

    def set_transferfunc(self, lut):
        if lut is None:
            _lib.check(self._L.vr_set_transferfunc(self._h, None, 0))
            return
        a = _f32(lut)
        _lib.check(self._L.vr_set_transferfunc(self._h, a.ctypes.data, a.shape[0]))
# ... 263 lines not shown
```

Measured before the change: 5636 Msamples/s.

## Route wave queues with precomputed ballot masks and fold env average into kernel args

Queue routing now takes one ballot per target state up front and pushes slots using those masks, replacing the per-queue ballot and lost-lane handling in specialized kernels. Specialized kernels treat the environment average importance as a kernel argument that is known to be set, and read it (plus show_environment) into scalar registers early. A new toggle sends scenes without that argument to the generic variant. The world-space inverse transform is also forced into scalar registers, and finer sub-section timing hooks are added. These target scalar-side overhead and redundant ballots in the wave scheduler, at the cost of extra live registers.

```diff
diff --git a/volren_amd/csrc/capi.cpp b/volren_amd/csrc/capi.cpp
--- a/volren_amd/csrc/capi.cpp
+++ b/volren_amd/csrc/capi.cpp
@@ -283,6 +283,7 @@
         else if (n == "coalesce_trace") { R.flush_pending(); R.coalesce_trace = v != 0; }
         else if (n == "majorant_layout") { if (v < -1 || v > 1) throw std::runtime_error("majorant_layout: -1 (per grid, chosen at commit), 0 (linear), 1 (4x4x4-cell blocks)"); R.majorant_layout = v; }
         else if (n == "tf_float_atlas") R.tf_float_atlas = v != 0;
+        else if (n == "env_average_arg") { if (v < 0 || v > 1) throw std::runtime_error("env_average_arg: 1 (the average importance is a kernel argument), 0 (left unset: the run-time variant fetches it)"); R.env_average_arg = v != 0; }
         else if (n == "wide_addressing") { if (v < 0 || v > 1) throw std::runtime_error("wide_addressing: 0 (by the tables' sizes), 1 (always the kernels with 64-bit gather addresses)"); R.tuning.wide_addressing = v; }
         else if (n == "gpu_encoder") R.gpu_encoder = v != 0;
         else if (n == "sample_pool_mb") { if (v < 16 || v > 65536) throw std::runtime_error("sample_pool_mb must be in [16, 65536] (item indices of a sub-launch are 32-bit: < 2^32 RGBA32F items)"); R.sample_pool_bytes = (size_t)v << 20; }
@@ -330,6 +331,7 @@
         else if (n == "env_compact") *v = R.environment && R.environment->envmap_rgbe ? 1 : 0;
         else if (n == "pending_samples") *v = R.pending_samples();
         else if (n == "tf_float_atlas") *v = R.tf_float_atlas ? 1 : 0;
+        else if (n == "env_average_arg") *v = R.env_average_arg ? 1 : 0;
         else if (n == "gpu_encoder") *v = R.gpu_encoder ? 1 : 0;
         else if (n == "sample_pool_mb") *v = (int)(R.sample_pool_bytes >> 20);
         else if (n == "launch_target_ms") *v = R.launch_target_ms;
diff --git a/volren_amd/csrc/renderer.cpp b/volren_amd/csrc/renderer.cpp
--- a/volren_amd/csrc/renderer.cpp
+++ b/volren_amd/csrc/renderer.cpp
@@ -368,7 +368,7 @@
         const mat4 efd = eti * dt;
         memcpy(P.emission_from_density, efd.m, sizeof efd.m);
         const bool scale_ok = u.vol_density_scale >= 1.0f / 65536.0f && u.vol_density_scale <= 16777216.0f;
-        P.paired = (integrator == 0 && environment->cdf_div_safe && scale_ok && density.atlas_paired && density.atlas_paired == emission.atlas_paired) ? 1 : 0;
+        P.paired = (integrator == 0 && environment->cdf_div_safe && env_average_arg && scale_ok && density.atlas_paired && density.atlas_paired == emission.atlas_paired) ? 1 : 0;
         if (P.paired) P.density = make_view(density, true, majorant_layout < 0 ? density.maj_blocked : majorant_layout == 1);
         P.emission = make_view(emission, P.paired != 0);
         u.has_emission = 1;
@@ -389,7 +389,7 @@
     P.envmap = environment->envmap->as<float>();
     P.env_rgbe = environment->envmap_rgbe ? environment->envmap_rgbe->as<uint32_t>() : nullptr;
     P.env_w = environment->width; P.env_h = environment->height;
-    P.env_avg_w = environment->avg_importance; P.env_avg_w_set = 1;
+    P.env_avg_w = env_average_arg ? environment->avg_importance : 0.0f; P.env_avg_w_set = env_average_arg ? 1 : 0;
     P.impmap = environment->impmap->as<float>();
     P.imp_dim = (int)environment->dimension();
     P.env_cdf = environment->cdf->as<float>();
diff --git a/volren_amd/csrc/renderer.h b/volren_amd/csrc/renderer.h
--- a/volren_amd/csrc/renderer.h
+++ b/volren_amd/csrc/renderer.h
@@ -102,6 +102,7 @@
     bool tf_float_atlas = true;
     int order_tiles = 1;
     int majorant_layout = -1;
+    bool env_average_arg = true;
     int variance = 0;
     int denoise_iterations = kDenoiseDefaultIterations;
     float denoise_sigma[5] = { kDenoiseDefaultSigma[0], kDenoiseDefaultSigma[1], kDenoiseDefaultSigma[2], kDenoiseDefaultSigma[3], kDenoiseDefaultSigma[4] };
diff --git a/volren_amd/csrc/vr_device.h b/volren_amd/csrc/vr_device.h
--- a/volren_amd/csrc/vr_device.h
+++ b/volren_amd/csrc/vr_device.h
@@ -30,7 +30,8 @@
     VR_VARIANT_INTEGRATOR = 1,
     VR_VARIANT_ENV_DIVISION = 2,
     VR_VARIANT_DENSITY_SCALE = 4,
-    VR_VARIANT_GRID_FORMS = 8
+    VR_VARIANT_GRID_FORMS = 8,
+    VR_VARIANT_ENV_AVERAGE = 16
 };
 int pathtrace_variant_of(const SceneParams& P, int* why);
 bool pathtrace_wide_of(const PathtraceTuning& T, const SceneParams& P);
diff --git a/volren_amd/csrc/vr_launch.hip b/volren_amd/csrc/vr_launch.hip
--- a/volren_amd/csrc/vr_launch.hip
+++ b/volren_amd/csrc/vr_launch.hip
@@ -128,6 +128,7 @@
     if (P.u.integrator != 0) reason |= VR_VARIANT_INTEGRATOR;
     if (!P.env_div_safe) reason |= VR_VARIANT_ENV_DIVISION;
     if (!scale_ok) reason |= VR_VARIANT_DENSITY_SCALE;
+    if (!P.env_avg_w_set) reason |= VR_VARIANT_ENV_AVERAGE;
     int variant;
     if (reason) variant = 3;
     else if (P.u.has_emission) {
diff --git a/volren_amd/csrc/vr_pathtrace.h b/volren_amd/csrc/vr_pathtrace.h
--- a/volren_amd/csrc/vr_pathtrace.h
+++ b/volren_amd/csrc/vr_pathtrace.h
@@ -167,8 +167,12 @@
         load(h, slot);
         const bool first = h.first != 0;
         if (WORLD) {
-            h.ipos = mat4_point(inv_transform, h.wpos);
-            h.idir = mat4_dir(inv_transform, h.wdir);
+            float m[16];
+#pragma unroll
+            for (int i = 0; i < 16; ++i) m[i] = (i & 3) == 3 ? 0.0f : inv_transform[i];
+            asm volatile("" : "+s"(m[0]), "+s"(m[1]), "+s"(m[2]), "+s"(m[4]), "+s"(m[5]), "+s"(m[6]), "+s"(m[8]), "+s"(m[9]), "+s"(m[10]), "+s"(m[12]), "+s"(m[13]), "+s"(m[14]));
+            h.ipos = mat4_point(m, h.wpos);
+            h.idir = mat4_dir(m, h.wdir);
         } else
         h.ipos = v3{ first ? cam_ipos[0] : h.ipos.x, first ? cam_ipos[1] : h.ipos.y, first ? cam_ipos[2] : h.ipos.z };
         h.Tr = first ? 1.0f : h.Tr;
@@ -466,29 +470,53 @@
 #ifndef VR_READY_FIFO
 #define VR_READY_FIFO 0
 #endif
+#define VR_PUSH_M(QI, CNT, M, COND, SLOTV) do { \
+        if (M) { if (COND) q[(QI) * NS + (CNT) + (int32_t)lane_rank(M)] = (uint8_t)(SLOTV); (CNT) += popc(M); } \
+    } while (0)
 #if VR_READY_FIFO
+#define VR_PUSH_READY_M(M, COND, SLOTV) VR_PUSH_READY(COND, SLOTV)
 #define VR_PUSH_READY(COND, SLOTV) do { \
         const uint64_t m_ = wave_ballot(COND); \
         if (m_) { if (COND) { int32_t p_ = rdy_head + cnt_ready + (int32_t)lane_rank(m_); p_ = p_ >= NS ? p_ - NS : p_; q[Q_READY * NS + p_] = (uint8_t)(SLOTV); } cnt_ready += popc(m_); } \
     } while (0)
 #else
 #define VR_PUSH_READY(COND, SLOTV) VR_PUSH(Q_READY, cnt_ready, COND, SLOTV)
+#define VR_PUSH_READY_M(M, COND, SLOTV) VR_PUSH_M(Q_READY, cnt_ready, M, COND, SLOTV)
 #endif
 #define VR_ROUTE_ST(BS, STV) do { \
          \
         const int32_t s_ = (BS) >= 0 ? (STV) : -1; \
-        VR_PUSH_READY((uint32_t)(s_ - ST_MARCH) < 2u, BS);                         \
-        VR_PUSH(Q_NEE, cnt_nee, s_ == ST_NEE, BS); \
-        VR_PUSH(Q_POST, cnt_post, s_ == ST_POSTNEE, BS); \
-        VR_PUSH(Q_ESC, cnt_esc, s_ == ST_ESCAPE, BS); \
-        const bool lost_ = s_ == ST_BEGIN || s_ > ST_ESCAPE || s_ < -1; \
-        if (wave_ballot(lost_)) { if (lost_) atomicOr(event_args().status, 2u); } \
-        const int32_t free0_ = cnt_free; \
-        VR_PUSH(Q_FREE, cnt_free, s_ == ST_NEW || lost_, BS); \
-        if (cnt_free != free0_) { idle_iters = 0u; t_elapsed = 0u; }           \
+        if (kRouteMasks) { \
+            const bool cr_ = (uint32_t)(s_ - ST_MARCH) < 2u, cn_ = s_ == ST_NEE, cp_ = s_ == ST_POSTNEE, ce_ = s_ == ST_ESCAPE, cw_ = s_ == ST_NEW;       \
+            const bool lost_ = s_ != -1 && !(cr_ || cn_ || cp_ || ce_ || cw_);             \
+            const bool cf_ = cw_ || lost_; \
+            const uint64_t mr_ = wave_ballot(cr_), mn_ = wave_ballot(cn_), mp_ = wave_ballot(cp_), me_ = wave_ballot(ce_), mw_ = wave_ballot(cw_); \
+            const uint64_t ml_ = wave_ballot(s_ != -1) & ~(mr_ | mn_ | mp_ | me_ | mw_), mf_ = mw_ | ml_;       \
+            if (ml_) { if (lost_) atomicOr(event_args().status, 2u); } \
+            VR_PUSH_READY_M(mr_, cr_, BS); \
+            VR_PUSH_M(Q_NEE, cnt_nee, mn_, cn_, BS); \
+            VR_PUSH_M(Q_POST, cnt_post, mp_, cp_, BS); \
+            VR_PUSH_M(Q_ESC, cnt_esc, me_, ce_, BS); \
+            VR_PUSH_M(Q_FREE, cnt_free, mf_, cf_, BS); \
+            if (mf_) { idle_iters = 0u; t_elapsed = 0u; }                      \
+        } else {                                                               \
+            VR_PUSH_READY((uint32_t)(s_ - ST_MARCH) < 2u, BS);                     \
+            VR_PUSH(Q_NEE, cnt_nee, s_ == ST_NEE, BS); \
+            VR_PUSH(Q_POST, cnt_post, s_ == ST_POSTNEE, BS); \
+            VR_PUSH(Q_ESC, cnt_esc, s_ == ST_ESCAPE, BS); \
+            const bool lost_ = s_ == ST_BEGIN || s_ > ST_ESCAPE || s_ < -1; \
+            if (wave_ballot(lost_)) { if (lost_) atomicOr(event_args().status, 2u); } \
+            const int32_t free0_ = cnt_free; \
+            VR_PUSH(Q_FREE, cnt_free, s_ == ST_NEW || lost_, BS); \
+            if (cnt_free != free0_) { idle_iters = 0u; t_elapsed = 0u; } \
+        } \
     } while (0)
+#ifndef VR_ROUTE_MASKS
+#define VR_ROUTE_MASKS 1
+#endif
+    constexpr bool kRouteMasks = VR_ROUTE_MASKS != 0 && K::global == 0 && K::emission == 0 && !(K::tf && K::dense == 0);
 #define VR_ROUTE(BS) VR_ROUTE_ST(BS, l.state)
-#define VR_ROUTE_B(BS) VR_ROUTE_ST(BS, b.state)
+#define VR_ROUTE_B(BS) do { VR_SUB_BEGIN(); VR_ROUTE_ST(BS, b.state); VR_SUB_END(2 * ST_BEGIN, false); if (STATS_T && VR_STAT_SCHED) stat_add(2 * ST_BEGIN + 1, 1u); } while (0)
 
     for (;;) {
         ++iters;
@@ -507,8 +535,13 @@
         uint32_t t_sec = STATS_T ? (uint32_t)__builtin_readcyclecounter() : 0u;
         if (STATS_T && have_tail) stat_add(26 + 4, t_sec - t_tail);
 #define VR_SECTION(K) do { if (STATS_T) { const uint32_t n_ = (uint32_t)__builtin_readcyclecounter(); stat_add(26 + (K), n_ - t_sec); t_sec = n_; } } while (0)
+        uint32_t t_sub = 0u;
+#define VR_SUB_BEGIN() do { if (STATS_T) t_sub = (uint32_t)__builtin_readcyclecounter(); } while (0)
+#define VR_SUB_END(I, DRAIN) do { if (STATS_T) { if (DRAIN) __builtin_amdgcn_s_waitcnt(0xC07F);  stat_add((I), (uint32_t)__builtin_readcyclecounter() - t_sub); } } while (0)
 #else
 #define VR_SECTION(K) do { } while (0)
+#define VR_SUB_BEGIN() do { } while (0)
+#define VR_SUB_END(I, DRAIN) do { } while (0)
 #endif
         {
             const uint64_t idle = wave_ballot(slot < 0);
@@ -693,6 +726,7 @@
             }
         }
         VR_SECTION(2);
+        VR_SUB_BEGIN();
         int32_t n;
         const int32_t n_live = popc(wave_ballot(slot >= 0)) + cnt_ready;
         const bool hungry = n_live < VR_THR_HUNGRY;
@@ -706,6 +740,7 @@
         const bool want_nee = cnt_nee > 0 && (cnt_nee >= VR_THR_NEE || (hungry && (cnt_nee == big || drain_all)));
         const bool want_post = cnt_post > 0 && (cnt_post >= VR_THR_POST || (hungry && (cnt_post == big || drain_all)));
         const bool want_esc = cnt_esc > 0 && (cnt_esc >= VR_THR_ESC || (hungry && (cnt_esc == big || drain_all)));
+        VR_SUB_END(31, false);
         if (want_new || want_nee || want_post || want_esc) {
 #if VR_BATCH_REGS
             Hot b;
@@ -721,7 +756,9 @@
                 n = min(64, cnt_esc);
                 VR_STAT(ST_ESCAPE, n);
                 int32_t bs = -1;
+                VR_SUB_BEGIN();
                 if (lane < n) { bs = q[Q_ESC * NS + cnt_esc - 1 - lane]; hs.load(b, bs); if (kLazyEm && b.first) b.eL = hs.load_first_radiance(bs); }
+                VR_SUB_END(18 + ST_BEGIN, true);
                 if (kItemInRegs) b.item = item_fetch(banks, lane, bs);
                 if constexpr (kColdRegs) {
                     ColdLocal c;
@@ -730,14 +767,14 @@
                     if (lane < n) {
                         const KernelArgs& E = event_args();
                         WorkUnit w; w.out = E.sbuf;
-                        do_escape<ColdLocal, false>(b, c, E.P, w);
+                        do_escape<ColdLocal, false, false, false, K::global != 2>(b, c, E.P, w);
                     }
                 } else
                 if (lane < n) {
                     const ColdT c = VR_COLD(b.first ? 0 : bs);
                     const KernelArgs& E = event_args();
                     WorkUnit w; w.out = E.sbuf;
-                    do_escape<ColdT, kItemInRegs, kLazyEm, kWorld>(b, c, E.P, w);
+                    do_escape<ColdT, kItemInRegs, kLazyEm, kWorld, K::global != 2>(b, c, E.P, w);
                 }
                 cnt_esc -= n;
                 VR_ROUTE_B(bs);
@@ -747,7 +784,9 @@
                 n = min(64, cnt_post);
                 VR_STAT(ST_POSTNEE, n);
                 int32_t bs = -1;
+                VR_SUB_BEGIN();
                 if (lane < n) { bs = q[Q_POST * NS + cnt_post - 1 - lane]; hs.load(b, bs); }
+                VR_SUB_END(18 + ST_BEGIN, true);
                 if (kShleInRegs) b.shle = shle_fetch(banks, lane, bs);
                 if (kItemInRegs) b.item = item_fetch(banks, lane, bs);
                 if constexpr (kColdRegs) {
@@ -812,7 +851,9 @@
                 int32_t bs = -1;
                 bool was_first = false;
                 uint32_t first_item = 0u;
+                VR_SUB_BEGIN();
                 if (lane < n) { bs = q[Q_NEE * NS + cnt_nee - 1 - lane]; hs.load(b, bs); }
+                VR_SUB_END(18 + ST_BEGIN, true);
                 if constexpr (kColdRegs) {
                     ColdLocal c;
                     cold_clear(c);
@@ -875,8 +916,12 @@
 #undef VR_THR_COLLIDE
 #undef VR_STAT_END
 #undef VR_SECTION
+#undef VR_SUB_BEGIN
+#undef VR_SUB_END
 #undef VR_PUSH
 #undef VR_PUSH_READY
+#undef VR_PUSH_M
+#undef VR_PUSH_READY_M
 #undef VR_ROUTE
 #undef VR_ROUTE_B
 #undef VR_ROUTE_ST
diff --git a/volren_amd/csrc/vr_probe.h b/volren_amd/csrc/vr_probe.h
--- a/volren_amd/csrc/vr_probe.h
+++ b/volren_amd/csrc/vr_probe.h
@@ -51,6 +51,7 @@
     case PROBE_SKY: return form != 0 ? "form out of range" : nullptr;
     case PROBE_LIGHT:
         if (form > 1) return "form out of range";
+        if (form == 0 && !P.env_avg_w_set) return "the sampler of the kernels of one scene kind without the average importance as an argument (env_avg_w_set = 0)";
         return (form == 0 && !P.env_div_safe) ? "the div_core sampler on a warp table that failed the division check (env_div_safe = 0)" : nullptr;
     case PROBE_TF:
         if (form != 0) return "form out of range";
diff --git a/volren_amd/csrc/vr_trace.h b/volren_amd/csrc/vr_trace.h
--- a/volren_amd/csrc/vr_trace.h
+++ b/volren_amd/csrc/vr_trace.h
@@ -647,7 +647,15 @@
     if (x < 0 || y < 0 || x >= d || y >= d) return 0.0f;
     return P.impmap[imp_level_offset(P.imp_dim, mip) + y * d + x];
 }
-VR_HD float env_average_importance(const SceneParams& P) { return P.env_avg_w_set ? P.env_avg_w : imp_fetch(P, 0, 0, P.u.env_imp_base_mip); }
+#ifndef VR_ENV_AVG_EARLY
+#if defined(VR_FAST_MATH) && VR_FAST_MATH
+#define VR_ENV_AVG_EARLY 2
+#else
+#define VR_ENV_AVG_EARLY 3
+#endif
+#endif
+template <bool ARG = false>
+VR_HD float env_average_importance(const SceneParams& P) { return (ARG || P.env_avg_w_set) ? P.env_avg_w : imp_fetch(P, 0, 0, P.u.env_imp_base_mip); }
 VR_HD v3 lookup_environment(const SceneParams& P, v3 dir) {
     const v3 idir = mat3_mul(P.u.env_inv_transform, dir);
     const float u = atan2_(idir.z, idir.x) / (2.0f * kPi) + 0.5f;
@@ -690,12 +698,20 @@
 #ifndef VR_ENV_BLOCK_BELOW
 #define VR_ENV_BLOCK_BELOW 64
 #endif
-template <bool BLOCK = true, bool ENVDC = false>
+template <bool BLOCK = true, bool ENVDC = false, bool AVG = false>
 VR_HD void sample_environment(const SceneParams& P, float r0, float r1, v3& w_i, v3& Le, float& pdf_out) {
     int32_t posx = 0, posy = 0;
     float px = r0, py = r1;
     const int32_t top = P.u.env_imp_base_mip - 1;
     const float* blk = P.env_cdf;
+#if defined(__HIP_DEVICE_COMPILE__)
+    constexpr bool EARLY = AVG && (VR_ENV_AVG_EARLY & 1) != 0;
+    float avg_arg = 0.0f;
+    if (EARLY) { avg_arg = P.env_avg_w; asm volatile("" : "+s"(avg_arg)); }
+#else
+    constexpr bool EARLY = false;
+    const float avg_arg = 0.0f;
+#endif
     float w_texel = 0.0f;
     int32_t k = 0;
     if ((top & 1) == 0) {
@@ -750,7 +766,7 @@
     w_i = mat3_mul(P.u.env_transform, v3{ sin_t * cos_p, cos_t, sin_t * sin_p });
     const v3 c = env_texture(P, u, v);
     Le = v3{ P.u.env_strength * c.x, P.u.env_strength * c.y, P.u.env_strength * c.z };
-    const float avg_w = env_average_importance(P);
+    const float avg_w = EARLY ? avg_arg : env_average_importance<AVG>(P);
     pdf_out = (w_texel / avg_w) * kInv4Pi;
 }
 
@@ -1203,7 +1219,7 @@
         const float r0 = rng(h.seed), r1 = rng(h.seed);
         float pdf;
         v3 w_i, Le;
-        sample_environment<K::global != 2, K::global != 2>(P, r0, r1, w_i, Le, pdf);
+        sample_environment<K::global != 2, K::global != 2, K::global != 2>(P, r0, r1, w_i, Le, pdf);
         dir = v3{ first ? h.ipos.x : dir.x, first ? h.ipos.y : dir.y, first ? h.ipos.z : dir.z };
         pos0 = v3{ first ? P.u.cam_pos[0] : pos0.x, first ? P.u.cam_pos[1] : pos0.y, first ? P.u.cam_pos[2] : pos0.z };
         thr = v3{ first ? 1.0f : thr.x, first ? 1.0f : thr.y, first ? 1.0f : thr.z };
@@ -1258,7 +1274,7 @@
     const float r0 = rng(h.seed), r1 = rng(h.seed);
     float pdf;
     v3 w_i, Le;
-    sample_environment<K::global != 2, K::global != 2>(P, r0, r1, w_i, Le, pdf);
+    sample_environment<K::global != 2, K::global != 2, K::global != 2>(P, r0, r1, w_i, Le, pdf);
     if (WS) {
         const bool lit = pdf > 0.0f;
         st3(c, C_DIR, dir); c.st(C_SHPDF, lit ? pdf : 0.0f);
@@ -1323,14 +1339,25 @@
     begin_segment<K>(h, P, q_p.a, sd, 0);
 }
 
-template <class Cold, bool ITEM_IN_HOT = false, bool FIRST_L_IN_HOT = false, bool WS = false>
+template <class Cold, bool ITEM_IN_HOT = false, bool FIRST_L_IN_HOT = false, bool WS = false, bool AVG = false>
 VR_HD void do_escape(Hot& h, const Cold& c, const SceneParams& P, const WorkUnit& wu) {
     const bool first = h.first != 0;
     v3 L = ld3(c, C_L), thr = ld3(c, C_THR), dir = ld3(c, C_DIR);
     uint32_t n_paths = ldu(c, C_NPATHS), item = ITEM_IN_HOT ? h.item : ldu(c, C_ITEM);
     const float f_p = c.ld(C_FP);
     v3 Le_early = v3{ 0.0f, 0.0f, 0.0f };
-    if (WS && P.u.show_environment > 0) Le_early = lookup_environment(P, h.wdir);
+#if defined(__HIP_DEVICE_COMPILE__)
+    constexpr bool EARLY = AVG && (VR_ENV_AVG_EARLY & 2) != 0;
+    float avg_arg = 0.0f;
+    int32_t show_early = 0;
+    if (EARLY) { avg_arg = P.env_avg_w; show_early = P.u.show_environment; asm volatile("" : "+s"(avg_arg), "+s"(show_early)); }
+#else
+    constexpr bool EARLY = false;
+    const float avg_arg = 0.0f;
+    const int32_t show_early = 0;
+#endif
+    const auto show_env = [&]() { return EARLY ? show_early > 0 : P.u.show_environment > 0; };
+    if (WS && show_env()) Le_early = lookup_environment(P, h.wdir);
     const v3 L_first = FIRST_L_IN_HOT ? h.eL : v3{ 0.0f, 0.0f, 0.0f };
     L = v3{ first ? L_first.x : L.x, first ? L_first.y : L.y, first ? L_first.z : L.z };
     thr = v3{ first ? 1.0f : thr.x, first ? 1.0f : thr.y, first ? 1.0f : thr.z };
@@ -1339,11 +1366,11 @@
     n_paths = first ? 0u : n_paths;
     item = first ? f2u(h.Tr) : item;
     h.first = 0;
-    if (P.u.show_environment > 0) {
+    if (show_env()) {
         const v3 Le = WS ? Le_early : lookup_environment(P, dir);
         float mis = 1.0f;
         if (n_paths > 0u) {
-            const float avg_w = env_average_importance(P);
+            const float avg_w = EARLY ? avg_arg : env_average_importance<AVG>(P);
             const float pdf_env = (luma(Le) / avg_w) * kInv4Pi;
             mis = power_heuristic(f_p, pdf_env);
         }
@@ -1575,7 +1602,7 @@
     case ST_COLLIDE: if (seg_clean(h)) do_collide<K, Cold, true>(h, c, P); else do_collide<K, Cold, false>(h, c, P); break;
     case ST_NEE: do_nee<K>(h, c, c, P); break;
     case ST_POSTNEE: do_postnee<K>(h, c, P, wu); break;
-    case ST_ESCAPE: do_escape<Cold, false, false, world_slot<K>()>(h, c, P, wu); break;
+    case ST_ESCAPE: do_escape<Cold, false, false, world_slot<K>(), K::global != 2>(h, c, P, wu); break;
     default: break;
     }
 }
diff --git a/volren_amd/renderer.py b/volren_amd/renderer.py
--- a/volren_amd/renderer.py
+++ b/volren_amd/renderer.py
@@ -6,7 +6,7 @@
 
 _INT_FIELDS = ("sample", "sppx", "seed", "bounces", "show_environment", "tonemapping", "integrator", "grid_frame_counter",
                "sample_pool_mb", "gpu_encoder", "fast_math", "tf_float_atlas", "launch_target_ms", "order_tiles", "coalesce_trace", "majorant_layout",
-               "variance", "denoise_iterations", "wide_addressing")
+               "variance", "denoise_iterations", "wide_addressing", "env_average_arg")
 _FLOAT_FIELDS = {"tonemap_exposure": 1, "tonemap_gamma": 1, "albedo": 3, "phase": 1, "density_scale": 1,
                  "emission_scale": 1, "vol_clip_min": 3, "vol_clip_max": 3, "env_strength": 1, "env_transform": 9,
                  "tf_window_left": 1, "tf_window_width": 1, "cam_pos": 3, "cam_dir": 3, "cam_up": 3, "cam_fov": 1,
```

Result: no change. 5640 Msamples/s (median of 2 runs) (+0.1%).
